# GAVLab/feature_extraction

Measured on AMD Instinct MI355X. Metric: VLP-16 scans/sec (16x1800 pts), detector+descriptor, higher is better.
Workload: dtype f32; 1 GPU; batch of 1024 synthetic VLP-16 scans (16x1800 pts, 64 uniform poles) per GPU, device-resident, preset 'launch', roll/pitch 0.02/-0.015; scans_per_gpu=1024, preset=launch, parallelism=frame-sharded x1, batches_in_flight=4

## Files before the change

feature_extraction_amd/capi.py:

```python
import ctypes as C
import os

import numpy as np

_HERE = os.path.dirname(os.path.abspath(__file__))
LIB_PATH = os.path.join(_HERE, "lib", "libfx_hip.so")

FX_DESC_BINS = 1980
FX_DESC_FLOATS = 1989
FX_FEATURE_RECORD_BYTES = 7984
FX_OK = 0
FX_ERR_NO_DEVICE = 2
FX_IN_DEVICE, FX_OUT_HOST, FX_OUT_DEBUG, FX_OUT_CLOUDS = 1, 2, 4, 8
FX_FLAG_RING_OVERFLOW, FX_FLAG_CAND_OVERFLOW, FX_FLAG_KP_OVERFLOW, FX_FLAG_NBR_OVERFLOW = 0x1, 0x2, 0x4, 0x8
FX_FLAG_NAMES = {0x1: "RING_OVERFLOW", 0x2: "CAND_OVERFLOW", 0x4: "KP_OVERFLOW", 0x8: "NBR_OVERFLOW",
                 0x10: "TOTAL_KP_OVERFLOW", 0x20: "KPC_OVERFLOW"}
FX_N_STAGES = 9
STAGE_NAMES = ("k_prep", "k_bucket", "k_rings_runs", "k_rings_large", "k_merge", "k_gather", "k_desc_group", "k_desc_mid",
               "k_desc_rare")
SINGLE_LAUNCH_STAGES = ("k_prep", "k_bucket", "k_rings_runs", "k_gather", "k_desc_group", "k_desc_mid")
STAGE_KERNELS = {"k_prep": ("k_prep", "k_front", "k_front_ab"),
                 "k_bucket": ("k_bucket", "k_bucket_many"),
                 "k_rings_large": ("k_rings_runs2", "k_rings_large"),
                 "k_merge": ("k_merge_small", "k_merge_big", "k_merge_huge", "k_front_redo", "k_slow"),
                 "k_desc_mid": ("k_desc_mid",),
                 "k_gather": ("k_gather", "k_rng_ord"),
                 "k_desc_rare": ("k_dense_sort", "k_dense_density", "k_dense_finish")}


class FxParams(C.Structure):
    _fields_ = [("cloud_leveling", C.c_int32),
                ("x_min", C.c_double), ("x_max", C.c_double),
                ("y_min", C.c_double), ("y_max", C.c_double),
                ("z_min", C.c_double), ("z_max", C.c_double),
                ("cluster_tolerance", C.c_double),
                ("cluster_min_count", C.c_int32), ("cluster_max_count", C.c_int32),
                ("cluster_radius_threshold", C.c_double),
                ("number_detection_channels", C.c_int32),
                ("estimate_descriptors", C.c_int32),
                ("descriptor_radius", C.c_double),
                ("n_rings", C.c_int32), ("el0_deg", C.c_double), ("el_step_deg", C.c_double),
                ("secondary_max", C.c_int32)]


class FxLimits(C.Structure):
    _fields_ = [(n, C.c_uint32) for n in
                ("max_batch", "max_points", "max_ring_points", "max_ring_candidates", "max_candidates",
                 "max_keypoints", "max_neighbors", "max_total_keypoints", "max_kpc_points", "max_dense_points", "max_overflow_points")]


class FxScanDesc(C.Structure):
    _fields_ = [("points", C.c_void_p), ("n_points", C.c_uint32), ("stride_bytes", C.c_uint32),
                ("roll", C.c_double), ("pitch", C.c_double)]


_U32P, _F32P, _I32P = C.POINTER(C.c_uint32), C.POINTER(C.c_float), C.POINTER(C.c_int32)


class FxBatchView(C.Structure):
    _fields_ = [("batch", C.c_uint32), ("max_points", C.c_uint32), ("max_keypoints", C.c_uint32),
                ("max_candidates", C.c_uint32), ("max_kpc_points", C.c_uint32), ("total_keypoints", C.c_uint32),
                ("d_n_keypoints", C.c_void_p), ("d_kp_offset", C.c_void_p), ("d_keypoints", C.c_void_p),
                ("d_descriptors", C.c_void_p), ("d_flags", C.c_void_p), ("d_n_filtered", C.c_void_p),
                ("d_filtered", C.c_void_p), ("d_n_kpc", C.c_void_p), ("d_kpc", C.c_void_p),
                ("h_n_keypoints", _U32P), ("h_kp_offset", _U32P), ("h_keypoints", _F32P),
                ("h_descriptors", _F32P), ("h_flags", _U32P), ("h_n_filtered", _U32P), ("h_filtered", _F32P),
                ("h_n_kpc", _U32P), ("h_kpc", _F32P),
                ("h_n_candidates", _U32P), ("h_candidates", _F32P), ("h_cand_size", _U32P),
                ("h_cand_keypoint", _I32P), ("h_kpc_cand", _U32P), ("h_kp_size", _U32P),
                ("h_kp_neighbors", _U32P)]


class FxPc2Layout(C.Structure):
    _fields_ = [(n, C.c_uint32) for n in
                ("point_step", "offset_x", "offset_y", "offset_z", "offset_intensity", "is_bigendian")]


class FxTimings(C.Structure):
    _fields_ = [("ms", C.c_float * FX_N_STAGES), ("total_ms", C.c_float), ("k_prep_exec_ms", C.c_float)]


class FxStageBytes(C.Structure):
    _fields_ = [("read", C.c_double * FX_N_STAGES), ("written", C.c_double * FX_N_STAGES)]


class FxSynthCfg(C.Structure):
    _fields_ = [("n_rings", C.c_uint32), ("n_az", C.c_uint32), ("el0_deg", C.c_double), ("el_step_deg", C.c_double),
                ("n_poles", C.c_uint32), ("pole_radius", C.c_double), ("pole_height", C.c_double),
                ("x_lo", C.c_double), ("x_hi", C.c_double), ("y_lo", C.c_double), ("y_hi", C.c_double),
                ("sensor_height", C.c_double), ("wall_radius", C.c_double), ("seed", C.c_uint64)]


FX_HEADER_VERSION = (0 << 16) | 7
EXPORTS = ("fx_version", "fx_check_abi", "fx_status_str", "fx_last_error", "fx_params_default", "fx_params_launch",
           "fx_limits_default", "fx_limits_sparse", "fx_create", "fx_destroy", "fx_set_stream", "fx_get_stream", "fx_set_graph_batch", "fx_set_batches_in_flight", "fx_set_profiling", "fx_set_profiling_stages", "fx_get_timings",
           "fx_get_stage_bytes", "fx_get_limits", "fx_process_batch", "fx_synchronize", "fx_pack_features", "fx_pack_keypoint_records", "fx_keypoint_block_bytes", "fx_pack_keypoint_block",
           "fx_rotation_from_roll_pitch", "fx_sc3d_tables", "fx_sc3d_xaxis", "fx_synth_cfg_vlp16",
           "fx_synth_scan", "fx_unpack_pointcloud2", "fx_pack_pointxyzi")
TEST_EXPORTS = ("fx_test_sort_replay", "fx_test_sort_replay_ranked", "fx_test_sort_replay_lists", "fx_test_sort_replay_device",
                "fx_test_elevation_device", "fx_test_within_device")

_lib = None
_libs = {}
TEST_LIB_PATH = os.path.join(_HERE, "lib", "libfx_hip_test.so")


class test_hooks:

    def __enter__(self):
        global _lib, LIB_PATH
        self._saved = (_lib, LIB_PATH)
        LIB_PATH = TEST_LIB_PATH
        _lib = _libs.get(LIB_PATH)
        try:
            return load()
        except BaseException:
            _lib, LIB_PATH = self._saved
            raise

    def __exit__(self, *exc):
        global _lib, LIB_PATH
        _lib, LIB_PATH = self._saved
        return False


def load_test():
    with test_hooks() as lib:
        return lib


def load():
    global _lib
    if _lib is not None:
        return _lib
    if LIB_PATH in _libs:
        _lib = _libs[LIB_PATH]
        return _lib
    try:
        import torch
    except ImportError:
        pass
    if not os.path.exists(LIB_PATH):
        raise RuntimeError(
            f"{LIB_PATH} is missing: build it with `python -c 'import __graft_entry__ as g; g.build()'` "
            "(hipcc --offload-arch=gfx950). The hot path has no CPU fallback.")
    lib = C.CDLL(LIB_PATH)
    lib.fx_version.restype = C.c_uint32
    lib.fx_last_error.restype = C.c_char_p
    lib.fx_check_abi.argtypes = [C.c_uint32, C.c_size_t, C.c_size_t, C.c_size_t, C.c_size_t]
    if lib.fx_check_abi(FX_HEADER_VERSION, C.sizeof(FxParams), C.sizeof(FxLimits), C.sizeof(FxScanDesc), C.sizeof(FxBatchView)) != FX_OK:
        raise RuntimeError(f"{LIB_PATH}: {lib.fx_last_error().decode()}")
    lib.fx_status_str.restype = C.c_char_p
    lib.fx_status_str.argtypes = [C.c_int]
    lib.fx_last_error.restype = C.c_char_p
    lib.fx_params_default.argtypes = [C.POINTER(FxParams)]
    lib.fx_params_launch.argtypes = [C.POINTER(FxParams)]
    lib.fx_limits_default.argtypes = [C.POINTER(FxLimits), C.c_uint32, C.c_uint32]
    lib.fx_limits_sparse.argtypes = [C.POINTER(FxLimits), C.c_uint32, C.c_uint32]
    lib.fx_create.argtypes = [C.POINTER(FxParams), C.POINTER(FxLimits), C.c_int, C.POINTER(C.c_void_p)]
    lib.fx_create.restype = C.c_int
    lib.fx_destroy.argtypes = [C.c_void_p]
    lib.fx_destroy.restype = None
    lib.fx_set_stream.argtypes = [C.c_void_p, C.c_void_p]
    lib.fx_set_profiling.argtypes = [C.c_void_p, C.c_int]
    lib.fx_set_profiling_stages.argtypes = [C.c_void_p, C.c_uint32]
    lib.fx_set_graph_batch.argtypes = [C.c_void_p, C.c_uint32]
    lib.fx_set_batches_in_flight.argtypes = [C.c_void_p, C.c_uint32]
    lib.fx_get_stream.argtypes = [C.c_void_p, C.POINTER(C.c_void_p)]
    lib.fx_get_stream.restype = C.c_int
    lib.fx_get_timings.argtypes = [C.c_void_p, C.c_uint32, C.POINTER(FxTimings)]
    lib.fx_get_limits.argtypes = [C.c_void_p, C.POINTER(FxLimits)]
    lib.fx_get_stage_bytes.argtypes = [C.c_void_p, C.POINTER(FxStageBytes)]
    lib.fx_process_batch.argtypes = [C.c_void_p, C.POINTER(FxScanDesc), C.c_uint32, C.c_uint32,
                                     C.POINTER(FxBatchView)]
    lib.fx_process_batch.restype = C.c_int
    lib.fx_synchronize.argtypes = [C.c_void_p]
    lib.fx_pack_features.argtypes = [C.c_void_p, C.c_void_p, C.c_uint32]
# ... 215 lines not shown
```

feature_extraction_amd/csrc/fx_api.cpp:

```cpp
#include <hip/hip_runtime.h>

#include <algorithm>
#include <cmath>
#include <cstdio>
#include <cstdlib>
#include <cstring>
#include <string>
#include <utility>
#include <vector>

#include "../../include/fx.h"
#include "fx_device.h"

extern "C" {
size_t fxk_ring_large_lds_bytes(uint32_t cap, uint32_t ccap);
void fxk_rings_large(hipStream_t s, const FxDevParams &P, const FxBuffers &B, uint32_t cap, uint32_t ccap, uint32_t grid,
                     uint32_t after_runs2);
void fxk_rings_runs2(hipStream_t s, const FxDevParams &P, const FxBuffers &B, uint32_t max_pts, uint32_t grid);
size_t fxk_merge_lds_bytes(uint32_t cap, uint32_t n_rings);
size_t fxk_desc_lds_bytes(uint32_t cap);
size_t fxk_gather_lds_bytes(uint32_t max_keypoints);
uint32_t fxk_dense_cells(void);
uint32_t fxk_group_cap(void);
uint32_t fxk_dfin_k(void);
void fxk_dense(hipStream_t s, const FxDevParams &P, const FxBuffers &B, uint32_t n_cu, uint32_t rows, uint32_t items, uint32_t skip);
size_t fxk_dense_slow_words(uint32_t max_points);
size_t fxk_merge_huge_lds_bytes(uint32_t cap, uint32_t ccap, uint32_t n_rings);
hipError_t fxk_configure(size_t ring_big, size_t merge_big, size_t merge_huge, size_t desc_big, size_t gather);
uint32_t fxk_near_words(uint32_t max_points);
void fxk_prep(hipStream_t s, const FxDevParams &P, const FxBuffers &B, uint32_t batch, float near_margin, float el0, float inv_step,
              uint32_t clk_slot);
void fxk_bucket(hipStream_t s, const FxDevParams &P, const FxBuffers &B, uint32_t batch, float el0, float inv_step, uint32_t clk_next);
uint32_t fxk_prep_slices_max(void);
void fxk_prep_sliced(hipStream_t s, const FxDevParams &P, const FxBuffers &B, uint32_t batch, uint32_t slices, float near_margin, float el0, float inv_step,
                     uint32_t clk_slot);
void fxk_bucket_sliced(hipStream_t s, const FxDevParams &P, const FxBuffers &B, uint32_t batch, uint32_t slices, float el0, float inv_step,
                       uint32_t clk_next);
size_t fxk_ring_runs_lds_bytes(void);
void fxk_rings_runs(hipStream_t s, const FxDevParams &P, const FxBuffers &B, uint32_t batch, uint32_t max_pts, uint32_t grid);
void fxk_merge_small(hipStream_t s, const FxDevParams &P, const FxBuffers &B, uint32_t batch, uint32_t cap);
void fxk_merge_big(hipStream_t s, const FxDevParams &P, const FxBuffers &B, uint32_t cap, uint32_t grid, uint32_t last);
void fxk_merge_huge(hipStream_t s, const FxDevParams &P, const FxBuffers &B, uint32_t cap, uint32_t ccap, uint32_t grid);
size_t fxk_merge_hp_words(uint32_t cap);
uint32_t fxk_merge_slices_max(void);
void fxk_merge_huge_split(hipStream_t s, const FxDevParams &P, const FxBuffers &B, uint32_t cap, uint32_t ccap, uint32_t grid, uint32_t slices);
uint32_t fxk_front_max_rings(void);
uint32_t fxk_front_merge_cap(void);
void fxk_front(hipStream_t s, const FxDevParams &P, const FxBuffers &B, uint32_t batch, float near_margin, float el0, float inv_step,
               uint32_t clk_slot, uint32_t merge_cap, uint32_t force_redo);
void fxk_front_ab(hipStream_t s, const FxDevParams &P, const FxBuffers &B, uint32_t batch, float near_margin, float el0, float inv_step,
                  uint32_t clk_slot, uint32_t force_redo);
void fxk_front_cd(hipStream_t s, const FxDevParams &P, const FxBuffers &B, uint32_t batch, uint32_t clk_slot, uint32_t merge_cap, uint32_t lean,
                  uint32_t self_n, uint32_t force_redo);
void fxk_front_redo(hipStream_t s, const FxDevParams &P, const FxBuffers &B, float el0, float inv_step, uint32_t huge_ccap, uint32_t force_slow,
                    uint32_t grid);
size_t fxk_slow_words(uint32_t max_ring_points, uint32_t max_candidates, uint32_t huge_ccap);
void fxk_slow(hipStream_t s, const FxDevParams &P, const FxBuffers &B, uint32_t huge_ccap, uint32_t grid, uint32_t batch, uint32_t clk_next);
hipError_t fxk_configure_front(void);
uint32_t fxk_gather_slices(uint32_t batch);
uint32_t fxk_gather(hipStream_t s, const FxDevParams &P, const FxBuffers &B, uint32_t batch, float box_margin, uint32_t counted);
uint32_t fxk_gather_counted_max(void);
void fxk_desc_group(hipStream_t s, const FxDevParams &P, const FxBuffers &B, uint32_t batch, uint32_t grid);
void fxk_desc_mid(hipStream_t s, const FxDevParams &P, const FxBuffers &B, uint32_t batch, uint32_t cap, uint32_t n_wg, uint32_t n_wave,
                  uint32_t n_dslow);
void fxk_pack_kp_records(hipStream_t s, const FxDevParams &P, const FxBuffers &B, uint32_t batch, void *dst,
                         uint32_t rec_kp);
size_t fxk_kp_block_bytes(uint32_t max_scans, uint32_t max_total);
void fxk_pack_kp_block(hipStream_t s, const FxDevParams &P, const FxBuffers &B, uint32_t batch, void *dst, uint32_t max_scans, uint32_t max_total,
                       uint32_t grid);
void fxk_rng_ord(hipStream_t s, const FxDevParams &P, const FxBuffers &B, uint32_t batch);
#ifdef FX_TEST_HOOKS
void fxk_test_sort_replay(hipStream_t s, const uint32_t *sizes, uint32_t n_seq, uint32_t n, uint32_t *perm);
void fxk_test_elevation(hipStream_t s, const float *xyz, uint32_t n, const double *tab, float *fast, uint8_t *ok, float *exact);
void fxk_test_within(hipStream_t s, const float4 *sp, uint32_t n, const float4 *queries, uint32_t nq, float r2, uint32_t *packed, uint32_t *plain);
#endif
void fxk_unpack_pc2(hipStream_t s, const void *src, uint32_t n, uint32_t point_step, uint32_t ox, uint32_t oy, uint32_t oz,
                    uint32_t oi, uint32_t big_endian, void *dst, uint32_t grid);
void fxk_pack_xyzi32(hipStream_t s, const void *src, uint32_t n, void *dst, uint32_t grid);
void fxk_pack_features(hipStream_t s, const FxDevParams &P, const FxBuffers &B, uint32_t batch, void *dst,
                       uint32_t capacity, uint32_t grid);
}

namespace {
thread_local std::string g_last_error;

fx_status fail(fx_status s, const std::string &msg) {
  g_last_error = msg;
  return s;
}
#define FX_HIP(expr)                                                                              \
  do {                                                                                            \
    hipError_t e_ = (expr);                                                                       \
    if (e_ != hipSuccess)                                                                         \
      return fail(e_ == hipErrorOutOfMemory ? FX_ERR_OOM : FX_ERR_HIP,                            \
                  std::string(#expr) + ": " + hipGetErrorString(e_));                             \
  } while (0)

constexpr int kMetaSlots = 8;
inline const char *test_hook(const char *name) {
#ifdef FX_TEST_HOOKS
  return getenv(name);
#else
  (void)name;
  return nullptr;
#endif
}
constexpr uint32_t kMergeCapSmall = 512, kListCap = 4096, kDenseMin = 1024;
}

struct fx_ctx {
  fx_params params;
  fx_limits lim;
  int device = 0;
  int n_cu = 256;
  FxDevParams dp;
  FxBuffers buf;
  std::vector<void *> dev_allocs;
  std::vector<void *> host_allocs;
  hipStream_t own_stream = nullptr, stream = nullptr;
  FxScanMeta *h_meta[kMetaSlots] = {};
  hipEvent_t meta_ev[kMetaSlots] = {};
  bool meta_used[kMetaSlots] = {};
  int meta_next = 0;
  FxScanMeta *d_meta = nullptr;
  float box_margin = 0.f;
  uint32_t desc_wgs_per_cu = 0;
  uint32_t desc_grid_abs = 0;
  uint32_t batches_in_flight = 1;
  uint32_t ring_lds_cap = 0;
  uint32_t merge_big_cap = 0;
  uint32_t merge_huge_cap = 0;
  uint32_t merge_huge_ccap = 0;
  float *d_stage = nullptr;
  uint32_t stage_stride = 0;
  uint32_t *h_hdr = nullptr;
  size_t hdr_stride = 0;
  uint32_t *h_n_kp = nullptr, *h_kp_offset = nullptr, *h_flags = nullptr, *h_n_filt = nullptr, *h_n_kpc = nullptr,
           *h_n_cand = nullptr, *h_cand_size = nullptr, *h_kpc_cand = nullptr, *h_kp_size = nullptr,
           *h_kp_nbrs = nullptr;
  int32_t *h_cand_kp = nullptr;
  float *h_keypoints = nullptr, *h_desc = nullptr, *h_filtered = nullptr, *h_kpc = nullptr, *h_cand = nullptr;
  bool profiling = false;
  std::vector<hipEvent_t> ev_ring;
  uint32_t ev_depth = 0, ev_count = 0;
  uint32_t prof_mask = ~0u;
  std::vector<uint32_t> ev_mask;
  std::vector<uint64_t> ev_seq;
  uint64_t batch_seq = 0;
  double clk_khz = 100000.0;
  hipEvent_t *ev = nullptr;
  uint32_t last_batch = 0;
  std::vector<std::pair<uint32_t, hipGraphExec_t>> graphs;
  uint32_t graph_max_batch = 0;
  bool debug_sync = false;
  volatile uint32_t *tier_hint = nullptr;
  uint32_t tier_min_grid = 8;
  uint32_t hint_hold[FX_N_HINTS] = {}, hint_age[FX_N_HINTS] = {};
  static constexpr uint32_t hint_hold_batches = 64;
  bool front_ok = false;
  bool front_last = false;
  uint32_t front_force = 0;
  int front_stream = -1;
  static constexpr uint32_t front_stream_max_batch = 8;
  int front_split = 0;
  bool state_suspect = false;
  uint32_t fail_after = 0;
  uint32_t front_pause = 0;
  uint32_t dense_fast_left = 0;
  static constexpr uint32_t dense_linger = 64;
  int gather_slices = -1;
  int merge_slices = -1;
  int prep_slices = -1;
  int dense_force = -1;
  uint32_t skip_mask = 0;
  static constexpr uint32_t front_retry = 64;
};

namespace {

template <typename T>
fx_status dev_alloc(fx_ctx *c, T **p, size_t count) {
  void *q = nullptr;
  const size_t bytes = (count ? count : 1) * sizeof(T);
  hipError_t e = hipMalloc(&q, bytes);
  if (e != hipSuccess) return fail(FX_ERR_OOM, std::string("hipMalloc(") + std::to_string(bytes) + "): " + hipGetErrorString(e));
  c->dev_allocs.push_back(q);
  *p = (T *)q;
  return FX_OK;
}
template <typename T>
fx_status host_alloc(fx_ctx *c, T **p, size_t count) {
  if (*p) return FX_OK;
  void *q = nullptr;
  const size_t bytes = (count ? count : 1) * sizeof(T);
  hipError_t e = hipHostMalloc(&q, bytes, hipHostMallocDefault);
  if (e != hipSuccess) return fail(FX_ERR_OOM, std::string("hipHostMalloc(") + std::to_string(bytes) + "): " + hipGetErrorString(e));
  c->host_allocs.push_back(q);
  *p = (T *)q;
  return FX_OK;
}
#define FX_TRY(expr)              \
  do {                            \
    fx_status s_ = (expr);        \
    if (s_ != FX_OK) return s_;   \
  } while (0)

}

namespace {
std::vector<double> atan_table() {
  std::vector<double> at((FX_ATAN_N + 1) * (FX_ATAN_DEG + 1));
  for (int i = 0; i <= FX_ATAN_N; ++i) {
    const long double cpt = (long double)i / FX_ATAN_N, a0 = atanl(cpt), th = atan2l(1.0L, cpt), st = sinl(th);
    long double pw = 1.0L;
    at[(size_t)i * (FX_ATAN_DEG + 1)] = (double)a0;
    for (int kk = 1; kk <= FX_ATAN_DEG; ++kk) {
      pw *= st;
      at[(size_t)i * (FX_ATAN_DEG + 1) + kk] = (double)(((kk & 1) ? 1.0L : -1.0L) * pw * sinl(kk * th) / kk);
    }
  }
  return at;
}

fx_status enqueue_stages(fx_ctx *c, hipStream_t s, uint32_t batch, bool prof, bool front, bool capture = false) {
  const fx_limits &L = c->lim;
  const FxDevParams &P = c->dp;
  const FxBuffers &B = c->buf;
  const uint32_t big_grid = (uint32_t)c->n_cu;
  uint32_t hint[FX_N_HINTS];
  for (int i = 0; i < FX_N_HINTS; ++i) {
    hint[i] = (capture || !c->tier_min_grid) ? 0xffffffffu : c->tier_hint[i];
    if (capture || !c->tier_min_grid) continue;
    if (hint[i] == 0xffffffffu || c->hint_hold[i] == 0xffffffffu || hint[i] >= c->hint_hold[i] || ++c->hint_age[i] > fx_ctx::hint_hold_batches)
      c->hint_hold[i] = hint[i], c->hint_age[i] = 0;
    hint[i] = c->hint_hold[i];
  }
  auto tier_grid = [&](uint32_t work, uint32_t full, uint32_t bound, uint32_t per = 1, uint32_t min_wg = 0) -> uint32_t {
    uint32_t g = work > full / 2 ? full : 2 * work;
    const uint32_t floor_wg = min_wg ? std::min(min_wg, c->tier_min_grid) : c->tier_min_grid;
    if (g < (floor_wg + per - 1) / per) g = (floor_wg + per - 1) / per;
    if (g > bound) g = bound ? bound : 1;
    return g < full ? g : full;
  };
  if (prof) {
    c->ev = &c->ev_ring[(size_t)(c->ev_count % c->ev_depth) * (FX_N_STAGES + 1)];
    c->ev_mask[c->ev_count % c->ev_depth] = c->prof_mask;
    c->ev_seq[c->ev_count % c->ev_depth] = c->batch_seq;
  }
  const uint32_t pmask = c->prof_mask;
  auto mark = [&](int i) -> hipError_t {
    if (c->debug_sync) {
      fprintf(stderr, "[fx] stage %d enqueued\n", i);
      hipError_t e = hipStreamSynchronize(s);
      if (e != hipSuccess) return e;
    }
    const bool wanted = i == 0 || i == FX_N_STAGES || ((pmask >> i) & 1u) || ((pmask >> (i - 1)) & 1u);
    return (prof && wanted) ? hipEventRecord(c->ev[i], s) : hipSuccess;
  };
  FX_HIP(mark(0));
  if (!batch) FX_HIP(hipMemsetAsync(B.counters, 0, FX_N_COUNTERS * sizeof(uint32_t), s));
  if (batch) {
    const uint32_t merge_small = L.max_candidates < kMergeCapSmall ? L.max_candidates : kMergeCapSmall;
    const uint32_t desc_per_cu = c->desc_wgs_per_cu ? c->desc_wgs_per_cu : (c->batches_in_flight >= 4u ? 1u : (c->batches_in_flight == 3u ? 3u : 10u));
    const uint32_t rows_bound = std::min<uint64_t>((uint64_t)batch * L.max_keypoints, L.max_total_keypoints);
    uint32_t desc_grid = std::max(1u, std::min((uint32_t)c->n_cu * desc_per_cu, (rows_bound + 15u) / 16u));
    if (c->desc_grid_abs) desc_grid = c->desc_grid_abs;
    const uint32_t clk_slot = (uint32_t)(c->batch_seq % FX_CLK_SLOTS), clk_next = (uint32_t)((c->batch_seq + 1) % FX_CLK_SLOTS);
    const float el0 = (float)c->params.el0_deg, inv_step = (float)(1.0 / c->params.el_step_deg);
    if (front) {
      const uint32_t mcap = std::min(fxk_front_merge_cap(), L.max_candidates);
      const bool split = c->front_split != 0;
      const bool stream = c->front_stream >= 0 ? c->front_stream != 0 : batch <= fx_ctx::front_stream_max_batch;
      if (stream && !split) {
        fxk_prep_sliced(s, P, B, batch, fxk_prep_slices_max(), c->box_margin, el0, inv_step, clk_slot);
        FX_HIP(mark(1));
        fxk_bucket_sliced(s, P, B, batch, fxk_prep_slices_max(), el0, inv_step, clk_next);
        fxk_front_cd(s, P, B, batch, clk_slot, mcap, 0u, 1u, c->front_force >= 1u ? 1u : 0u);
      } else if (split) {
        fxk_front_ab(s, P, B, batch, c->box_margin, el0, inv_step, clk_slot, c->front_force >= 1u ? 1u : 0u);
        FX_HIP(mark(1));
        fxk_front_cd(s, P, B, batch, clk_slot, mcap, c->front_split >= 2 ? 1u : 0u, 0u, 0u);
      } else {
        fxk_front(s, P, B, batch, c->box_margin, el0, inv_step, clk_slot, mcap, c->front_force >= 1u ? 1u : 0u);
        FX_HIP(mark(1));
      }
      for (int i = 2; i <= 4; ++i) FX_HIP(mark(i));
      const uint32_t redo_floor = c->batches_in_flight >= 4u ? 1u : 4u;
      if (!(c->skip_mask & 1u))
      fxk_front_redo(s, P, B, el0, inv_step, c->merge_huge_ccap, c->front_force >= 2u ? 1u : 0u, tier_grid(hint[6], 2 * big_grid, batch, 1, redo_floor));
      fxk_slow(s, P, B, c->merge_huge_ccap, tier_grid(hint[7], big_grid, batch), batch, clk_next);
      FX_HIP(mark(5));
    } else {
    uint32_t slices = 1;
    if (c->prep_slices >= 0) {
      slices = (uint32_t)c->prep_slices;
    } else if (4u * batch <= 2u * big_grid && L.max_points >= 65536u) {
      slices = 3u * big_grid / batch;
    }
    slices = std::max(1u, std::min(slices, fxk_prep_slices_max()));
    if (slices > 1) {
      fxk_prep_sliced(s, P, B, batch, slices, c->box_margin, el0, inv_step, clk_slot);
      FX_HIP(mark(1));
      fxk_bucket_sliced(s, P, B, batch, slices, el0, inv_step, clk_next);
    } else {
      fxk_prep(s, P, B, batch, c->box_margin, el0, inv_step, clk_slot);
      FX_HIP(mark(1));
      fxk_bucket(s, P, B, batch, el0, inv_step, clk_next);
    }
    FX_HIP(mark(2));
    fxk_rings_runs(s, P, B, batch, L.max_ring_points, (batch * (uint32_t)c->params.n_rings + 7) / 8 * 8);
    FX_HIP(mark(3));
    const bool runs2 = c->params.n_rings > 16;
    const uint32_t n_items = batch * (uint32_t)c->params.n_rings;
    if (runs2) fxk_rings_runs2(s, P, B, L.max_ring_points, 8 * tier_grid(hint[0], (big_grid * 7 + 7) / 8, (n_items + 7) / 8, 8));
    fxk_rings_large(s, P, B, c->ring_lds_cap, c->ring_lds_cap, 8 * tier_grid(hint[runs2 ? 1 : 0], (big_grid + 7) / 8, (n_items + 7) / 8, 8),
                    runs2 ? 1u : 0u);
    FX_HIP(mark(4));
    fxk_merge_small(s, P, B, batch, merge_small);
    fxk_merge_big(s, P, B, c->merge_big_cap, tier_grid(hint[2], big_grid, batch), c->merge_big_cap >= L.max_candidates);
    if (c->merge_big_cap < L.max_candidates) {
      const uint32_t g = tier_grid(hint[3], big_grid, batch);
      uint32_t slices = 1;
      if (c->merge_slices >= 0)
        slices = (uint32_t)c->merge_slices;
      else if (!capture && hint[3] != 0xffffffffu && hint[3] > 0 && 2u * hint[3] * c->batches_in_flight <= big_grid)
        slices = big_grid / (hint[3] * c->batches_in_flight);
      slices = std::min(slices, fxk_merge_slices_max());
      if (slices > 1 && B.merge_hp)
        fxk_merge_huge_split(s, P, B, c->merge_huge_cap, c->merge_huge_ccap, g, slices);
      else
        fxk_merge_huge(s, P, B, c->merge_huge_cap, c->merge_huge_ccap, g);
    }
    fxk_slow(s, P, B, c->merge_huge_ccap, tier_grid(hint[7], big_grid, batch), batch, clk_next);
    FX_HIP(mark(5));
    }
    if (P.estimate_descriptors) {
      uint32_t counted = 1;
      if (c->gather_slices >= 0)
        counted = (uint32_t)c->gather_slices;
      else if (!capture && 10u * batch * c->batches_in_flight <= 3u * big_grid && L.max_points >= 65536u)
        counted = 3u * big_grid / (batch * c->batches_in_flight);
      if (fxk_gather(s, P, B, batch, c->box_margin, counted) > 1) fxk_rng_ord(s, P, B, batch);
      FX_HIP(mark(6));
      fxk_desc_group(s, P, B, batch, desc_grid);
      FX_HIP(mark(7));
      bool fast = capture || hint[4] != 0u;
      if (fast && !capture && hint[4] != 0xffffffffu) c->dense_fast_left = fx_ctx::dense_linger;
      if (!fast && c->dense_fast_left) --c->dense_fast_left, fast = true;
      if (c->dense_force >= 0) fast = c->dense_force == 0;
      const bool skip_dense = (c->skip_mask & 2u) != 0u;
      fxk_desc_mid(s, P, B, batch, P.list_cap < P.dense_min ? P.list_cap : P.dense_min, std::max(1u, std::min(big_grid * 4, rows_bound)),
                   std::max(1u, std::min(big_grid * 4, (rows_bound + 3u) / 4u)), fast || skip_dense ? 0u : (c->tier_min_grid ? c->tier_min_grid : 8u));
      FX_HIP(mark(8));
      if (fast && !skip_dense) {
        const uint32_t max_rows = batch * L.max_keypoints < L.max_total_keypoints ? batch * L.max_keypoints : L.max_total_keypoints;
        const uint32_t rows = tier_grid(hint[4], 3 * big_grid, max_rows);
        const uint32_t items = hint[5] == 0xffffffffu ? 3 * big_grid : tier_grid(hint[4] + hint[5] / 1024u, 3 * big_grid, 0xffffffffu);
        fxk_dense(s, P, B, big_grid, rows, items, (c->skip_mask >> 2) & 3u);
      }
    } else {
      for (int i = 6; i <= 8; ++i) FX_HIP(mark(i));
    }
    FX_HIP(mark(9));
    FX_HIP(hipGetLastError());
  } else {
    for (int i = 1; i <= FX_N_STAGES; ++i) FX_HIP(mark(i));
  }
  return FX_OK;
}

fx_status launch_graph(fx_ctx *c, hipStream_t s, uint32_t batch, bool front) {
  hipGraphExec_t exec = nullptr;
  const uint32_t key = batch | (front ? 0x80000000u : 0u);
  for (auto &g : c->graphs)
    if (g.first == key) exec = g.second;
  if (!exec) {
    hipGraph_t graph = nullptr;
    FX_HIP(hipStreamBeginCapture(s, hipStreamCaptureModeThreadLocal));
    fx_status st = enqueue_stages(c, s, batch, false, front, true);
    hipError_t e = hipStreamEndCapture(s, &graph);
    if (st != FX_OK) {
      if (graph) (void)hipGraphDestroy(graph);
      return st;
    }
    FX_HIP(e);
    e = hipGraphInstantiate(&exec, graph, nullptr, nullptr, 0);
    (void)hipGraphDestroy(graph);
    FX_HIP(e);
    if (c->graphs.size() >= 8) {
      (void)hipGraphExecDestroy(c->graphs.front().second);
      c->graphs.erase(c->graphs.begin());
    }
    c->graphs.emplace_back(key, exec);
  }
  FX_HIP(hipGraphLaunch(exec, s));
  return FX_OK;
}
}

extern "C" {

const char *fx_last_error(void) { return g_last_error.c_str(); }

fx_status fx_check_abi(uint32_t header_version, size_t sizeof_params, size_t sizeof_limits, size_t sizeof_scan_desc, size_t sizeof_batch_view) {
  const uint32_t lib_version = ((uint32_t)FX_VERSION_MAJOR << 16) | FX_VERSION_MINOR;
  if (header_version == lib_version && sizeof_params == sizeof(fx_params) && sizeof_limits == sizeof(fx_limits) &&
      sizeof_scan_desc == sizeof(fx_scan_desc) && sizeof_batch_view == sizeof(fx_batch_view))
    return FX_OK;
  char msg[256];
  snprintf(msg, sizeof msg, "caller compiled against fx.h %u.%u (fx_params %zu, fx_limits %zu, fx_scan_desc %zu, fx_batch_view %zu bytes); "
           "this library is %u.%u (%zu, %zu, %zu, %zu)", header_version >> 16, header_version & 0xffffu, sizeof_params, sizeof_limits,
           sizeof_scan_desc, sizeof_batch_view, lib_version >> 16, lib_version & 0xffffu, sizeof(fx_params), sizeof(fx_limits),
           sizeof(fx_scan_desc), sizeof(fx_batch_view));
  return fail(FX_ERR_INVALID_ARG, msg);
}

fx_status fx_create(const fx_params *params, const fx_limits *limits, int device_id, fx_ctx **out) {
  if (!params || !limits || !out) return fail(FX_ERR_INVALID_ARG, "null argument");
  *out = nullptr;
  int n_dev = 0;
  hipError_t e = hipGetDeviceCount(&n_dev);
  if (e != hipSuccess || n_dev <= 0)
    return fail(FX_ERR_NO_DEVICE, std::string("hipGetDeviceCount: ") + (e != hipSuccess ? hipGetErrorString(e) : "0 devices"));
  if (device_id < 0 || device_id >= n_dev) return fail(FX_ERR_INVALID_ARG, "device_id out of range");

  fx_limits L = *limits;
  fx_limits D;
  fx_limits_default(&D, L.max_batch, L.max_points);
  if (!L.max_ring_points) L.max_ring_points = D.max_ring_points;
  if (!L.max_ring_candidates) L.max_ring_candidates = D.max_ring_candidates;
  if (!L.max_candidates) L.max_candidates = D.max_candidates;
  if (!L.max_keypoints) L.max_keypoints = D.max_keypoints;
  if (!L.max_neighbors) L.max_neighbors = D.max_neighbors;
  if (!L.max_total_keypoints) L.max_total_keypoints = D.max_total_keypoints;
  if (!L.max_kpc_points) L.max_kpc_points = D.max_kpc_points;
  if (!L.max_dense_points) L.max_dense_points = D.max_dense_points;
  if (!L.max_overflow_points) L.max_overflow_points = D.max_overflow_points;
  if (L.max_batch == 0 || L.max_points == 0) return fail(FX_ERR_INVALID_ARG, "max_batch and max_points must be > 0");
  if (L.max_batch > 65535) return fail(FX_ERR_INVALID_ARG, "max_batch > 65535 (one grid row per scan in the support gather)");
  if (L.max_points > (1u << 20)) return fail(FX_ERR_INVALID_ARG, "max_points > 2^20 (descriptor sort key packs the point index in 20 bits)");
  if (params->n_rings < 1 || params->n_rings > 1024) return fail(FX_ERR_INVALID_ARG, "n_rings must be in [1, 1024]");
  if (!(params->descriptor_radius > 0.0) || !(params->el_step_deg > 0.0))
    return fail(FX_ERR_INVALID_ARG, "descriptor_radius and el_step_deg must be > 0");
  if (params->descriptor_radius < 1e-12 || params->descriptor_radius > 1e12)
    return fail(FX_ERR_INVALID_ARG, "descriptor_radius out of range");
  if (L.max_ring_candidates > L.max_ring_points) L.max_ring_candidates = L.max_ring_points;
  const size_t kLds = 160 * 1024;
  if (L.max_ring_points > 32768 || L.max_candidates > 32768 || L.max_keypoints > 65535)
    return fail(FX_ERR_INVALID_ARG, "limit exceeds the 16-bit packing of the order replay (max_ring_points, max_candidates <= 32768)");
  uint32_t ring_lds_cap = L.max_ring_points;
  while (fxk_ring_large_lds_bytes(ring_lds_cap, ring_lds_cap) > kLds) ring_lds_cap -= ring_lds_cap > 64 ? 16 : 1;
  uint32_t merge_big_cap = L.max_candidates;
  while (fxk_merge_lds_bytes(merge_big_cap, params->n_rings) > kLds) merge_big_cap -= merge_big_cap > 64 ? 64 : 1;
  if (const char *e = test_hook("FX_MERGE_BIG_CAP")) {
    const uint32_t v = (uint32_t)atoi(e);
    if (v >= 16 && v < merge_big_cap) merge_big_cap = v;
  }
  const uint32_t merge_huge_ccap = L.max_keypoints > 64 ? L.max_keypoints : 64;
  uint32_t merge_huge_cap = L.max_candidates;
  while (merge_huge_cap > merge_big_cap && fxk_merge_huge_lds_bytes(merge_huge_cap, merge_huge_ccap, params->n_rings) > kLds) merge_huge_cap -= 64;
  if (merge_huge_cap < merge_big_cap) merge_huge_cap = merge_big_cap;
  if (const char *e = test_hook("FX_MERGE_HUGE_CAP")) {
    const uint32_t v = (uint32_t)atoi(e);
    if (v >= merge_big_cap && v < merge_huge_cap) merge_huge_cap = v;
  }
  if (const char *e = test_hook("FX_RING_LDS_CAP")) {
    const uint32_t v = (uint32_t)atoi(e);
    if (v >= 16 && v < ring_lds_cap) ring_lds_cap = v & ~3u;
  }
  if (fxk_gather_lds_bytes(L.max_keypoints) > kLds) return fail(FX_ERR_INVALID_ARG, "support gather: LDS tables beyond the budget (build parameter FX_GATHER_KCAP)");

  FX_HIP(hipSetDevice(device_id));
  fx_ctx *c = new fx_ctx();
  c->params = *params;
  c->lim = L;
  c->device = device_id;
  c->ring_lds_cap = ring_lds_cap;
  c->merge_big_cap = merge_big_cap;
  c->merge_huge_cap = merge_huge_cap;
  c->merge_huge_ccap = merge_huge_ccap;
  if (const char *e = test_hook("FX_DESC_WGS_PER_CU")) {
    const int v = atoi(e);
    if (v >= 1 && v <= 32) c->desc_wgs_per_cu = (uint32_t)v;
  }
  if (const char *e = test_hook("FX_DESC_GRID")) c->desc_grid_abs = (uint32_t)std::max(0, atoi(e));
  if (const char *e = test_hook("FX_DEBUG_SYNC")) c->debug_sync = atoi(e) != 0;
  if (const char *e = test_hook("FX_GRAPH_MAX_BATCH")) {
    const int v = atoi(e);
    if (v >= 0) c->graph_max_batch = (uint32_t)v;
  }
  hipDeviceProp_t prop;
  if (hipGetDeviceProperties(&prop, device_id) == hipSuccess) c->n_cu = prop.multiProcessorCount;

  FxDevParams &P = c->dp;
  std::memset(&P, 0, sizeof(P));
  P.x_min = (float)params->x_min;
  P.x_max = (float)params->x_max;
  P.y_min = (float)params->y_min;
  P.y_max = (float)params->y_max;
  P.z_min = (float)params->z_min;
  P.z_max = (float)params->z_max;
  P.n_rings = params->n_rings;
  {
    const double tol = (double)(float)params->cluster_tolerance;
    P.r2_cluster = (float)(tol * tol);
    const double crt = (double)(float)params->cluster_radius_threshold;
    P.r2_merge = (float)(crt * crt);
  }
  P.min_count = (uint32_t)params->cluster_min_count;
  P.max_count = (uint32_t)params->cluster_max_count;
  P.gate_diameter = 2 * params->cluster_radius_threshold;
  P.crt = params->cluster_radius_threshold;
  P.ndc = (uint32_t)params->number_detection_channels;
  P.secondary_max = (uint32_t)params->secondary_max;
  {
    const double R = params->descriptor_radius, rd = params->descriptor_radius / 5.0;
    P.r2_search = (float)(R * R);
    P.r2_density = (float)(rd * rd);
    const double rs = (R + rd) * 1.0001 + 1e-4;
    P.r2_support = (float)(rs * rs);
    c->box_margin = (float)(rs * 1.001 + 1e-3);
  }
  P.estimate_descriptors = params->estimate_descriptors;
  P.max_points = L.max_points;
  P.max_ring_cands = L.max_ring_candidates;
  P.max_candidates = L.max_candidates;
  P.max_keypoints = L.max_keypoints;
  P.max_total_kp = L.max_total_keypoints;
  P.max_kpc = L.max_kpc_points;
  P.max_neighbors = L.max_neighbors;
  P.max_ring_points = L.max_ring_points;
  P.list_cap = L.max_neighbors < kListCap ? L.max_neighbors : kListCap;
  P.near_words = fxk_near_words(L.max_points);
  P.dense_min = kDenseMin;
  P.ovf_cap = L.max_overflow_points > 0x7ff00000u ? 0x7ff00000u : L.max_overflow_points;
  {
    const unsigned long long want = L.max_dense_points ? L.max_dense_points : (unsigned long long)(L.max_batch > 32u ? L.max_batch : 32u) * L.max_points;
    P.dense_cap = (uint32_t)(want > 0xfff00000ull ? 0xfff00000ull : (want < 4096ull ? 4096ull : want));
    const uint32_t per_row = P.list_cap < P.dense_min ? P.list_cap : P.dense_min;
    const unsigned long long rows = (unsigned long long)P.dense_cap / (per_row ? per_row : 1u) + 1ull;
    P.max_dense_rows = (uint32_t)(rows < L.max_total_keypoints ? rows : L.max_total_keypoints);
  }
  P.dense_qcap = P.dense_cap > 0x7ff00000u ? 0xfff00000u : 2u * P.dense_cap;
  P.dense_lds_keys = fxk_dfin_k();
  if (const char *e = test_hook("FX_DENSE_LDS_KEYS")) {
    const int v = atoi(e);
    if (v >= 1 && (uint32_t)v < P.dense_lds_keys) P.dense_lds_keys = (uint32_t)v;
  }
  P.dense_won_points = 0xffffffffu;
  if (const char *e = test_hook("FX_DENSE_WON_POINTS")) {
    const int v = atoi(e);
    if (v >= 0) P.dense_won_points = (uint32_t)v;
  }
  P.ring_slot_cap = 2 * L.max_points;
  P.ring_list_cap = ((L.max_batch + 7) / 8) * (uint32_t)params->n_rings;

  fx_status st = FX_OK;
  auto bail = [&](fx_status s) {
    fx_destroy(c);
    return s;
  };
#define FX_A(expr)                     \
  st = (expr);                         \
  if (st != FX_OK) return bail(st)

  const size_t B = L.max_batch, R = (size_t)params->n_rings;
  FxBuffers &b = c->buf;
  std::memset(&b, 0, sizeof(b));
  FX_A(dev_alloc(c, &c->d_meta, B));
  b.meta = c->d_meta;
  float2 *d_win = nullptr;
  FX_A(dev_alloc(c, &d_win, R));
  b.ring_win = d_win;
  double *d_atan = nullptr;
  FX_A(dev_alloc(c, &d_atan, (size_t)(FX_ATAN_N + 1) * (FX_ATAN_DEG + 1)));
  b.atan_tab = d_atan;
  FxScTables *d_tab = nullptr;
  FX_A(dev_alloc(c, &d_tab, 1));
  b.tables = d_tab;
  float2 *d_xa = nullptr;
  FX_A(dev_alloc(c, &d_xa, L.max_keypoints));
  b.xaxis = d_xa;
  FX_A(dev_alloc(c, &b.filt, B * L.max_points));
  {
    c->hdr_stride = (B + 1 + 3) & ~(size_t)3;
    uint32_t *hdr = nullptr;
    FX_A(dev_alloc(c, &hdr, 5 * c->hdr_stride));
    if (hipMemset(hdr, 0, 5 * c->hdr_stride * sizeof(uint32_t)) != hipSuccess) return bail(fail(FX_ERR_HIP, "hipMemset"));
    b.n_kp = hdr, b.kp_offset = hdr + c->hdr_stride, b.flags = hdr + 2 * c->hdr_stride, b.n_filt = hdr + 3 * c->hdr_stride,
    b.n_kpc = hdr + 4 * c->hdr_stride;
  }
  FX_A(dev_alloc(c, &b.near_bits, B * P.near_words));
  FX_A(dev_alloc(c, &b.prep_cnt, B * fxk_prep_slices_max()));
  FX_A(dev_alloc(c, &b.prep_ring_cnt, B * fxk_prep_slices_max() * R));
  FX_A(dev_alloc(c, &b.ring_cand, B * R * L.max_ring_candidates));
  FX_A(dev_alloc(c, &b.ring_cand_size, B * R * L.max_ring_candidates));
  FX_A(dev_alloc(c, &b.ring_cand_cnt, B * R));
  FX_A(dev_alloc(c, &b.ring_pts, B * P.ring_slot_cap));
  FX_A(dev_alloc(c, &b.ring_off, B * R));
  FX_A(dev_alloc(c, &b.ring_cnt, B * R));
  FX_A(dev_alloc(c, &b.kpc_pool, B * P.ring_slot_cap));
  FX_A(dev_alloc(c, &b.kpc_pool_cand, B * P.ring_slot_cap));
  FX_A(dev_alloc(c, &b.kpc_ring_cnt, B * R));
  FX_A(dev_alloc(c, &b.cand, B * L.max_candidates));
  FX_A(dev_alloc(c, &b.cand_size, B * L.max_candidates));
  FX_A(dev_alloc(c, &b.cand_kp, B * L.max_candidates));
  FX_A(dev_alloc(c, &b.n_cand, B));
  FX_A(dev_alloc(c, &b.keypoints, B * L.max_keypoints));
  FX_A(dev_alloc(c, &b.kp_size, B * L.max_keypoints));
  FX_A(dev_alloc(c, &b.kp_nbrs, B * L.max_keypoints));
  FX_A(dev_alloc(c, &b.kpc, B * L.max_kpc_points));
  FX_A(dev_alloc(c, &b.kpc_cand, B * L.max_kpc_points));
  FX_A(dev_alloc(c, &b.desc, (size_t)L.max_total_keypoints * FX_DESC_FLOATS + 4));
  FX_A(dev_alloc(c, &b.desc_nbins, (size_t)L.max_total_keypoints));
  FX_A(dev_alloc(c, &b.desc_bins, (size_t)L.max_total_keypoints * fxk_group_cap()));
  if (hipMemset(b.desc, 0, ((size_t)L.max_total_keypoints * FX_DESC_FLOATS + 4) * sizeof(float)) != hipSuccess ||
      hipMemset(b.desc_nbins, 0, (size_t)L.max_total_keypoints * sizeof(uint32_t)) != hipSuccess)
    return bail(fail(FX_ERR_HIP, "hipMemset"));
  FX_A(dev_alloc(c, &b.huge_rings, (size_t)8 * P.ring_list_cap));
  FX_A(dev_alloc(c, &b.huge_rings2, (size_t)8 * P.ring_list_cap));
  FX_A(dev_alloc(c, &b.big_merge, B));
  FX_A(dev_alloc(c, &b.huge_merge, B));
  FX_A(dev_alloc(c, &b.redo, B));
  FX_A(dev_alloc(c, &b.front_n, B));
  FX_A(dev_alloc(c, &b.slow, B));
  FX_A(dev_alloc(c, &b.slow_state, B));
  FX_A(dev_alloc(c, &b.ring_pending, B * ((R + 31) / 32)));
  if (hipMemset(b.slow_state, 0, B * sizeof(uint32_t)) != hipSuccess || hipMemset(b.ring_pending, 0, B * ((R + 31) / 32) * sizeof(uint32_t)) != hipSuccess)
    return bail(fail(FX_ERR_HIP, "hipMemset"));
  {
    const size_t words = fxk_slow_words(L.max_ring_points, L.max_candidates, c->merge_huge_ccap);
    size_t slots = std::min<size_t>((size_t)c->n_cu, B);
    while (slots > 1 && slots * words * 4 > ((size_t)256 << 20)) --slots;
    P.gs_words = (uint32_t)words;
    P.gs_slots = (uint32_t)slots;
    FX_A(dev_alloc(c, &b.gs_pool, slots * words));
  }
  {
    const size_t words = fxk_dense_slow_words(L.max_points);
    size_t slots = 32;
    while (slots > 1 && slots * words * 4 > ((size_t)128 << 20)) --slots;
    P.gsd_words = (uint32_t)words;
    P.gsd_slots = (uint32_t)slots;
    FX_A(dev_alloc(c, &b.gsd_pool, slots * words));
  }
  FX_A(dev_alloc(c, &b.merge_sorted, (size_t)B * L.max_candidates));
  if (c->merge_big_cap < L.max_candidates && (size_t)B * fxk_merge_hp_words(c->merge_huge_cap) * 4 <= ((size_t)256 << 20))
    FX_A(dev_alloc(c, &b.merge_hp, (size_t)B * fxk_merge_hp_words(c->merge_huge_cap)));
  FX_A(dev_alloc(c, &b.list_desc, L.max_total_keypoints));
  FX_A(dev_alloc(c, &b.s_pts, (size_t)L.max_total_keypoints * P.list_cap));
  FX_A(dev_alloc(c, &b.s_cnt, L.max_total_keypoints));
  FX_A(dev_alloc(c, &b.gather_cnt, (size_t)B * fxk_gather_counted_max() * L.max_keypoints));
  FX_A(dev_alloc(c, &b.row_map, L.max_total_keypoints));
  FX_A(dev_alloc(c, &b.row_kp, L.max_total_keypoints));
  FX_A(dev_alloc(c, &b.row_xa, L.max_total_keypoints));
  FX_A(dev_alloc(c, &b.wave_desc, L.max_total_keypoints));
  FX_A(dev_alloc(c, &b.dense_rows, P.max_dense_rows));
  FX_A(dev_alloc(c, &b.dense_order, (size_t)4 * P.max_dense_rows));
  FX_A(dev_alloc(c, &b.dense_off, P.max_dense_rows));
  FX_A(dev_alloc(c, &b.dense_koff, P.max_dense_rows));
  FX_A(dev_alloc(c, &b.dense_nq, P.max_dense_rows));
  FX_A(dev_alloc(c, &b.dense_nm, P.max_dense_rows));
  FX_A(dev_alloc(c, &b.dense_cells, (size_t)P.max_dense_rows * fxk_dense_cells()));
  FX_A(dev_alloc(c, &b.dense_items, (size_t)P.dense_cap / 256 + P.max_dense_rows + 1));
  FX_A(dev_alloc(c, &b.dense_pts, P.dense_cap));
  FX_A(dev_alloc(c, &b.dense_q, P.dense_qcap));
  FX_A(dev_alloc(c, &b.dense_qoff, P.max_dense_rows));
  FX_A(dev_alloc(c, &b.dense_key, P.dense_cap));
  FX_A(dev_alloc(c, &b.dens_cache, B * L.max_points));
  FX_A(dev_alloc(c, &b.seq, 1));
  FX_A(dev_alloc(c, &b.ovf_pts, (size_t)B * P.ovf_cap));
  FX_A(dev_alloc(c, &b.ovf_kp, (size_t)B * P.ovf_cap));
  FX_A(dev_alloc(c, &b.ovf_cnt, B));
  if (hipMemset(b.dens_cache, 0, B * L.max_points * sizeof(unsigned long long)) != hipSuccess) return bail(fail(FX_ERR_HIP, "hipMemset"));
  if (hipMemset(b.seq, 0, sizeof(unsigned long long)) != hipSuccess) return bail(fail(FX_ERR_HIP, "hipMemset"));
  if (hipMemset(b.ovf_cnt, 0, B * sizeof(uint32_t)) != hipSuccess) return bail(fail(FX_ERR_HIP, "hipMemset"));
  FX_A(dev_alloc(c, &b.counters, FX_N_COUNTER_WORDS));
  {
    uint32_t *h = nullptr;
    FX_A(host_alloc(c, &h, FX_N_HINTS));
    for (int i = 0; i < FX_N_HINTS; ++i) h[i] = 0xffffffffu;
    void *dv = nullptr;
    if (hipHostGetDevicePointer(&dv, h, 0) != hipSuccess) return bail(fail(FX_ERR_HIP, "hipHostGetDevicePointer"));
    b.tier_hint = (uint32_t *)dv;
    c->tier_hint = h;
    if (const char *e = test_hook("FX_TIER_MIN_GRID")) c->tier_min_grid = (uint32_t)std::max(0, atoi(e));
  }
  FX_A(dev_alloc(c, &b.clk, 2 * FX_CLK_SLOTS));
  {
    std::vector<unsigned long long> init(2 * FX_CLK_SLOTS);
    for (int i = 0; i < FX_CLK_SLOTS; ++i) init[2 * i] = ~0ull, init[2 * i + 1] = 0ull;
    if (hipMemcpy(b.clk, init.data(), init.size() * 8, hipMemcpyHostToDevice) != hipSuccess) return bail(fail(FX_ERR_HIP, "hipMemcpy"));
    int khz = 0;
    if (hipDeviceGetAttribute(&khz, hipDeviceAttributeWallClockRate, device_id) == hipSuccess && khz > 0) c->clk_khz = khz;
  }
  FX_A(dev_alloc(c, &b.stamps, 64 * 64));
  if (hipMemset(b.stamps, 0, 64 * 64 * 8) != hipSuccess) return bail(fail(FX_ERR_HIP, "hipMemset"));

  {
    std::vector<float2> win(R);
    const double half = params->el_step_deg / 2.0;
    for (size_t i = 0; i < R; ++i) {
      const double centre = params->el0_deg + (double)i * params->el_step_deg;
      win[i].x = (float)(centre - half);
      win[i].y = (float)(centre + half);
    }
    if (hipMemcpy(d_win, win.data(), R * sizeof(float2), hipMemcpyHostToDevice) != hipSuccess)
      return bail(fail(FX_ERR_HIP, "upload ring windows"));
    {
      const std::vector<double> at = atan_table();
      if (hipMemcpy(d_atan, at.data(), at.size() * sizeof(double), hipMemcpyHostToDevice) != hipSuccess)
        return bail(fail(FX_ERR_HIP, "upload arctangent table"));
    }
    FxScTables T;
    std::vector<float> lut(FX_DESC_BINS);
    fx_sc3d_tables(params->descriptor_radius, T.radii, T.theta, T.phi, lut.data());
    for (int k = 0; k < 11; ++k)
      for (int j = 0; j < 15; ++j) T.lut[k * 15 + j] = lut[k * 15 + j];
    if (hipMemcpy(d_tab, &T, sizeof(T), hipMemcpyHostToDevice) != hipSuccess)
      return bail(fail(FX_ERR_HIP, "upload 3DSC tables"));
    std::vector<float2> xa(L.max_keypoints);
    for (uint32_t k = 0; k < L.max_keypoints; ++k) {
      float xy[2];
      fx_sc3d_xaxis(k, xy);
      xa[k].x = xy[0];
      xa[k].y = xy[1];
    }
    if (hipMemcpy(d_xa, xa.data(), xa.size() * sizeof(float2), hipMemcpyHostToDevice) != hipSuccess)
      return bail(fail(FX_ERR_HIP, "upload 3DSC x-axes"));
  }
  for (int i = 0; i < kMetaSlots; ++i) {
    FX_A(host_alloc(c, &c->h_meta[i], B));
    if (hipEventCreateWithFlags(&c->meta_ev[i], hipEventDisableTiming) != hipSuccess)
      return bail(fail(FX_ERR_HIP, "hipEventCreate"));
  }
  if (hipStreamCreateWithFlags(&c->own_stream, hipStreamNonBlocking) != hipSuccess)
    return bail(fail(FX_ERR_HIP, "hipStreamCreate"));
  c->stream = c->own_stream;
  {
    hipError_t ce = fxk_configure(fxk_ring_large_lds_bytes(c->ring_lds_cap, c->ring_lds_cap), fxk_merge_lds_bytes(c->merge_big_cap, params->n_rings),
                                  c->merge_big_cap < L.max_candidates ? fxk_merge_huge_lds_bytes(c->merge_huge_cap, c->merge_huge_ccap, params->n_rings) : 0,
                                  fxk_desc_lds_bytes(P.list_cap < P.dense_min ? P.list_cap : P.dense_min), fxk_gather_lds_bytes(L.max_keypoints));
    if (ce != hipSuccess) return bail(fail(FX_ERR_HIP, std::string("hipFuncSetAttribute: ") + hipGetErrorString(ce)));
  }
  if (hipMemset(b.counters, 0, FX_N_COUNTER_WORDS * sizeof(uint32_t)) != hipSuccess) return bail(fail(FX_ERR_HIP, "hipMemset"));
  c->front_ok = (uint32_t)params->n_rings <= fxk_front_max_rings();
  if (const char *e = test_hook("FX_FRONT")) c->front_ok = c->front_ok && atoi(e) != 0;
  if (const char *e = test_hook("FX_FRONT_FORCE")) c->front_force = (uint32_t)std::max(0, atoi(e));
  if (const char *e = test_hook("FX_FRONT_STREAM")) c->front_stream = atoi(e) != 0 ? 1 : 0;
  if (const char *e = test_hook("FX_FRONT_SPLIT")) c->front_split = std::max(0, std::min(2, atoi(e)));
  if (const char *e = test_hook("FX_FAIL_AFTER_ENQUEUE")) c->fail_after = (uint32_t)std::max(0, atoi(e));
  if (const char *e = test_hook("FX_SKIP_EMPTY")) c->skip_mask = (uint32_t)std::max(0, atoi(e));
  if (const char *e = test_hook("FX_DENSE_SLOW")) c->dense_force = atoi(e) != 0 ? 1 : 0;
  if (const char *e = test_hook("FX_PREP_SLICES")) c->prep_slices = std::max(1, atoi(e));
  if (const char *e = test_hook("FX_MERGE_SLICES")) c->merge_slices = std::max(1, atoi(e));
  if (const char *e = test_hook("FX_GATHER_COUNTED")) c->gather_slices = std::max(1, atoi(e));
  if (c->front_ok) {
    hipError_t ce = fxk_configure_front();
    if (ce != hipSuccess) return bail(fail(FX_ERR_HIP, std::string("hipFuncSetAttribute: ") + hipGetErrorString(ce)));
  }
  if (hipMemset(b.kp_offset, 0, (B + 1) * sizeof(uint32_t)) != hipSuccess) return bail(fail(FX_ERR_HIP, "hipMemset"));
  if (hipMemset(b.n_kp, 0, B * sizeof(uint32_t)) != hipSuccess) return bail(fail(FX_ERR_HIP, "hipMemset"));
#undef FX_A
  *out = c;
  return FX_OK;
}

void fx_destroy(fx_ctx *c) {
  if (!c) return;
  (void)hipSetDevice(c->device);
  if (c->own_stream) (void)hipStreamSynchronize(c->own_stream);
  (void)hipDeviceSynchronize();
  for (void *p : c->dev_allocs) (void)hipFree(p);
  for (void *p : c->host_allocs) (void)hipHostFree(p);
  if (c->d_stage) (void)hipFree(c->d_stage);
  for (int i = 0; i < kMetaSlots; ++i)
    if (c->meta_ev[i]) (void)hipEventDestroy(c->meta_ev[i]);
  for (hipEvent_t e : c->ev_ring) (void)hipEventDestroy(e);
  for (auto &g : c->graphs) (void)hipGraphExecDestroy(g.second);
  if (c->own_stream) (void)hipStreamDestroy(c->own_stream);
  delete c;
}

fx_status fx_set_stream(fx_ctx *c, void *hip_stream) {
  if (!c) return fail(FX_ERR_INVALID_ARG, "null ctx");
  c->stream = hip_stream ? (hipStream_t)hip_stream : c->own_stream;
  return FX_OK;
}
fx_status fx_get_stream(fx_ctx *c, void **hip_stream) {
  if (!c || !hip_stream) return fail(FX_ERR_INVALID_ARG, "null argument");
  *hip_stream = (void *)c->stream;
  return FX_OK;
}
fx_status fx_set_batches_in_flight(fx_ctx *c, uint32_t n) {
  if (!c) return fail(FX_ERR_INVALID_ARG, "null ctx");
  c->batches_in_flight = n ? n : 1u;
  if (!c->graphs.empty()) {
    FX_HIP(hipSetDevice(c->device));
    FX_HIP(hipStreamSynchronize(c->stream));
    for (auto &g : c->graphs) (void)hipGraphExecDestroy(g.second);
    c->graphs.clear();
  }
  return FX_OK;
}
fx_status fx_set_graph_batch(fx_ctx *c, uint32_t max_batch) {
  if (!c) return fail(FX_ERR_INVALID_ARG, "null ctx");
  c->graph_max_batch = max_batch;
  return FX_OK;
}

fx_status fx_set_profiling(fx_ctx *c, int depth) {
  if (!c || depth < 0) return fail(FX_ERR_INVALID_ARG, "bad argument");
  FX_HIP(hipSetDevice(c->device));
  FX_HIP(hipStreamSynchronize(c->stream));
  for (hipEvent_t e : c->ev_ring) (void)hipEventDestroy(e);
  c->ev_ring.clear();
  c->ev_depth = (uint32_t)depth;
  c->ev_count = 0;
  c->profiling = depth > 0;
  c->ev_ring.resize((size_t)depth * (FX_N_STAGES + 1), nullptr);
  c->ev_mask.assign((size_t)depth, ~0u);
  c->ev_seq.assign((size_t)depth, 0);
  for (hipEvent_t &e : c->ev_ring) FX_HIP(hipEventCreate(&e));
  return FX_OK;
}
fx_status fx_get_limits(const fx_ctx *c, fx_limits *l) {
  if (!c || !l) return fail(FX_ERR_INVALID_ARG, "null argument");
  *l = c->lim;
  return FX_OK;
}
fx_status fx_set_profiling_stages(fx_ctx *c, uint32_t stage_mask) {
  if (!c) return fail(FX_ERR_INVALID_ARG, "null ctx");
  c->prof_mask = stage_mask;
  return FX_OK;
}
fx_status fx_get_timings(fx_ctx *c, uint32_t back, fx_timings *t) {
  if (!c || !t) return fail(FX_ERR_INVALID_ARG, "null argument");
  std::memset(t, 0, sizeof(*t));
  if (!c->profiling || back >= c->ev_count || back >= c->ev_depth)
    return fail(FX_ERR_INVALID_ARG, "no profiled batch that far back (fx_set_profiling(depth) first)");
  hipEvent_t *ev = &c->ev_ring[(size_t)((c->ev_count - 1 - back) % c->ev_depth) * (FX_N_STAGES + 1)];
  FX_HIP(hipEventSynchronize(ev[FX_N_STAGES]));
  const uint32_t mask = c->ev_mask[(c->ev_count - 1 - back) % c->ev_depth];
  for (int i = 0; i < FX_N_STAGES; ++i)
    if ((mask >> i) & 1u) FX_HIP(hipEventElapsedTime(&t->ms[i], ev[i], ev[i + 1]));
  FX_HIP(hipEventElapsedTime(&t->total_ms, ev[0], ev[FX_N_STAGES]));
  {
    const uint64_t seq = c->ev_seq[(c->ev_count - 1 - back) % c->ev_depth];
    unsigned long long span[2] = {0, 0};
    if (c->batch_seq - seq < FX_CLK_SLOTS - 1) {
      FX_HIP(hipMemcpy(span, c->buf.clk + 2 * (seq % FX_CLK_SLOTS), sizeof(span), hipMemcpyDeviceToHost));
      if (span[1] > span[0]) t->k_prep_exec_ms = (float)((double)(span[1] - span[0]) / c->clk_khz);
    }
  }
  return FX_OK;
}
fx_status fx_get_stage_bytes(fx_ctx *c, fx_stage_bytes *out) {
  if (!c || !out) return fail(FX_ERR_INVALID_ARG, "null argument");
  std::memset(out, 0, sizeof(*out));
  const uint32_t B = c->last_batch;
  if (!B) return FX_OK;
  FX_HIP(hipSetDevice(c->device));
  FX_HIP(hipStreamSynchronize(c->stream));
  const fx_limits &L = c->lim;
  const FxBuffers &b = c->buf;
  const size_t R = (size_t)c->params.n_rings;
  auto fetch = [&](const uint32_t *src, size_t n, std::vector<uint32_t> &v) -> hipError_t {
    v.resize(n);
    return n ? hipMemcpy(v.data(), src, n * 4, hipMemcpyDeviceToHost) : hipSuccess;
  };
  std::vector<uint32_t> n_filt, ring_cnt, ring_cand, kpc_ring, n_cand, n_kp, n_kpc, kp_off, s_cnt, near;
  std::vector<FxScanMeta> meta(B);
  FX_HIP(hipMemcpy(meta.data(), c->d_meta, (size_t)B * sizeof(FxScanMeta), hipMemcpyDeviceToHost));
  FX_HIP(fetch(b.n_filt, B, n_filt));
  FX_HIP(fetch(b.ring_cnt, B * R, ring_cnt));
  FX_HIP(fetch(b.ring_cand_cnt, B * R, ring_cand));
  FX_HIP(fetch(b.kpc_ring_cnt, B * R, kpc_ring));
  FX_HIP(fetch(b.n_cand, B, n_cand));
  FX_HIP(fetch(b.n_kp, B, n_kp));
  FX_HIP(fetch(b.n_kpc, B, n_kpc));
  FX_HIP(fetch(b.kp_offset, B + 1, kp_off));
  uint32_t total_kp = kp_off[B] < L.max_total_keypoints ? kp_off[B] : L.max_total_keypoints;
  FX_HIP(fetch(b.s_cnt, total_kp, s_cnt));
  FX_HIP(fetch(b.near_bits, (size_t)B * c->dp.near_words, near));
  double n_pts = 0, nf = 0, n_ring = 0, n_rc = 0, n_mem = 0, nc = 0, nk = 0, nkpc = 0, near_pts = 0;
  for (uint32_t i = 0; i < B; ++i) {
    n_pts += meta[i].n, nf += n_filt[i], nc += n_cand[i], nk += n_kp[i], nkpc += n_kpc[i];
    for (size_t r = 0; r < R; ++r) n_ring += ring_cnt[i * R + r], n_rc += ring_cand[i * R + r], n_mem += kpc_ring[i * R + r];
    if (n_kp[i]) {
      const uint32_t words = (meta[i].n + 127u) / 128u;
      for (uint32_t w = 0; w < words && w < c->dp.near_words; ++w) near_pts += 4.0 * __builtin_popcount(near[(size_t)i * c->dp.near_words + w]);
    }
  }
  double s_small = 0, s_mid = 0, s_dense = 0, rows_mid = 0, rows_dense = 0;
  for (uint32_t r = 0; r < total_kp; ++r) {
    const double n = s_cnt[r];
    if (s_cnt[r] > c->dp.dense_min || s_cnt[r] > c->dp.list_cap)
      s_dense += n, rows_dense += 1;
    else if (s_cnt[r] > 64u)
      s_mid += n, rows_mid += 1;
    else
      s_small += n;
  }
  const bool desc = c->params.estimate_descriptors != 0;
  double *rd = out->read, *wr = out->written;
  rd[0] = 16.0 * n_pts, wr[0] = 16.0 * nf + n_pts / 32.0 + 4.0 * R * B;
// ... 408 lines not shown
```

feature_extraction_amd/csrc/fx_device.h:

```cpp
#ifndef FX_DEVICE_H_
#define FX_DEVICE_H_
#include <stdint.h>

struct FxScanMeta {
  const float *pts;
  uint32_t n;
  uint32_t stride_f;
  float R[9];
  uint32_t pad_;
};

struct FxDevParams {
  float x_min, x_max, y_min, y_max, z_min, z_max;
  int32_t n_rings;
  float r2_cluster;
  uint32_t min_count, max_count;
  double gate_diameter;
  double crt;
  float r2_merge;
  uint32_t ndc, secondary_max;
  float r2_search, r2_density, r2_support;
  int32_t estimate_descriptors;
  uint32_t max_points, max_ring_cands, max_candidates, max_keypoints, max_total_kp, max_kpc, max_neighbors,
      max_ring_points, list_cap, ring_slot_cap;
  uint32_t ring_list_cap;
  uint32_t near_words;
  uint32_t dense_min;
  uint32_t ovf_cap;
  uint32_t dense_cap;
  uint32_t max_dense_rows;
  uint32_t dense_qcap;
  uint32_t dense_lds_keys;
  uint32_t dense_won_points;
  uint32_t gs_slots;
  uint32_t gs_words;
  uint32_t gsd_slots, gsd_words;
};

struct FxScTables {
  float radii[16];
  float theta[12];
  float phi[13];
  float lut[165];
};

#define FX_CLK_SLOTS 64
#define FX_N_COUNTERS 48
#define FX_CNT_REDO 48
#define FX_CNT_SLOW_TICKET 50
#define FX_N_COUNTER_WORDS 56
#define FX_CNT_RUNS2_TICKET 40
#define FX_ATAN_N 64
#define FX_ATAN_DEG 6
#define FX_ROW_DIRTY 0xffffffffu
#define FX_N_HINTS 8
#define FX_CNT_QPOOL 32
#define FX_CNT_LARGE2 16
#define FX_CNT_LARGE 24
struct FxBuffers {
  const FxScanMeta *meta;
  const float2 *ring_win;
  const double *atan_tab;
  const FxScTables *tables;
  const float2 *xaxis;
  float4 *filt;
  uint32_t *n_filt;
  uint32_t *near_bits;
  uint32_t *prep_cnt;
  uint32_t *prep_ring_cnt;
  float4 *ring_pts;
  uint32_t *ring_off;
  uint32_t *ring_cnt;
  float4 *ring_cand;
  uint32_t *ring_cand_size;
  uint32_t *ring_cand_cnt;
  float4 *kpc_pool;
  uint32_t *kpc_pool_cand;
  uint32_t *kpc_ring_cnt;
  float4 *cand;
  uint32_t *cand_size;
  int32_t *cand_kp;
  uint32_t *n_cand;
  float4 *keypoints;
  uint32_t *kp_size;
  uint32_t *kp_nbrs;
  uint32_t *n_kp;
  uint32_t *kp_offset;
  float4 *kpc;
  uint32_t *kpc_cand;
  uint32_t *n_kpc;
  float *desc;
  uint32_t *desc_nbins;
  uint16_t *desc_bins;
  uint32_t *flags;
  uint32_t *huge_rings;
  uint32_t *huge_rings2;
  uint32_t *big_merge;
  uint32_t *huge_merge;
  uint32_t *front_n;
  uint32_t *redo;
  uint32_t *slow;
  uint32_t *slow_state;
  uint32_t *ring_pending;
  uint32_t *gs_pool;
  uint32_t *gsd_pool;
  uint32_t *merge_hp;
  float4 *merge_sorted;
  uint32_t *list_desc;
  uint32_t *wave_desc;
  uint32_t *dense_rows;
  uint32_t *dense_order;
  uint32_t *dense_off;
  uint32_t *dense_koff;
  uint32_t *dense_qoff;
  uint32_t *dense_nq;
  uint32_t *dense_nm;
  uint32_t *dense_cells;
  uint2 *dense_items;
  float4 *dense_pts;
  uint32_t *dense_q;
  unsigned long long *dense_key;
  unsigned long long *dens_cache;
  unsigned long long *seq;
  float4 *ovf_pts;
  uint32_t *ovf_kp;
  uint32_t *ovf_cnt;
  uint32_t *gather_cnt;
  float4 *s_pts;
  uint32_t *s_cnt;
  uint2 *row_map;
  float4 *row_kp;
  float2 *row_xa;
  unsigned long long *clk;
  unsigned long long *stamps;
  uint32_t *tier_hint;
  uint32_t *counters;
};

#endif
```

feature_extraction_amd/csrc/fx_kernels.hip:

```cpp
#include <hip/hip_runtime.h>
#include <float.h>
#include <math.h>
#include <type_traits>
#include <algorithm>

#include "fx_device.h"
#include "fx_sort_replay.h"
#include "../../include/fx.h"

#pragma clang fp contract(off)

#define FX_WG 256
#define FX_NWAVE (FX_WG / 64)

namespace {

typedef float fx_f2 __attribute__((ext_vector_type(2)));

__device__ __forceinline__ uint32_t lanes_below(unsigned long long m) {
  return __builtin_amdgcn_mbcnt_hi((uint32_t)(m >> 32), __builtin_amdgcn_mbcnt_lo((uint32_t)m, 0u));
}

__device__ __forceinline__ uint32_t wave_incl_scan(uint32_t x) {
  x += (uint32_t)__builtin_amdgcn_update_dpp(0, (int)x, 0x111, 0xf, 0xf, false);
// ... 3559 lines not shown
    if (b < batch) {
      const uint32_t off = run + ex;
      B.kp_offset[b] = off;
      if (off + c > P.max_total_kp) atomicOr(&B.flags[b], FX_FLAG_TOTAL_KP_OVERFLOW);
    }
    run += tot;
  }
  if (threadIdx.x == 0) {
    uint32_t l1 = 0, l2 = 0;
    for (uint32_t c = 0; c < 8u; ++c) l1 = max(l1, B.counters[FX_CNT_LARGE + c]), l2 = max(l2, B.counters[FX_CNT_LARGE2 + c]);
    B.tier_hint[0] = l1;
    B.tier_hint[1] = l2;
    B.tier_hint[2] = B.counters[1];
    B.tier_hint[3] = B.counters[9];
    B.tier_hint[6] = B.counters[FX_CNT_REDO];
    B.tier_hint[7] = B.counters[FX_CNT_REDO + 1];
    B.counters[FX_CNT_REDO] = 0u;
    B.counters[FX_CNT_REDO + 1] = 0u;
    B.clk[2 * clk_next] = ~0ull;
    B.clk[2 * clk_next + 1] = 0ull;
    B.kp_offset[batch] = run;
    B.seq[0] += 1ull;
  }
}


__device__ __forceinline__ uint32_t dense_class(uint32_t nS);
__device__ __forceinline__ uint32_t dense_class_counter(uint32_t cls);

__device__ __forceinline__ uint32_t scan_of_row(const uint32_t *kp_offset, uint32_t batch, uint32_t w) {
  uint32_t lo = 0, hi = batch;
  while (hi - lo > 1) {
    const uint32_t mid = (lo + hi) >> 1;
    if (kp_offset[mid] <= w)
      lo = mid;
    else
      hi = mid;
  }
  return lo;
}

#define FX_FAST_EPS_DEG 5e-4f
__device__ __forceinline__ bool near_multiple(float v, float step, float inv_step) {
  const float t = v * inv_step;
  return fabsf(t - rintf(t)) * step < FX_FAST_EPS_DEG;
}
__device__ __noinline__ void sc3d_angles_exact(float cn, float xd, float tc, float *phi, float *theta) {
  *phi = (float)atan2((double)cn, (double)xd) * 57.29578f;
  *theta = (float)acos((double)tc) * 57.29578f;
}
template <bool FAST>
__device__ __forceinline__ uint32_t sc3d_bin(const float4 kp, float bx, float by, float bz, float d2, const float2 xa,
                                             const FxScTables *T, float &lut, bool &amb) {
  const float nx = 0.0f, ny = 0.0f, nz = 1.0f;
  const float ax = xa.x, ay = xa.y, az = -0.0f;
  const float r = sqrtf(d2);
  const float pox = bx - kp.x, poy = by - kp.y, poz = bz - kp.z;
  const float lambda = nx * pox + (ny * poy + nz * poz);
  float p0 = (bx - lambda * nx) - kp.x;
  float p1 = (by - lambda * ny) - kp.y;
  float p2 = (bz - lambda * nz) - kp.z;
  {
    const float zz = p0 * p0 + (p1 * p1 + p2 * p2);
    if (zz > 0.0f) {
      const float s = sqrtf(zz);
      p0 /= s;
      p1 /= s;
      p2 /= s;
    }
  }
  const float c0 = ay * p2 - az * p1;
  const float c1 = az * p0 - ax * p2;
  const float c2 = ax * p1 - ay * p0;
  const float cn = sqrtf(c0 * c0 + (c1 * c1 + c2 * c2));
  const float xd = ax * p0 + (ay * p1 + az * p2);
  float phi = (FAST ? atan2f(cn, xd) : (float)atan2((double)cn, (double)xd)) * 57.29578f;
  const float cdn = c0 * nx + (c1 * ny + c2 * nz);
  phi = cdn < 0.f ? (360.0f - phi) : phi;
  float n0 = pox, n1 = poy, n2 = poz;
  {
    const float zz = n0 * n0 + (n1 * n1 + n2 * n2);
    if (zz > 0.0f) {
      const float s = sqrtf(zz);
      n0 /= s;
      n1 /= s;
      n2 /= s;
    }
  }
  float theta = nx * n0 + (ny * n1 + nz * n2);
  const float mx = (-1.0f < theta) ? theta : -1.0f;
  const float tc = (mx < 1.0f) ? mx : 1.0f;
  theta = (FAST ? acosf(tc) : (float)acos((double)tc)) * 57.29578f;
#ifndef FX_TRIG_LITERAL_F32
  if (FAST) {
    if (!(phi == phi) || !(theta == theta) || near_multiple(phi, 30.0f, 1.0f / 30.0f) ||
        near_multiple(theta, 180.0f / 11.0f, 11.0f / 180.0f)) {
      float pe, te;
      sc3d_angles_exact(cn, xd, tc, &pe, &te);
      phi = cdn < 0.f ? (360.0f - pe) : pe;
      theta = te;
    }
  }
#endif

  uint32_t j = 0, kk = 0, l = 0;
#pragma unroll
  for (uint32_t rad = 1; rad < 16; ++rad) j += (r > T->radii[rad]) ? 1u : 0u;
#pragma unroll
  for (uint32_t ang = 1; ang < 12; ++ang) kk += (theta > T->theta[ang]) ? 1u : 0u;
#pragma unroll
  for (uint32_t ang = 1; ang < 13; ++ang) l += (phi > T->phi[ang]) ? 1u : 0u;
  j = j == 15u ? 0u : j;
  kk = kk == 11u ? 0u : kk;
  l = l == 12u ? 0u : l;
  lut = T->lut[kk * 15 + j];
  return (l * 11 + kk) * 15 + j;
}
#ifdef FX_SKIP_EPSILON
__device__ __forceinline__ bool sc3d_is_origin(float d2) { return fabsf(d2 - 0.0f) < FLT_EPSILON; }
#else
__device__ __forceinline__ bool sc3d_is_origin(float d2) { return fabsf(d2 - 0.0f) < FLT_MIN; }
#endif
__device__ __forceinline__ unsigned long long sc3d_key(uint32_t bin, float d2, uint32_t idx) {
  return ((unsigned long long)bin << 52) | ((unsigned long long)__float_as_uint(d2) << 20) | (unsigned long long)idx;
}

#ifndef FX_GATHER_T
#define FX_GATHER_T 256
#endif
#define FX_GATHER_WIDE_T 1024
#define FX_GATHER_G 32
#define FX_GATHER_CELLS (FX_GATHER_G * FX_GATHER_G)
#ifndef FX_GATHER_STAGE
#define FX_GATHER_STAGE 384
#endif
#ifndef FX_GATHER_DIRECT
#define FX_GATHER_DIRECT 1
#endif
#ifndef FX_GATHER_QUEUE
#define FX_GATHER_QUEUE 128
#endif
#define FX_GATHER_QUEUE_WIDE 80
#define FX_GATHER_KCAP 2048
__host__ __device__ constexpr uint32_t gather_queue(uint32_t nt) { return nt <= 256u ? (uint32_t)FX_GATHER_QUEUE : (uint32_t)FX_GATHER_QUEUE_WIDE; }
__host__ __device__ inline uint32_t gather_words(uint32_t mk, uint32_t nt) {
  uint32_t w = 32 + 4 * mk;
  w += FX_GATHER_CELLS + 4;
  w += ((9 * mk + 1) / 2 + 3) & ~3u;
  w += (5 * mk + 3) & ~3u;
  w += FX_GATHER_STAGE + 4 * FX_GATHER_STAGE;
  w += (nt / 64) * gather_queue(nt) * 5;
  return w;
}
template <int NT, bool PASSES, int MODE = 0>
__device__ __forceinline__ void gather_body(const FxDevParams &P, const FxBuffers &B, float box_margin, uint32_t *smem) {
  static_assert(MODE == 0 || !PASSES, "the counted slices hold a scan's keypoints in one pass");
  static_assert(MODE == 0 || FX_GATHER_DIRECT, "the scatter pass writes its hits straight to their slots");
  constexpr uint32_t FX_GATHER_NW = NT / 64;
  const uint32_t MK = PASSES ? (uint32_t)FX_GATHER_KCAP : P.max_keypoints;
  uint32_t *s_w = smem;
  float4 *s_kp = reinterpret_cast<float4 *>(smem + 32);
  uint32_t *s_cell = smem + 32 + 4 * MK;
  uint16_t *s_flat = reinterpret_cast<uint16_t *>(s_cell + FX_GATHER_CELLS + 4);
  uint32_t *s_kcnt = reinterpret_cast<uint32_t *>(s_flat) + (((9 * MK + 1) / 2 + 3) & ~3u);
  uint32_t *s_kbase = s_kcnt + MK;
  uint32_t *s_kpos = s_kbase + MK;
  uint32_t *s_knbr = s_kpos + MK;
  uint32_t *s_kovf = s_knbr + MK;
  uint32_t *s_smeta = s_kcnt + ((5 * MK + 3) & ~3u);
  const bool solo = gridDim.x == 1 && MODE == 0;
  const bool own = solo || MODE == 2;
  float4 *s_spt = reinterpret_cast<float4 *>(s_smeta + FX_GATHER_STAGE);
  uint32_t *s_cur = reinterpret_cast<uint32_t *>(s_spt);
  const uint32_t scan = blockIdx.y, slice = blockIdx.x, tid = threadIdx.x, lane = tid & 63, wave = tid >> 6;
  constexpr uint32_t kQueue = gather_queue(NT);
  float4 *q_pt = s_spt + FX_GATHER_STAGE + wave * kQueue;
  uint32_t *q_info = reinterpret_cast<uint32_t *>(s_spt + FX_GATHER_STAGE + FX_GATHER_NW * kQueue) + wave * kQueue;
  uint32_t K_all = B.n_kp[scan];
  if (K_all == 0) return;
  const uint32_t row_first = B.kp_offset[scan];
  if (row_first >= P.max_total_kp) return;
  if (row_first + K_all > P.max_total_kp) K_all = P.max_total_kp - row_first;
  const FxScanMeta M = B.meta[scan];
  const bool passes = PASSES && K_all > MK;
  if (tid == 0) s_w[9] = 0;
  uint32_t kb = 0;
  do {
  const uint32_t K = PASSES ? min(MK, K_all - kb) : K_all, row0 = row_first + kb;
  __syncthreads();
  if (slice == 0 && MODE != 1)
    for (uint32_t k = tid; k < K; k += NT) B.row_map[row0 + k] = make_uint2(scan, kb + k);
  if (tid < 6) s_w[tid] = (tid & 1) ? f2ord(-INFINITY) : f2ord(INFINITY);
  if (tid == 0) s_w[8] = 0;
  for (uint32_t c = tid; c < FX_GATHER_CELLS; c += NT) s_cell[c] = 0;
  __syncthreads();
  for (uint32_t k = tid; k < K; k += NT) {
    const float4 kp = B.keypoints[(size_t)scan * P.max_keypoints + kb + k];
    s_kp[k] = kp;
    s_kcnt[k] = 0;
    s_kpos[k] = 0;
    s_knbr[k] = 0;
    if (slice == 0 && MODE != 1) B.row_kp[row0 + k] = kp;
    atomicMin(&s_w[0], f2ord(kp.x));
    atomicMax(&s_w[1], f2ord(kp.x));
    atomicMin(&s_w[2], f2ord(kp.y));
    atomicMax(&s_w[3], f2ord(kp.y));
    atomicMin(&s_w[4], f2ord(kp.z));
    atomicMax(&s_w[5], f2ord(kp.z));
  }
  __syncthreads();
  const float kx0 = ord2f(s_w[0]), kx1 = ord2f(s_w[1]), ky0 = ord2f(s_w[2]), ky1 = ord2f(s_w[3]);
  const float bx0 = kx0 - box_margin, bx1 = kx1 + box_margin;
  const float by0 = ky0 - box_margin, by1 = ky1 + box_margin;
  const float bz0 = ord2f(s_w[4]) - box_margin, bz1 = ord2f(s_w[5]) + box_margin;
  const float wx = fmaxf(box_margin, (bx1 - bx0) / (float)(FX_GATHER_G - 1) * 1.0001f + 1e-6f);
  const float wy = fmaxf(box_margin, (by1 - by0) / (float)(FX_GATHER_G - 1) * 1.0001f + 1e-6f);
  const float inv_wx = 1.0f / wx, inv_wy = 1.0f / wy;
  const int ncx = min((int)((bx1 - bx0) * inv_wx) + 1, FX_GATHER_G), ncy = min((int)((by1 - by0) * inv_wy) + 1, FX_GATHER_G);
  auto cell_x = [&](float x) { return min(max((int)floorf((x - bx0) * inv_wx), 0), ncx - 1); };
  auto cell_y = [&](float y) { return min(max((int)floorf((y - by0) * inv_wy), 0), ncy - 1); };
  for (uint32_t k = tid; k < K; k += NT) {
    const int cx = cell_x(s_kp[k].x), cy = cell_y(s_kp[k].y);
    for (int dy = -1; dy <= 1; ++dy)
      for (int dx = -1; dx <= 1; ++dx)
        if (cx + dx >= 0 && cx + dx < ncx && cy + dy >= 0 && cy + dy < ncy) atomicAdd(&s_cell[(cy + dy) * ncx + cx + dx], 1u);
  }
  __syncthreads();
  if (tid < 64) {
    const uint32_t n_cells = (uint32_t)(ncx * ncy), per = (n_cells + 63) / 64;
    uint32_t sum = 0;
    for (uint32_t u = 0; u < per; ++u) {
      const uint32_t ci = tid * per + u;
      sum += ci < n_cells ? s_cell[ci] : 0u;
    }
    uint32_t incl = sum;
    incl = wave_incl_scan(incl);
    uint32_t run = incl - sum;
    for (uint32_t u = 0; u < per; ++u) {
      const uint32_t ci = tid * per + u;
      if (ci < n_cells) {
        const uint32_t c = s_cell[ci];
        s_cell[ci] = run | (c << 20);
        s_cur[ci] = run;
        run += c;
      }
    }
  }
  __syncthreads();
  for (uint32_t k = tid; k < K; k += NT) {
    const int cx = cell_x(s_kp[k].x), cy = cell_y(s_kp[k].y);
    for (int dy = -1; dy <= 1; ++dy)
      for (int dx = -1; dx <= 1; ++dx)
        if (cx + dx >= 0 && cx + dx < ncx && cy + dy >= 0 && cy + dy < ncy)
          s_flat[atomicAdd(&s_cur[(cy + dy) * ncx + cx + dx], 1u)] = (uint16_t)k;
  }
  __syncthreads();

  if (MODE == 2) {
    const uint32_t S = gridDim.x;
    const uint32_t *cnt = B.gather_cnt + (size_t)scan * S * P.max_keypoints;
    uint32_t ovf_before = 0, ovf_all = 0;
    for (uint32_t k = tid; k < K; k += NT) {
      uint32_t run = 0, mine = 0;
      for (uint32_t sl = 0; sl < S; ++sl) {
        const uint32_t c = cnt[(size_t)sl * P.max_keypoints + k];
        const uint32_t o = run + c > P.list_cap ? run + c - max(run, P.list_cap) : 0u;
        if (sl == slice) mine = run;
        if (sl < slice) ovf_before += o;
        ovf_all += o;
        run += c;
      }
      s_kpos[k] = mine;
      if (slice == 0) B.s_cnt[row0 + k] = run;
    }
    if (ovf_before) atomicAdd(&s_w[9], ovf_before);
    if (slice == 0 && ovf_all) atomicAdd(&B.ovf_cnt[scan], ovf_all);
    __syncthreads();
  }
  constexpr uint32_t kTile = NT * 4;
  const uint32_t n = M.n;
  uint32_t chunk = (n + gridDim.x - 1) / gridDim.x;
  chunk = (chunk + kTile - 1) / kTile * kTile;
  const uint32_t tstep = MODE != 0 ? gridDim.x * kTile : kTile;
  const uint32_t lo = MODE != 0 ? slice * kTile : slice * chunk;
  const uint32_t hi = MODE != 0 ? n : (lo + chunk < n ? lo + chunk : n);
  const uint32_t *near_bits = B.near_bits + (size_t)scan * P.near_words;
  float4 *ovf_pts = B.ovf_pts + (size_t)scan * P.ovf_cap;
  uint32_t *ovf_kp = B.ovf_kp + (size_t)scan * P.ovf_cap;
  auto ovf_reserve = [&](uint32_t n) -> uint32_t { return own ? atomicAdd(&s_w[9], n) : atomicAdd(&B.ovf_cnt[scan], n); };
  auto flush = [&](uint32_t staged) {
    staged = min(staged, (uint32_t)FX_GATHER_STAGE);
    for (uint32_t k = tid; k < K; k += NT) {
      const uint32_t c = s_kcnt[k];
      if (c) {
        uint32_t base;
        if (solo) {
          base = s_kpos[k];
          s_kpos[k] = base + c;
        } else {
          base = atomicAdd(&B.s_cnt[row0 + k], c);
        }
        s_kbase[k] = base;
        if (base + c > P.list_cap) {
          const uint32_t first = base < P.list_cap ? P.list_cap - base : 0u;
          s_kovf[k] = ovf_reserve(c - first) - first;
        }
// ... 12 lines not shown
          ovf_pts[slot] = s_spt[e];
          ovf_kp[slot] = k;
        }
      }
    }
    if (tid == 0) s_w[8] = 0;
    __syncthreads();
  };
  uint32_t qn = 0;
  auto drain = [&]() {
    wave_sync_lds();
    for (uint32_t t = lane; t < qn; t += 64) {
      const float4 pq = q_pt[t];
      const uint32_t info = q_info[t], st = info & 0xfffffu, cnt = info >> 20;
      for (uint32_t e = 0; e < cnt; ++e) {
        const uint32_t k = s_flat[st + e];
        const float4 kp = s_kp[k];
        const float d2 = dist2(kp.x, kp.y, kp.z, pq.x, pq.y, pq.z);
        if (d2 < P.r2_support) {
          if (d2 < P.r2_search && MODE != 2) {
            if (solo && !passes)
              s_knbr[k] = 1u;
            else
              B.kp_nbrs[(size_t)scan * P.max_keypoints + kb + k] = 1u;
          }
          if (MODE == 1) {
            atomicAdd(&s_kpos[k], 1u);
            continue;
          }
          const uint32_t slot = (FX_GATHER_DIRECT && own) ? FX_GATHER_STAGE : atomicAdd(&s_w[8], 1u);
          if (slot < FX_GATHER_STAGE) {
            s_spt[slot] = pq;
            s_smeta[slot] = (k << 16) | atomicAdd(&s_kcnt[k], 1u);
          } else {
            const uint32_t pos = own ? atomicAdd(&s_kpos[k], 1u) : atomicAdd(&B.s_cnt[row0 + k], 1u);
            if (pos < P.list_cap) {
              B.s_pts[(size_t)(row0 + k) * P.list_cap + pos] = pq;
            } else {
              const uint32_t os = ovf_reserve(1u);
              if (os < P.ovf_cap) {
                ovf_pts[os] = pq;
                ovf_kp[os] = k;
              }
            }
          }
        }
      }
    }
    wave_sync_lds();
    qn = 0;
  };
  uint2 nb_words = make_uint2(0u, 0u);
  uint32_t nb_first = lo;
  auto nb_fill = [&](uint32_t i_first) {
    nb_first = i_first;
    const uint32_t i = i_first + lane * tstep;
    nb_words = make_uint2(0u, 0u);
    if (i < hi) {
      const uint32_t w = (i + wave * 256u) / 128u;
      nb_words = *reinterpret_cast<const uint2 *>(near_bits + w);
    }
  };
  nb_fill(lo);
  auto near_sectors = [&](uint32_t i0) -> unsigned long long {
    if (i0 >= hi) return 0ull;
    uint32_t t = (i0 - nb_first) / tstep;
    if (t >= 64u) nb_fill(i0), t = 0u;
    const uint32_t ts = (uint32_t)__builtin_amdgcn_readfirstlane((int)t);
    return (unsigned long long)(uint32_t)__builtin_amdgcn_readlane((int)nb_words.x, (int)ts) |
           ((unsigned long long)(uint32_t)__builtin_amdgcn_readlane((int)nb_words.y, (int)ts) << 32);
  };
  auto load_tile = [&](uint32_t i0, unsigned long long sect, float4 (&v)[4]) {
#pragma unroll
    for (int u = 0; u < 4; ++u) {
      const uint32_t i = i0 + wave * 256 + u * 64 + lane;
      v[u] = make_float4(NAN, NAN, NAN, 0);
      if (((sect >> (16 * u + (lane >> 2))) & 1ull) && i < hi) v[u] = *reinterpret_cast<const float4 *>(M.pts + (size_t)i * M.stride_f);
    }
  };
  float4 v[4], nv[4];
  unsigned long long nib = near_sectors(lo), nnib = 0;
  load_tile(lo, nib, v);
  for (uint32_t i0 = lo; i0 < hi; i0 += tstep) {
    nnib = near_sectors(i0 + tstep);
    load_tile(i0 + tstep, nnib, nv);
    if (MODE == 0 && i0 != lo && !(FX_GATHER_DIRECT && solo)) {
      __syncthreads();
      const uint32_t staged = s_w[8];
      __syncthreads();
      if (staged > FX_GATHER_STAGE / 2) flush(staged);
    }
#pragma unroll
    for (int u = 0; u < 4; ++u) {
      if (!((nib >> (16 * u)) & 0xffffull)) continue;
      const float x = v[u].x, y = v[u].y, z = v[u].z;
      const float rx = ((M.R[0] * x + M.R[1] * y) + M.R[2] * z) + 0.0f;
      const float ry = ((M.R[3] * x + M.R[4] * y) + M.R[5] * z) + 0.0f;
      const float rz = ((M.R[6] * x + M.R[7] * y) + M.R[8] * z) + 0.0f;
      const bool near = rx >= bx0 && rx <= bx1 && ry >= by0 && ry <= by1 && rz >= bz0 && rz <= bz1 &&
                        isfinite(rx) && isfinite(ry) && isfinite(rz);
      uint32_t info = 0;
      if (near) info = s_cell[cell_y(ry) * ncx + cell_x(rx)];
      const bool has = (info >> 20) != 0u;
      const unsigned long long m = __ballot(has);
      if (m) {
        if (has) {
          const uint32_t slot = qn + lanes_below(m);
          q_pt[slot] = make_float4(rx, ry, rz, __uint_as_float(i0 + wave * 256 + u * 64 + lane));
          q_info[slot] = info;
        }
        qn += (uint32_t)__popcll(m);
        if (qn > kQueue - 64) drain();
      }
    }
    nib = nnib;
#pragma unroll
    for (int u = 0; u < 4; ++u) v[u] = nv[u];
  }
  drain();
  __syncthreads();
  if (MODE == 0) flush(s_w[8]);
  if (MODE == 1) {
    uint32_t *cnt = B.gather_cnt + ((size_t)scan * gridDim.x + slice) * P.max_keypoints;
    for (uint32_t k = tid; k < K; k += NT) cnt[k] = s_kpos[k];
  }
  if (solo) {
    for (uint32_t k = tid; k < K; k += NT) B.s_cnt[row0 + k] = s_kpos[k];
    __syncthreads();
    if (wave == 0 && !passes) {
      uint32_t base = 0;
      for (uint32_t k0 = 0; k0 < K; k0 += 64) {
        const uint32_t k = k0 + lane;
        const unsigned long long m = __ballot(k < K && s_knbr[k] != 0u);
        if (k < K) B.row_xa[row0 + k] = B.xaxis[base + lanes_below(m)];
        base += (uint32_t)__popcll(m);
      }
    }
  }
  } while (PASSES && (kb += MK) < K_all);
  if (solo) {
    if (tid == 0) B.ovf_cnt[scan] = s_w[9];
    if (passes) {
      wg_global_sync();
      if (wave == 0) {
        uint32_t base = 0;
        for (uint32_t k0 = 0; k0 < K_all; k0 += 64) {
          const uint32_t k = k0 + lane;
          const unsigned long long m = __ballot(k < K_all && B.kp_nbrs[(size_t)scan * P.max_keypoints + k] != 0u);
          if (k < K_all) B.row_xa[row_first + k] = B.xaxis[base + lanes_below(m)];
          base += (uint32_t)__popcll(m);
        }
      }
    }
  }
}
extern "C" __global__ __launch_bounds__(FX_GATHER_T) void k_gather(FxDevParams P, FxBuffers B, float box_margin) {
  extern __shared__ __attribute__((aligned(16))) uint32_t smem[];
  gather_body<FX_GATHER_T, false>(P, B, box_margin, smem);
}
extern "C" __global__ __launch_bounds__(FX_GATHER_WIDE_T) void k_gather_wide(FxDevParams P, FxBuffers B, float box_margin) {
  extern __shared__ __attribute__((aligned(16))) uint32_t smem[];
  gather_body<FX_GATHER_WIDE_T, false>(P, B, box_margin, smem);
}
extern "C" __global__ __launch_bounds__(FX_GATHER_T) void k_gather_count(FxDevParams P, FxBuffers B, float box_margin) {
  extern __shared__ __attribute__((aligned(16))) uint32_t smem[];
  gather_body<FX_GATHER_T, false, 1>(P, B, box_margin, smem);
}
extern "C" __global__ __launch_bounds__(FX_GATHER_T) void k_gather_scatter(FxDevParams P, FxBuffers B, float box_margin) {
  extern __shared__ __attribute__((aligned(16))) uint32_t smem[];
  gather_body<FX_GATHER_T, false, 2>(P, B, box_margin, smem);
}
extern "C" __global__ __launch_bounds__(FX_GATHER_WIDE_T) void k_gather_passes(FxDevParams P, FxBuffers B, float box_margin) {
  extern __shared__ __attribute__((aligned(16))) uint32_t smem[];
  gather_body<FX_GATHER_WIDE_T, true>(P, B, box_margin, smem);
}

#ifndef FX_WAVE_CAP
#define FX_WAVE_CAP 192
#endif
#define FX_WAVE_WORDS (FX_WAVE_CAP * 8)
__device__ __forceinline__ void desc_zero_row(float *out, uint32_t lane, uint32_t stride) {
  const uint32_t head = (uint32_t)((16u - ((uintptr_t)out & 15u)) & 15u) / 4u;
  const uint32_t n4 = (FX_DESC_FLOATS - head) / 4u, tail0 = head + 4u * n4;
  if (lane < head) out[lane] = 0.0f;
  if (lane < FX_DESC_FLOATS - tail0) out[tail0 + lane] = 0.0f;
  float4 *body = reinterpret_cast<float4 *>(out + head);
  for (uint32_t t = lane; t < n4; t += stride) body[t] = make_float4(0.f, 0.f, 0.f, 0.f);
}
__device__ __forceinline__ void desc_fill_nan(float *out, uint32_t lane, uint32_t stride) {
  for (uint32_t t = lane; t < FX_DESC_FLOATS; t += stride) out[t] = t < FX_DESC_BINS ? NAN : 0.0f;
}

#define FX_TABLE_WORDS 208
__device__ __forceinline__ const FxScTables *tables_to_lds(const FxBuffers &B, uint32_t *dst) {
  const float *src = reinterpret_cast<const float *>(B.tables);
  for (uint32_t t = threadIdx.x; t < sizeof(FxScTables) / 4; t += blockDim.x) dst[t] = __float_as_uint(src[t]);
  __syncthreads();
  return reinterpret_cast<const FxScTables *>(dst);
}

template <bool FAST>
__device__ __forceinline__ void desc_wave_body(const FxDevParams &P, const FxBuffers &B, uint32_t batch,
                                               uint32_t *smem, uint32_t bid, uint32_t nblk) {
  const uint32_t lane = threadIdx.x & 63, wave = threadIdx.x >> 6;
  const WithinR2 within(P.r2_density);
  uint32_t *base = smem + wave * FX_WAVE_WORDS;
  float4 *sp = reinterpret_cast<float4 *>(base);
  unsigned long long *nkey = reinterpret_cast<unsigned long long *>(base + 4 * FX_WAVE_CAP);
  float *nw = reinterpret_cast<float *>(base + 6 * FX_WAVE_CAP);
  uint32_t *sidx = base + 7 * FX_WAVE_CAP;
  unsigned long long *skey = reinterpret_cast<unsigned long long *>(base);
  float *sw = reinterpret_cast<float *>(base + 2 * FX_WAVE_CAP);
  const FxScTables *T = tables_to_lds(B, smem + FX_NWAVE * FX_WAVE_WORDS);

  uint32_t total = B.kp_offset[batch];
  if (total > P.max_total_kp) total = P.max_total_kp;
  const uint32_t n_items = B.counters[8];
  for (uint32_t it = bid * FX_NWAVE + wave; it < n_items; it += nblk * FX_NWAVE) {
    const uint32_t row = B.wave_desc[it];
    const uint2 rm = B.row_map[row];
    const uint32_t scan = rm.x, k = rm.y;
    const uint32_t nS = B.s_cnt[row];
    const float4 kp = B.row_kp[row];
    const float2 xa = B.row_xa[row];
    float4 lv[FX_WAVE_CAP / 64];
#pragma unroll
    for (uint32_t u = 0; u < FX_WAVE_CAP / 64; ++u)
      if (lane + u * 64 < P.list_cap) lv[u] = B.s_pts[(size_t)row * P.list_cap + lane + u * 64];
    if (nS > FX_WAVE_CAP || nS > P.list_cap) continue;
    float *out = B.desc + (size_t)row * FX_DESC_FLOATS;
    __builtin_amdgcn_wave_barrier();
#pragma unroll
    for (uint32_t u = 0; u < FX_WAVE_CAP / 64; ++u) {
      const uint32_t e = lane + u * 64;
      if (e < nS) {
        const float4 v = lv[u];
        sp[e] = make_float4(v.x, v.y, v.z, dist2(kp.x, kp.y, kp.z, v.x, v.y, v.z));
        sidx[e] = __float_as_uint(v.w);
      }
    }
    __builtin_amdgcn_fence(__ATOMIC_RELEASE, "wavefront");
    __builtin_amdgcn_wave_barrier();
    __builtin_amdgcn_fence(__ATOMIC_ACQUIRE, "wavefront");

    uint32_t nAll = 0, nM = 0;
    bool amb = false;
    for (uint32_t e0 = 0; e0 < nS; e0 += 64) {
      const uint32_t e = e0 + lane;
      const float4 b = e < nS ? sp[e] : make_float4(0, 0, 0, INFINITY);
      const float d2 = b.w;
      const bool nb = d2 < P.r2_search;
      nAll += (uint32_t)__popcll(__ballot(nb));
      const bool use = nb && !sc3d_is_origin(d2);
      unsigned long long key = 0;
      float w = 0.f;
      if (use) {
        float lut;
        const uint32_t bin = sc3d_bin<FAST>(kp, b.x, b.y, b.z, d2, xa, T, lut, amb);
        const uint32_t dens = within.count(sp, 0u, nS, b.x, b.y, b.z);
        w = (1.0f / (float)dens) * lut;
        key = sc3d_key(bin, d2, sidx[e]);
      }
      const unsigned long long um = __ballot(use);
      if (use) {
        const uint32_t pos = nM + lanes_below(um);
        nkey[pos] = key;
        nw[pos] = w;
      }
      nM += (uint32_t)__popcll(um);
    }
    if (lane == 0) B.kp_nbrs[(size_t)scan * P.max_keypoints + k] = nAll;
    if (nAll == 0) {
      desc_fill_nan(out, lane, 64);
      continue;
    }
    __builtin_amdgcn_fence(__ATOMIC_RELEASE, "wavefront");
    __builtin_amdgcn_wave_barrier();
    __builtin_amdgcn_fence(__ATOMIC_ACQUIRE, "wavefront");
    for (uint32_t e0 = 0; e0 < nM; e0 += 64) {
      const uint32_t e = e0 + lane;
      if (e < nM) {
        const unsigned long long key = nkey[e];
        uint32_t rank = 0;
#pragma unroll 8
        for (uint32_t q = 0; q < nM; ++q) rank += (nkey[q] < key) ? 1u : 0u;
        skey[rank] = key;
        sw[rank] = nw[e];
      }
    }
    __builtin_amdgcn_fence(__ATOMIC_RELEASE, "wavefront");
    __builtin_amdgcn_wave_barrier();
    __builtin_amdgcn_fence(__ATOMIC_ACQUIRE, "wavefront");
    for (uint32_t e0 = 0; e0 < nM; e0 += 64) {
      const uint32_t e = e0 + lane;
      if (e >= nM) continue;
      const uint32_t bin = (uint32_t)(skey[e] >> 52);
      if (e > 0 && (uint32_t)(skey[e - 1] >> 52) == bin) continue;
      float acc = 0.0f;
      uint32_t q = e;
      do {
        acc += sw[q];
        ++q;
      } while (q < nM && (uint32_t)(skey[q] >> 52) == bin);
      out[bin] = acc;
    }
    __builtin_amdgcn_wave_barrier();
  }
}

#ifndef FX_GLANES
#define FX_GLANES 16
#endif
#define FX_GROUPS (64 / FX_GLANES)
#ifndef FX_GROUP_CAP
#define FX_GROUP_CAP 64
#endif
#define FX_GROUP_WORDS (FX_GROUP_CAP * 8 + 8)
#ifndef FX_GROUP_UNROLL
#define FX_GROUP_UNROLL 8
#endif
#ifndef FX_GROUP_OCC
#define FX_GROUP_OCC 4
#endif
extern "C" __global__ __launch_bounds__(FX_WG, FX_GROUP_OCC) void k_desc_group(FxDevParams P, FxBuffers B, uint32_t batch) {
  extern __shared__ __attribute__((aligned(16))) uint32_t smem[];
  const uint32_t lane = threadIdx.x & 63, wave = threadIdx.x >> 6;
  const uint32_t gl = lane % FX_GLANES, g = lane / FX_GLANES;
  const WithinR2 within(P.r2_density);
  uint32_t *base = smem + (wave * FX_GROUPS + g) * FX_GROUP_WORDS;
  float4 *sp = reinterpret_cast<float4 *>(base);
  unsigned long long *nkey = reinterpret_cast<unsigned long long *>(base + 4 * FX_GROUP_CAP);
  float *nw = reinterpret_cast<float *>(base + 6 * FX_GROUP_CAP);
  uint32_t *sidx = base + 7 * FX_GROUP_CAP;
  uint32_t *cnt = base + 8 * FX_GROUP_CAP;
  unsigned long long *skey = reinterpret_cast<unsigned long long *>(base);
  float *sw = reinterpret_cast<float *>(base + 2 * FX_GROUP_CAP);
  const FxScTables *T = tables_to_lds(B, smem + FX_NWAVE * FX_GROUPS * FX_GROUP_WORDS);

  uint32_t total = B.kp_offset[batch];
  if (total > P.max_total_kp) total = P.max_total_kp;
  const uint32_t stride = gridDim.x * FX_NWAVE * FX_GROUPS;
  static_assert(FX_GROUP_CAP == 4 * FX_GLANES, "a lane fetches four slots of the row's bin list");
  uint2 f_rm = make_uint2(0u, 0u), f_pb = make_uint2(0u, 0u);
  uint32_t f_nS = 0, f_nb = 0;
  float4 f_kp = make_float4(0, 0, 0, 0), f_lv[FX_GROUP_CAP / FX_GLANES];
  float2 f_xa = make_float2(1.f, 0.f);
  auto fetch = [&](uint32_t row) {
    f_rm = make_uint2(0u, 0u), f_pb = make_uint2(0u, 0u), f_nS = 0, f_nb = 0, f_kp = make_float4(0, 0, 0, 0), f_xa = make_float2(1.f, 0.f);
#pragma unroll
    for (uint32_t u = 0; u < FX_GROUP_CAP / FX_GLANES; ++u) f_lv[u] = make_float4(0, 0, 0, 0);
    if (row < total) {
      f_rm = B.row_map[row];
      f_nS = B.s_cnt[row];
      f_kp = B.row_kp[row];
      f_xa = B.row_xa[row];
#pragma unroll
      for (uint32_t u = 0; u < FX_GROUP_CAP / FX_GLANES; ++u)
        if (gl + u * FX_GLANES < P.list_cap) f_lv[u] = B.s_pts[(size_t)row * P.list_cap + gl + u * FX_GLANES];
      f_nb = B.desc_nbins[row];
      f_pb = *reinterpret_cast<const uint2 *>(B.desc_bins + (size_t)row * FX_GROUP_CAP + 4u * gl);
    }
  };
  fetch((blockIdx.x * FX_NWAVE + wave) * FX_GROUPS + g);
  for (uint32_t r0 = (blockIdx.x * FX_NWAVE + wave) * FX_GROUPS; r0 < total; r0 += stride) {
    const uint32_t row = r0 + g;
    bool live = row < total;
    uint32_t scan = 0, k = 0, nS = 0;
    float4 kp = make_float4(0, 0, 0, 0);
    float2 xa = make_float2(1.f, 0.f);
    float4 lv[FX_GROUP_CAP / FX_GLANES];
    uint32_t nb_prev = 0;
    uint2 pb = make_uint2(0u, 0u);
    if (live) {
      scan = f_rm.x, k = f_rm.y, nS = f_nS, kp = f_kp, xa = f_xa, nb_prev = f_nb, pb = f_pb;
#pragma unroll
      for (uint32_t u = 0; u < FX_GROUP_CAP / FX_GLANES; ++u) lv[u] = f_lv[u];
    }
    float *out = B.desc + (size_t)row * FX_DESC_FLOATS;
    uint16_t *my_bins = B.desc_bins + (size_t)row * FX_GROUP_CAP;
    if (live) {
      if (nb_prev > FX_GROUP_CAP) {
        desc_zero_row(out, gl, FX_GLANES);
      } else {
        const uint32_t t0 = 4u * gl;
        if (t0 + 0u < nb_prev) out[pb.x & 0xffffu] = 0.0f;
        if (t0 + 1u < nb_prev) out[pb.x >> 16] = 0.0f;
        if (t0 + 2u < nb_prev) out[pb.y & 0xffffu] = 0.0f;
        if (t0 + 3u < nb_prev) out[pb.y >> 16] = 0.0f;
      }
    }
    const bool too_long = live && (nS > FX_GROUP_CAP || nS > P.list_cap);
    uint32_t dense_fail = 0;
    {
      const bool lead = too_long && gl == 0;
      const bool to_dense = lead && (nS > P.dense_min || nS > P.list_cap);
      const bool to_list = lead && !to_dense && nS > FX_WAVE_CAP, to_wave = lead && !to_dense && !to_list;
      auto draw = [&](unsigned long long m, bool mine, uint32_t c, uint32_t amount, uint32_t before) -> uint32_t {
        if (!m) return 0u;
        const uint32_t first = (uint32_t)__ffsll((long long)m) - 1u;
        uint32_t b0 = 0;
        if (lane == first) b0 = atomicAdd(&B.counters[c], amount);
        b0 = (uint32_t)__shfl((int)b0, (int)first, 64);
        return mine ? b0 + before : 0u;
      };
      const unsigned long long m_list = __ballot(to_list), m_wave = __ballot(to_wave), m_dense = __ballot(to_dense);
      const uint32_t p_list = draw(m_list, to_list, 4u, (uint32_t)__popcll(m_list), lanes_below(m_list));
      const uint32_t p_wave = draw(m_wave, to_wave, 8u, (uint32_t)__popcll(m_wave), lanes_below(m_wave));
      if (to_list) B.list_desc[p_list] = row;
      if (to_wave) B.wave_desc[p_wave] = row;
      if (m_dense) {
        uint32_t pre = 0, tot = 0;
#pragma unroll
        for (uint32_t g2 = 0; g2 < FX_GROUPS; ++g2) {
          const uint32_t v = (uint32_t)__shfl((int)(to_dense ? nS : 0u), (int)(g2 * FX_GLANES), 64);
          pre += g2 < g ? v : 0u;
          tot += v;
        }
        const uint32_t slot = draw(m_dense, to_dense, 6u, (uint32_t)__popcll(m_dense), lanes_below(m_dense));
        const uint32_t off = draw(m_dense, to_dense, 13u, tot, pre);
        const uint32_t cls = dense_class(nS);
        uint32_t p_cls = 0;
#pragma unroll
        for (uint32_t c2 = 0; c2 < 4u; ++c2) {
          const bool in = to_dense && slot < P.max_dense_rows && cls == c2;
          const unsigned long long m_c = __ballot(in);
          const uint32_t v = draw(m_c, in, dense_class_counter(c2), (uint32_t)__popcll(m_c), lanes_below(m_c));
          p_cls = in ? v : p_cls;
        }
        if (to_dense) {
          const bool ok = slot < P.max_dense_rows && off <= P.dense_cap && nS <= P.dense_cap - off;
          if (slot < P.max_dense_rows) {
            B.dense_rows[slot] = ok ? row : FX_NONE;
            B.dense_off[slot] = off;
            B.dense_order[cls * P.max_dense_rows + p_cls] = slot;
          }
          if (!ok) {
            atomicOr(&B.flags[scan], FX_FLAG_NBR_OVERFLOW);
            B.kp_nbrs[(size_t)scan * P.max_keypoints + k] = FX_NONE;
            dense_fail = 1;
          }
        }
      }
    }
    dense_fail = (uint32_t)__shfl((int)dense_fail, (int)(g * FX_GLANES), 64);
    if (dense_fail) {
      __builtin_amdgcn_fence(__ATOMIC_RELEASE, "workgroup");
      desc_fill_nan(out, gl, FX_GLANES);
    }
    if (too_long && gl == 0) B.desc_nbins[row] = FX_ROW_DIRTY;
    if (too_long) live = false;
    if (!live) nS = 0;
    __builtin_amdgcn_wave_barrier();
#pragma unroll
    for (uint32_t u = 0; u < FX_GROUP_CAP / FX_GLANES; ++u) {
      const uint32_t e = gl + u * FX_GLANES;
      if (e < nS) {
        const float4 v = lv[u];
        sp[e] = make_float4(v.x, v.y, v.z, dist2(kp.x, kp.y, kp.z, v.x, v.y, v.z));
        sidx[e] = __float_as_uint(v.w);
      }
    }
    if (gl < 3) cnt[gl] = 0;
    __builtin_amdgcn_fence(__ATOMIC_RELEASE, "wavefront");
    __builtin_amdgcn_wave_barrier();
    __builtin_amdgcn_fence(__ATOMIC_ACQUIRE, "wavefront");
    for (uint32_t e = gl; e < nS; e += FX_GLANES) {
      const float4 b = sp[e];
      const float d2 = b.w;
      if (!(d2 < P.r2_search)) continue;
      atomicAdd(&cnt[0], 1u);
      if (sc3d_is_origin(d2)) continue;
      float lut;
      bool amb = false;
      const uint32_t bin = sc3d_bin<true>(kp, b.x, b.y, b.z, d2, xa, T, lut, amb);
      const uint32_t dens = within.count(sp, 0u, nS, b.x, b.y, b.z);
      const uint32_t pos = atomicAdd(&cnt[1], 1u);
      nkey[pos] = sc3d_key(bin, d2, sidx[e]);
      nw[pos] = (1.0f / (float)dens) * lut;
    }
    __builtin_amdgcn_fence(__ATOMIC_RELEASE, "wavefront");
    __builtin_amdgcn_wave_barrier();
    __builtin_amdgcn_fence(__ATOMIC_ACQUIRE, "wavefront");
    const uint32_t nAll = live ? cnt[0] : 0u;
    uint32_t nM = live ? cnt[1] : 0u;
    __builtin_amdgcn_fence(__ATOMIC_RELEASE, "workgroup");
    if (live) {
      if (gl == 0) B.kp_nbrs[(size_t)scan * P.max_keypoints + k] = nAll;
      if (nAll == 0) {
        desc_fill_nan(out, gl, FX_GLANES);
        nM = 0;
        if (gl == 0) B.desc_nbins[row] = FX_ROW_DIRTY;
      }
    }
    if (gl == 0) cnt[2] = 0;
    unsigned long long my_key[FX_GROUP_CAP / FX_GLANES];
    float my_w[FX_GROUP_CAP / FX_GLANES];
    uint32_t my_rank[FX_GROUP_CAP / FX_GLANES];
#pragma unroll
    for (uint32_t u = 0; u < FX_GROUP_CAP / FX_GLANES; ++u) {
      const uint32_t e = gl + u * FX_GLANES;
      my_rank[u] = FX_NONE;
      if (e < nM) {
        my_key[u] = nkey[e];
        my_w[u] = nw[e];
        uint32_t rank = 0;
#pragma unroll FX_GROUP_UNROLL
        for (uint32_t q = 0; q < nM; ++q) rank += (nkey[q] < my_key[u]) ? 1u : 0u;
        my_rank[u] = rank;
      }
    }
    __builtin_amdgcn_fence(__ATOMIC_RELEASE, "wavefront");
    __builtin_amdgcn_wave_barrier();
    __builtin_amdgcn_fence(__ATOMIC_ACQUIRE, "wavefront");
#pragma unroll
    for (uint32_t u = 0; u < FX_GROUP_CAP / FX_GLANES; ++u)
      if (my_rank[u] != FX_NONE) {
        skey[my_rank[u]] = my_key[u];
        sw[my_rank[u]] = my_w[u];
      }
    __builtin_amdgcn_fence(__ATOMIC_RELEASE, "wavefront");
    __builtin_amdgcn_wave_barrier();
    __builtin_amdgcn_fence(__ATOMIC_ACQUIRE, "wavefront");
    fetch(r0 + stride + g);
    for (uint32_t e = gl; e < nM; e += FX_GLANES) {
      const uint32_t bin = (uint32_t)(skey[e] >> 52);
      if (e > 0 && (uint32_t)(skey[e - 1] >> 52) == bin) continue;
      float acc = 0.0f;
      uint32_t q = e;
      do {
        acc += sw[q];
        ++q;
      } while (q < nM && (uint32_t)(skey[q] >> 52) == bin);
      out[bin] = acc;
      my_bins[atomicAdd(&cnt[2], 1u)] = (uint16_t)bin;
    }
    __builtin_amdgcn_fence(__ATOMIC_RELEASE, "wavefront");
    __builtin_amdgcn_wave_barrier();
    __builtin_amdgcn_fence(__ATOMIC_ACQUIRE, "wavefront");
    if (live && nAll != 0 && gl == 0) B.desc_nbins[row] = cnt[2];
  }
}

struct DescLds {
  unsigned long long *nkey;
  float4 *sp;
  float *nw, *img;
  uint32_t *sidx, *s_w;
};
#define FX_DESC_WORDS_PER_POINT 8
#define FX_DGRID3 12
__device__ __forceinline__ DescLds desc_carve(uint32_t *smem, uint32_t cap) {
  DescLds L;
  L.s_w = smem;
  uint32_t *p = smem + 16;
  L.sp = (float4 *)p, p += 4 * cap;
  L.nkey = (unsigned long long *)p, p += 2 * cap;
  L.nw = (float *)p, p += cap;
  L.sidx = p, p += cap;
  L.img = (float *)p;
  return L;
}

__device__ __forceinline__ DescLds desc_carve_gs(uint32_t *smem, uint32_t *gs, uint32_t cap) {
  DescLds L;
  L.s_w = smem;
  L.img = (float *)(smem + 16);
  uint32_t *p = gs;
  L.sp = (float4 *)p, p += 4 * (size_t)cap;
  L.nkey = (unsigned long long *)p, p += 2 * (size_t)cap;
  L.nw = (float *)p, p += cap;
  L.sidx = p;
  return L;
}

template <bool FAST, int NT, bool GS = false>
__device__ __forceinline__ bool desc_body(const FxDevParams &P, const FxBuffers &B, uint32_t row, uint32_t scan, uint32_t k,
                          uint32_t cap, uint32_t *smem, bool from_list, uint32_t *gs = nullptr) {
  DescLds L = GS ? desc_carve_gs(smem, gs, cap) : desc_carve(smem, cap);
  FX_STAMP_INIT(B.stamps && FAST ? B.stamps + 48 : nullptr);
  const uint32_t tid = threadIdx.x;
  const WithinR2 within(P.r2_density);
  const FxScanMeta M = B.meta[scan];
  const float4 kp = B.keypoints[(size_t)scan * P.max_keypoints + k];
  float *out = B.desc + (size_t)row * FX_DESC_FLOATS;
  constexpr uint32_t kPre = 4;
  const bool pre = from_list && !GS;
  float4 lv[kPre];
  uint32_t nS_pre = 0;
  float2 xa_pre = make_float2(1.f, 0.f);
  if (pre) {
    nS_pre = B.s_cnt[row];
    xa_pre = B.row_xa[row];
#pragma unroll
    for (uint32_t u = 0; u < kPre; ++u)
      if (tid + u * NT < P.list_cap) lv[u] = B.s_pts[(size_t)row * P.list_cap + tid + u * NT];
  }

  if (tid < 4) L.s_w[tid] = 0;
  uint32_t *tl = reinterpret_cast<uint32_t *>(L.img) + FX_DGRID3 * FX_DGRID3 * FX_DGRID3;
  for (uint32_t t = tid; t < sizeof(FxScTables) / 4; t += NT) tl[t] = __float_as_uint(reinterpret_cast<const float *>(B.tables)[t]);
  wg_sync<GS>();
  uint32_t nS;
  constexpr uint32_t G = FX_DGRID3, kCells = G * G * G;
  uint32_t *cell_end = reinterpret_cast<uint32_t *>(L.img);
  const float r_sup = sqrtf(P.r2_support);
  const float cell_w = fmaxf(sqrtf(P.r2_density) * 1.001f, 2.0f * r_sup / (float)(G - 1) * 1.0001f);
  const float inv_cw = 1.0f / cell_w, gx0 = kp.x - r_sup, gy0 = kp.y - r_sup, gz0 = kp.z - r_sup;
  auto cell_1d = [&](float v, float v0) { return (uint32_t)min(max((int)floorf((v - v0) * inv_cw), 0), (int)G - 1); };
  auto cell_of = [&](float x, float y, float z) { return (cell_1d(z, gz0) * G + cell_1d(y, gy0)) * G + cell_1d(x, gx0); };
  bool grid = false;
  if (from_list) {
    nS = pre ? nS_pre : B.s_cnt[row];
    grid = nS <= cap;
    const bool in_regs = pre && nS <= kPre * NT;
    if (grid) {
      const float4 *lst = B.s_pts + (size_t)row * P.list_cap;
      for (uint32_t t = tid; t < kCells; t += NT) cell_end[t] = 0;
      wg_sync<GS>();
      if (in_regs) {
#pragma unroll
        for (uint32_t u = 0; u < kPre; ++u)
          if (tid + u * NT < nS) atomicAdd(&cell_end[cell_of(lv[u].x, lv[u].y, lv[u].z)], 1u);
      } else {
        for (uint32_t e = tid; e < nS; e += NT) {
          const float4 v = lst[e];
          atomicAdd(&cell_end[cell_of(v.x, v.y, v.z)], 1u);
        }
      }
      wg_sync<GS>();
      if (tid < 64) {
        constexpr uint32_t per = (kCells + 63) / 64;
        uint32_t sum = 0;
        for (uint32_t u = 0; u < per; ++u) {
          const uint32_t ci = tid * per + u;
          sum += ci < kCells ? cell_end[ci] : 0u;
        }
        uint32_t incl = sum;
        incl = wave_incl_scan(incl);
        uint32_t run = incl - sum;
        for (uint32_t u = 0; u < per; ++u) {
          const uint32_t ci = tid * per + u;
          if (ci < kCells) {
            const uint32_t c = cell_end[ci];
            cell_end[ci] = run;
            run += c;
          }
        }
      }
      wg_sync<GS>();
      if (in_regs) {
#pragma unroll
        for (uint32_t u = 0; u < kPre; ++u)
          if (tid + u * NT < nS) {
            const float4 v = lv[u];
            const uint32_t slot = atomicAdd(&cell_end[cell_of(v.x, v.y, v.z)], 1u);
            L.sp[slot] = make_float4(v.x, v.y, v.z, dist2(kp.x, kp.y, kp.z, v.x, v.y, v.z));
            L.sidx[slot] = __float_as_uint(v.w);
          }
      } else {
        for (uint32_t e = tid; e < nS; e += NT) {
          const float4 v = lst[e];
          const uint32_t slot = atomicAdd(&cell_end[cell_of(v.x, v.y, v.z)], 1u);
          L.sp[slot] = make_float4(v.x, v.y, v.z, dist2(kp.x, kp.y, kp.z, v.x, v.y, v.z));
          L.sidx[slot] = __float_as_uint(v.w);
        }
      }
    } else {
      for (uint32_t e = tid; e < nS; e += NT) {
        const float4 v = B.s_pts[(size_t)row * P.list_cap + e];
        L.sp[e] = make_float4(v.x, v.y, v.z, dist2(kp.x, kp.y, kp.z, v.x, v.y, v.z));
        L.sidx[e] = __float_as_uint(v.w);
      }
    }
    wg_sync<GS>();
  } else {
    const uint32_t n = M.n;
    for (uint32_t i0 = 0; i0 < n; i0 += NT * 4) {
      float4 v[4];
#pragma unroll
      for (int u = 0; u < 4; ++u) {
        const uint32_t i = i0 + u * NT + tid;
        v[u] = i < n ? *reinterpret_cast<const float4 *>(M.pts + (size_t)i * M.stride_f) : make_float4(NAN, NAN, NAN, 0);
      }
#pragma unroll
      for (int u = 0; u < 4; ++u) {
        const float x = v[u].x, y = v[u].y, z = v[u].z;
        const float rx = ((M.R[0] * x + M.R[1] * y) + M.R[2] * z) + 0.0f;
        const float ry = ((M.R[3] * x + M.R[4] * y) + M.R[5] * z) + 0.0f;
        const float rz = ((M.R[6] * x + M.R[7] * y) + M.R[8] * z) + 0.0f;
        const float d = dist2(kp.x, kp.y, kp.z, rx, ry, rz);
        if (d < P.r2_support && isfinite(rx) && isfinite(ry) && isfinite(rz)) {
          const uint32_t pos = atomicAdd(&L.s_w[0], 1u);
          if (pos < cap) {
            L.sp[pos] = make_float4(rx, ry, rz, d);
            L.sidx[pos] = i0 + u * NT + tid;
          }
        }
      }
    }
    wg_sync<GS>();
    nS = L.s_w[0];
    if (nS > cap) return false;
  }
  FX_STAMP(1);

  const FxScTables *T = reinterpret_cast<const FxScTables *>(tl);
  const float2 xa = pre ? xa_pre : B.row_xa[row];
  uint32_t *nlist = reinterpret_cast<uint32_t *>(L.nw);
  uint32_t *dens = reinterpret_cast<uint32_t *>(L.nkey);
  {
    uint32_t *scratch = reinterpret_cast<uint32_t *>(L.img) + FX_DESC_BINS - 32;
    uint32_t n_use = 0;
    for (uint32_t e0 = 0; e0 < nS; e0 += NT) {
      const uint32_t e = e0 + tid;
      const float d2 = e < nS ? L.sp[e].w : INFINITY;
      const bool nb = d2 < P.r2_search, use = nb && !sc3d_is_origin(d2);
      const unsigned long long m_nb = __ballot(nb);
      if ((tid & 63u) == 0 && m_nb) atomicAdd(&L.s_w[2], (uint32_t)__popcll(m_nb));
      uint32_t tot;
      const uint32_t r = block_rank<NT>(use, scratch, tot);
      if (use) {
        nlist[n_use + r] = e;
        dens[2 * (n_use + r)] = 0u;
      }
      n_use += tot;
    }
    if (tid == 0) L.s_w[1] = n_use;
  }
  wg_sync<GS>();
  FX_STAMP(6);
  {
    const uint32_t nMq = L.s_w[1];
    uint32_t parts = 1;
    while (parts < (grid ? 8u : 32u) && nMq * parts * 2 <= (uint32_t)NT) parts <<= 1;
    const uint32_t chunk = (nS + parts - 1) / parts;
    for (uint32_t t = tid; t < nMq * parts; t += NT) {
      const uint32_t m = t / parts, part = t % parts;
      const float4 bq = L.sp[nlist[m]];
      uint32_t c = 0;
      if (grid) {
        const uint32_t cx = cell_1d(bq.x, gx0), cy = cell_1d(bq.y, gy0), cz = cell_1d(bq.z, gz0);
        const uint32_t xa0 = cx > 0 ? cx - 1 : 0, xa1 = min(cx + 1, G - 1);
        for (uint32_t rowi = part; rowi < 9; rowi += parts) {
          const uint32_t yy = cy + rowi % 3u - 1u, zz = cz + rowi / 3u - 1u;
          if (yy >= G || zz >= G) continue;
          const uint32_t c0 = (zz * G + yy) * G + xa0, c1 = (zz * G + yy) * G + xa1;
          const uint32_t q0 = c0 ? cell_end[c0 - 1] : 0u, q1 = cell_end[c1];
          c += within.count(L.sp, q0, q1, bq.x, bq.y, bq.z);
        }
      } else {
        const uint32_t q0 = part * chunk, q1 = min(q0 + chunk, nS);
        c += within.count(L.sp, q0, q1, bq.x, bq.y, bq.z);
      }
      if (c) atomicAdd(&dens[2 * m], c);
    }
    wg_sync<GS>();
    FX_STAMP(7);
    for (uint32_t m = tid; m < nMq; m += NT) {
      const uint32_t e = nlist[m];
      const float4 bq = L.sp[e];
      float lut;
      bool amb = false;
      const uint32_t bin = sc3d_bin<FAST>(kp, bq.x, bq.y, bq.z, bq.w, xa, T, lut, amb);
      const uint32_t d = dens[2 * m];
      L.nkey[m] = sc3d_key(bin, bq.w, L.sidx[e]);
      L.nw[m] = (1.0f / (float)d) * lut;
    }
  }
  wg_sync<GS>();
  FX_STAMP(2);
  for (uint32_t t = tid; t < FX_DESC_BINS; t += NT) L.img[t] = 0.0f;
  const uint32_t nM = L.s_w[1], nAll = L.s_w[2];
  if (tid == 0) {
    FX_COUNT(12, 1);
    FX_COUNT(13, nS);
    FX_COUNT(14, nM);
  }
  if (tid == 0) B.kp_nbrs[(size_t)scan * P.max_keypoints + k] = nAll;
  if (nAll == 0) {
    desc_fill_nan(out, tid, NT);
    wg_sync<GS>();
    return true;
  }
  uint32_t *bin_end = reinterpret_cast<uint32_t *>(L.img);
  unsigned long long *skey = reinterpret_cast<unsigned long long *>(L.sp);
  float *sw = reinterpret_cast<float *>(L.sp) + 2 * cap;
  float *sorted_w = reinterpret_cast<float *>(L.sp) + 3 * cap;
  wg_sync<GS>();
  for (uint32_t m = tid; m < nM; m += NT) atomicAdd(&bin_end[(uint32_t)(L.nkey[m] >> 52)], 1u);
  wg_sync<GS>();
  if (tid < 64) {
    constexpr uint32_t per = (FX_DESC_BINS + 63) / 64;
    uint32_t sum = 0;
    for (uint32_t u = 0; u < per; ++u) {
      const uint32_t bi = tid * per + u;
      sum += bi < FX_DESC_BINS ? bin_end[bi] : 0u;
    }
    uint32_t incl = sum;
    incl = wave_incl_scan(incl);
    uint32_t run = incl - sum;
    for (uint32_t u = 0; u < per; ++u) {
      const uint32_t bi = tid * per + u;
      if (bi < FX_DESC_BINS) {
        const uint32_t c = bin_end[bi];
        bin_end[bi] = run;
        run += c;
      }
    }
  }
  wg_sync<GS>();
  for (uint32_t m = tid; m < nM; m += NT) {
    const unsigned long long key = L.nkey[m];
    const uint32_t pos = atomicAdd(&bin_end[(uint32_t)(key >> 52)], 1u);
    skey[pos] = key;
    sw[pos] = L.nw[m];
  }
  wg_sync<GS>();
  for (uint32_t p = tid; p < nM; p += NT) {
    const unsigned long long key = skey[p];
    const uint32_t bin = (uint32_t)(key >> 52);
    const uint32_t s0 = bin ? bin_end[bin - 1u] : 0u, s1 = bin_end[bin];
    uint32_t rank = 0;
    for (uint32_t q = s0; q < s1; ++q) rank += skey[q] < key ? 1u : 0u;
    sorted_w[s0 + rank] = sw[p];
  }
  wg_sync<GS>();
  FX_STAMP(3);
  for (uint32_t bin = tid; bin < FX_DESC_BINS; bin += NT) {
    const uint32_t s0 = bin ? bin_end[bin - 1u] : 0u, s1 = bin_end[bin];
    if (s0 == s1) continue;
    float acc = 0.0f;
    for (uint32_t q = s0; q < s1; ++q) acc += sorted_w[q];
    out[bin] = acc;
  }
  wg_sync<GS>();
  FX_STAMP(4);
  FX_STAMP(5);
  return true;
}

template <bool FAST, int NT>
__device__ __forceinline__ void desc_wg_loop(const FxDevParams &P, const FxBuffers &B, uint32_t batch, uint32_t cap,
                                             uint32_t *smem, uint32_t bid, uint32_t nblk) {
  const uint32_t n_items = B.counters[4];
  for (uint32_t i = bid; i < n_items; i += nblk) {
    const uint32_t row = B.list_desc[i];
    const uint2 rm = B.row_map[row];
    const uint32_t nS = B.s_cnt[row];
    if (nS > P.list_cap || nS > cap) continue;
    desc_body<FAST, NT>(P, B, row, rm.x, rm.y, cap, smem, true);
    __syncthreads();
  }
}
#define FX_DESC_WG_FAST_T 256
#define FX_DSLOW_T 256
__device__ __forceinline__ void dense_slow_loop(const FxDevParams &P, const FxBuffers &B, uint32_t *smem, uint32_t bid, uint32_t nblk) {
  const uint32_t n_rows = min(B.counters[6], P.max_dense_rows);
  uint32_t *gs = B.gsd_pool + (size_t)bid * P.gsd_words;
  for (uint32_t slot = bid; slot < n_rows; slot += nblk) {
    const uint32_t row = B.dense_rows[slot];
    if (row == FX_NONE) continue;
    const uint2 rm = B.row_map[row];
    desc_body<true, FX_DSLOW_T, true>(P, B, row, rm.x, rm.y, P.max_points, smem, false, gs);
    wg_global_sync();
  }
}
static_assert(FX_DSLOW_T == FX_WG && FX_DESC_WG_FAST_T == FX_WG, "k_desc_mid's three kinds of workgroups");
extern "C" __global__ __launch_bounds__(FX_WG) void k_desc_mid(FxDevParams P, FxBuffers B, uint32_t batch, uint32_t cap,
                                                                uint32_t n_wg, uint32_t n_dslow) {
  if (blockIdx.x == 0 && threadIdx.x == 0) {
    B.tier_hint[4] = B.counters[6];
    B.tier_hint[5] = B.counters[13];
  }
  extern __shared__ __attribute__((aligned(16))) uint32_t smem[];
  const uint32_t n_mid = gridDim.x - n_dslow;
  if (blockIdx.x >= n_mid)
    dense_slow_loop(P, B, smem, blockIdx.x - n_mid, n_dslow);
  else if (blockIdx.x < n_wg)
    desc_wg_loop<true, FX_DESC_WG_FAST_T>(P, B, batch, cap, smem, blockIdx.x, n_wg);
  else
    desc_wave_body<true>(P, B, batch, smem, blockIdx.x - n_wg, n_mid - n_wg);
}

#define FX_DG 25
#define FX_DGZ 7
#define FX_DCELLS (FX_DG * FX_DG * FX_DGZ)
#define FX_DENS_BITS 21
#define FX_DENS_MASK ((1ull << FX_DENS_BITS) - 1ull)
#ifndef FX_DSORT_T
#define FX_DSORT_T 512
#endif
#ifndef FX_DSORT_PER_CU
#define FX_DSORT_PER_CU (1024 / FX_DSORT_T)
#endif
#define FX_DSORT_WONW 2048
#define FX_DQ_WON 0x80000000u
#ifndef FX_DFIN_K
#define FX_DFIN_K 14336
#endif
#ifndef FX_DFIN_T
#define FX_DFIN_T 1024
#endif
#ifndef FX_DFIN_OCC
#define FX_DFIN_OCC 1
#endif
__device__ __forceinline__ uint32_t dense_class(uint32_t nS) { return nS > 8192u ? 0u : (nS > 4096u ? 1u : (nS > 2048u ? 2u : 3u)); }
__device__ __forceinline__ uint32_t dense_class_counter(uint32_t cls) { return cls == 0u ? 2u : (cls == 1u ? 3u : (cls == 2u ? 7u : 10u)); }
__device__ __forceinline__ uint32_t dense_nth(const FxDevParams &P, const FxBuffers &B, uint32_t i) {
#pragma unroll
  for (uint32_t cls = 0; cls < 4; ++cls) {
    const uint32_t n = min(B.counters[dense_class_counter(cls)], P.max_dense_rows);
    if (i < n) return B.dense_order[cls * P.max_dense_rows + i];
    i -= n;
  }
  return FX_NONE;
}
__device__ __forceinline__ uint32_t dense_next(const FxDevParams &P, const FxBuffers &B, uint32_t ticket_counter, uint32_t *s_slot) {
  __syncthreads();
  if (threadIdx.x == 0) *s_slot = dense_nth(P, B, atomicAdd(&B.counters[ticket_counter], 1u));
  __syncthreads();
  return *s_slot;
}
struct DenseGrid {
  float gx0, gy0, gz0, inv_cw, inv_ch;
  __device__ __forceinline__ uint32_t cx(float x) const { return (uint32_t)min(max((int)floorf((x - gx0) * inv_cw), 0), FX_DG - 1); }
  __device__ __forceinline__ uint32_t cy(float y) const { return (uint32_t)min(max((int)floorf((y - gy0) * inv_cw), 0), FX_DG - 1); }
  __device__ __forceinline__ uint32_t cz(float z) const { return (uint32_t)min(max((int)floorf((z - gz0) * inv_ch), 0), FX_DGZ - 1); }
  __device__ __forceinline__ uint32_t cell(float x, float y, float z) const { return (cz(z) * FX_DG + cy(y)) * FX_DG + cx(x); }
};
__device__ __forceinline__ DenseGrid dense_grid(const FxDevParams &P, const float4 kp) {
  const float r_sup = sqrtf(P.r2_support), r_d = sqrtf(P.r2_density);
  const float cw = fmaxf(0.5f * r_d * 1.001f, 2.0f * r_sup / (float)(FX_DG - 1) * 1.0001f);
  const float ch = fmaxf(r_d * 1.001f, 2.0f * r_sup / (float)(FX_DGZ - 1) * 1.0001f);
  DenseGrid g;
  g.gx0 = kp.x - r_sup, g.gy0 = kp.y - r_sup, g.gz0 = kp.z - r_sup;
  g.inv_cw = 1.0f / cw, g.inv_ch = 1.0f / ch;
  return g;
}
__device__ __forceinline__ void dense_row_failed(const FxDevParams &P, const FxBuffers &B, uint32_t slot, uint32_t row, uint32_t scan,
                                                 uint32_t k, uint32_t nt) {
  if (threadIdx.x == 0) {
    atomicOr(&B.flags[scan], FX_FLAG_NBR_OVERFLOW);
    B.kp_nbrs[(size_t)scan * P.max_keypoints + k] = FX_NONE;
    B.dense_nq[slot] = 0u;
    B.dense_nm[slot] = FX_NONE;
  }
  desc_fill_nan(B.desc + (size_t)row * FX_DESC_FLOATS, threadIdx.x, nt);
}

template <int NT, bool PAD>
__device__ __forceinline__ uint32_t dense_cells_prefix(uint32_t *cells, uint32_t *tmp) {
  constexpr uint32_t per = (FX_DCELLS + NT - 1) / NT;
  const uint32_t tid = threadIdx.x, lane = tid & 63u, wave = tid >> 6;
  uint32_t sum = 0;
  for (uint32_t u = 0; u < per; ++u) {
    const uint32_t ci = tid * per + u;
    const uint32_t c = ci < FX_DCELLS ? cells[ci] : 0u;
    sum += PAD ? (c + 3u) & ~3u : c;
  }
  uint32_t incl = sum;
  incl = wave_incl_scan(incl);
  if (lane == 63u) tmp[wave] = incl;
  __syncthreads();
  uint32_t run = incl - sum, total = 0;
#pragma unroll
  for (uint32_t w = 0; w < NT / 64; ++w) {
    const uint32_t t = tmp[w];
    run += w < wave ? t : 0u;
    total += t;
  }
  for (uint32_t u = 0; u < per; ++u) {
    const uint32_t ci = tid * per + u;
    if (ci < FX_DCELLS) {
      const uint32_t c = PAD ? (cells[ci] + 3u) & ~3u : cells[ci];
      cells[ci] = run;
      run += c;
    }
  }
  return total;
}

extern "C" __global__ __launch_bounds__(FX_DSORT_T) void k_dense_sort(FxDevParams P, FxBuffers B) {
  __shared__ uint32_t s_scan[FX_DSORT_T / 64];
  __shared__ uint32_t cell_end[FX_DCELLS + 1];
  __shared__ uint32_t s_w[16];
  const uint32_t tid = threadIdx.x;
  __shared__ uint32_t s_slot;
  __shared__ uint32_t won_bits[FX_DSORT_WONW];
  __shared__ uint32_t cell_q[FX_DCELLS + 1];
  if (B.counters[6] == 0u) return;
  const unsigned long long seq = B.seq[0];
  FX_STAMP_INIT(B.stamps ? B.stamps + 16 : nullptr);
  while (true) {
    const uint32_t slot = dense_next(P, B, 11u, &s_slot);
    if (slot == FX_NONE) break;
    const uint32_t row = B.dense_rows[slot];
    if (row == FX_NONE) {
      if (tid == 0) B.dense_nq[slot] = 0u, B.dense_nm[slot] = FX_NONE;
      continue;
    }
    const uint2 rm = B.row_map[row];
    const uint32_t scan = rm.x, k = rm.y;
    const float4 kp = B.row_kp[row];
    const uint32_t nS = B.s_cnt[row], off = B.dense_off[slot];
    const uint32_t n_list = min(nS, P.list_cap);
    const uint32_t n_ovf = nS > P.list_cap ? min(B.ovf_cnt[scan], P.ovf_cap) : 0u;
    const float4 *lst = B.s_pts + (size_t)row * P.list_cap;
    const float4 *ovf = B.ovf_pts + (size_t)scan * P.ovf_cap;
    const uint32_t *ovf_kp = B.ovf_kp + (size_t)scan * P.ovf_cap;
    const DenseGrid G = dense_grid(P, kp);
    float4 *dst = B.dense_pts + off;
    uint32_t *table = B.dense_cells + (size_t)slot * FX_DCELLS;
    __syncthreads();
#ifdef FX_STAMPS
    stamp_prev_ = __builtin_amdgcn_s_memtime();
#endif
    const bool in_lds = nS <= min(32u * FX_DSORT_WONW, P.dense_won_points);
    for (uint32_t t = tid; t < FX_DCELLS + 1; t += FX_DSORT_T) cell_end[t] = 0u, cell_q[t] = 0u;
    if (in_lds)
      for (uint32_t t = tid; t < (nS + 31u) / 32u; t += FX_DSORT_T) won_bits[t] = 0u;
    if (tid < 16) s_w[tid] = 0;
    __syncthreads();
    uint32_t mine = 0;
    auto each_point = [&](auto &&fn, auto &&done) {
      for (uint32_t e0 = 0; e0 < n_list; e0 += 4u * FX_DSORT_T) {
        float4 v[4];
#pragma unroll
        for (int u = 0; u < 4; ++u) {
          const uint32_t e = e0 + (uint32_t)u * FX_DSORT_T + tid;
          if (e < n_list) v[u] = lst[e];
        }
#pragma unroll
        for (int u = 0; u < 4; ++u) fn(v[u], u, e0 + (uint32_t)u * FX_DSORT_T + tid < n_list);
        done();
      }
      for (uint32_t e0 = 0; e0 < n_ovf; e0 += 4u * FX_DSORT_T) {
        uint32_t kk[4];
        float4 v[4];
#pragma unroll
        for (int u = 0; u < 4; ++u) {
          const uint32_t e = e0 + (uint32_t)u * FX_DSORT_T + tid;
          kk[u] = e < n_ovf ? ovf_kp[e] : FX_NONE;
        }
#pragma unroll
        for (int u = 0; u < 4; ++u)
          if (kk[u] == k) v[u] = ovf[e0 + (uint32_t)u * FX_DSORT_T + tid];
#pragma unroll
        for (int u = 0; u < 4; ++u) {
          fn(v[u], u, kk[u] == k);
          mine += kk[u] == k ? 1u : 0u;
        }
        done();
      }
    };
    each_point([&](const float4 &v, int, bool valid) { if (valid) atomicAdd(&cell_end[G.cell(v.x, v.y, v.z)], 1u); }, [] {});
    if (mine) atomicAdd(&s_w[8], mine);
    __syncthreads();
    FX_STAMP(1);
    if (n_list + s_w[8] != nS) {
      dense_row_failed(P, B, slot, row, scan, k, FX_DSORT_T);
// ... 489 lines not shown
      }
      desc_fill_nan(out, tid, NT);
      __syncthreads();
      return;
    }
    for (uint32_t t = tid; t < nM; t += NT) {
      const uint32_t bin = (uint32_t)(sk[t] >> 32);
      if (t > 0 && (uint32_t)(sk[t - 1] >> 32) == bin) continue;
      float acc = 0.0f;
      uint32_t e = t;
      do {
        acc += __uint_as_float((uint32_t)sk[e]);
        ++e;
      } while (e < nM && (uint32_t)(sk[e] >> 32) == bin);
      out[bin] = acc;
    }
    __syncthreads();
    return;
  }
  for (uint32_t t = tid; t < 1984; t += NT) bin_end[t] = 0;
  __syncthreads();
  dense_keys<NT, true>(P, pts, nS, kp, xa, T, keys, bin_end, s_w);
  __syncthreads();
  FX_STAMP(49);
  if (tid < 64) {
    constexpr uint32_t per = 1984 / 64;
    uint32_t sum = 0;
    for (uint32_t u = 0; u < per; ++u) sum += bin_end[tid * per + u];
    uint32_t incl = sum;
    incl = wave_incl_scan(incl);
    uint32_t run = incl - sum;
    for (uint32_t u = 0; u < per; ++u) {
      const uint32_t c = bin_end[tid * per + u];
      bin_end[tid * per + u] = run;
      run += c;
    }
  }
  __syncthreads();
  FX_STAMP(50);
  for (uint32_t e = tid; e < nM; e += NT) ord[atomicAdd(&bin_end[(uint32_t)(keys[e] >> 52)], 1u)] = (uint16_t)e;
  __syncthreads();
  FX_STAMP(51);
  unsigned long long mykey[PER];
#pragma unroll
  for (int u = 0; u < PER; ++u) {
    const uint32_t p = tid + (uint32_t)u * NT;
    mykey[u] = p < nM ? keys[ord[p]] : 0ull;
  }
  __syncthreads();
#pragma unroll
  for (int u = 0; u < PER; ++u) {
    const uint32_t p = tid + (uint32_t)u * NT;
    if (p < nM) keys[p] = mykey[u];
  }
  __syncthreads();
  uint32_t dst[PER];
  float wgt[PER];
#pragma unroll
  for (int u = 0; u < PER; ++u) {
    const uint32_t p = tid + (uint32_t)u * NT;
    dst[u] = FX_NONE;
    if (p < nM) {
      const unsigned long long key = mykey[u];
      const uint32_t bin = (uint32_t)(key >> 52);
      const uint32_t s0 = bin ? bin_end[bin - 1u] : 0u, s1 = bin_end[bin];
      uint32_t rank = 0;
#pragma unroll 4
      for (uint32_t qq = s0; qq < s1; ++qq) rank += keys[qq] < key ? 1u : 0u;
      dst[u] = s0 + rank;
    }
  }
#ifdef FX_STAMPS
  __syncthreads();
  FX_STAMP(57);
#endif
#pragma unroll
  for (int u = 0; u < PER; ++u) {
    const uint32_t p = tid + (uint32_t)u * NT;
    if (p < nM) wgt[u] = dense_weight(mykey[u], cache, seq, T, &s_w[1]);
  }
  __syncthreads();
  FX_STAMP(52);
  if (s_w[1]) {
    if (tid == 0) {
      atomicOr(&B.flags[scan], FX_FLAG_NBR_OVERFLOW);
      B.kp_nbrs[(size_t)scan * P.max_keypoints + B.row_map[row].y] = FX_NONE;
    }
    desc_fill_nan(out, tid, NT);
    __syncthreads();
    return;
  }
  float *sw = reinterpret_cast<float *>(keys);
#pragma unroll
  for (int u = 0; u < PER; ++u)
    if (dst[u] != FX_NONE) sw[dst[u]] = wgt[u];
  __syncthreads();
  for (uint32_t bin = tid; bin < FX_DESC_BINS; bin += NT) {
    const uint32_t s0 = bin ? bin_end[bin - 1u] : 0u, s1 = bin_end[bin];
    if (s0 == s1) continue;
    float acc = 0.0f;
#pragma unroll 4
    for (uint32_t qq = s0; qq < s1; ++qq) acc += sw[qq];
    out[bin] = acc;
  }
  __syncthreads();
  FX_STAMP(53);
  if (tid == 0) {
    FX_COUNT(54, 1);
    FX_COUNT(55, nM);
    FX_COUNT(56, nS);
  }
}
template <int KMAX, int NT>
__device__ __forceinline__ void dense_finish_loop(const FxDevParams &P, const FxBuffers &B) {
  extern __shared__ __attribute__((aligned(16))) uint32_t smem[];
  if (B.counters[6] == 0u) return;
  uint32_t *tl = smem + 2 * KMAX + KMAX / 2 + 1984;
  const FxScTables *T = tables_to_lds(B, tl);
  uint32_t *s_slot = tl + FX_TABLE_WORDS + 8;
  const unsigned long long seq = B.seq[0];
  while (true) {
    const uint32_t slot = dense_next(P, B, 0u, s_slot);
    if (slot == FX_NONE) break;
    const uint32_t nM = B.dense_nm[slot];
    if (nM == FX_NONE) continue;
    const uint32_t row = B.dense_rows[slot];
    const uint2 rm = B.row_map[row];
    if (B.kp_nbrs[(size_t)rm.x * P.max_keypoints + rm.y] == 0u) {
      desc_fill_nan(B.desc + (size_t)row * FX_DESC_FLOATS, threadIdx.x, NT);
      continue;
    }
    if (nM == 0) continue;
    dense_finish_row<KMAX, NT>(P, B, slot, smem, T, seq);
  }
}
extern "C" __global__ __launch_bounds__(FX_DFIN_T, FX_DFIN_OCC) void k_dense_finish(FxDevParams P, FxBuffers B) {
  dense_finish_loop<FX_DFIN_K, FX_DFIN_T>(P, B);
}

extern "C" __global__ __launch_bounds__(FX_WG) void k_rng_ord(FxDevParams P, FxBuffers B, uint32_t batch) {
  const uint32_t b = (blockIdx.x * FX_WG + threadIdx.x) >> 6, lane = threadIdx.x & 63;
  if (b >= batch) return;
  uint32_t K = B.n_kp[b];
  const uint32_t row0 = B.kp_offset[b];
  if (row0 >= P.max_total_kp) return;
  if (row0 + K > P.max_total_kp) K = P.max_total_kp - row0;
  uint32_t base = 0;
  for (uint32_t k0 = 0; k0 < K; k0 += 64) {
    const uint32_t k = k0 + lane;
    const unsigned long long m = __ballot(k < K && B.kp_nbrs[(size_t)b * P.max_keypoints + k] != 0u);
    if (k < K) B.row_xa[row0 + k] = B.xaxis[base + lanes_below(m)];
    base += (uint32_t)__popcll(m);
  }
}

extern "C" __global__ __launch_bounds__(FX_WG) void k_pack_features(FxDevParams P, FxBuffers B, uint32_t batch,
                                                                     uint8_t *dst, uint32_t capacity) {
  uint32_t total = B.kp_offset[batch];
  if (total > P.max_total_kp) total = P.max_total_kp;
  if (total > capacity) total = capacity;
  for (uint32_t w = blockIdx.x; w < total; w += gridDim.x) {
    const uint32_t scan = scan_of_row(B.kp_offset, batch, w);
    const uint32_t k = w - B.kp_offset[scan];
    const float4 kp = B.keypoints[(size_t)scan * P.max_keypoints + k];
    float *rec = reinterpret_cast<float *>(dst + (size_t)w * FX_FEATURE_RECORD_BYTES);
    const float *src = B.desc + (size_t)w * FX_DESC_FLOATS;
    if (threadIdx.x == 0) {
      rec[0] = kp.x;
      rec[1] = kp.y;
      rec[2] = kp.z;
      rec[3] = 1.0f;
      rec[4] = kp.w;
    }
    for (uint32_t t = threadIdx.x; t < FX_DESC_FLOATS; t += FX_WG) rec[5 + t] = src[t];
    if (threadIdx.x < 2) rec[5 + FX_DESC_FLOATS + threadIdx.x] = 0.0f;
  }
}

extern "C" __global__ __launch_bounds__(FX_WG) void k_pack_kp_records(FxDevParams P, FxBuffers B, uint32_t batch,
                                                                       float4 *dst, uint32_t rec_kp) {
  const uint32_t scan = blockIdx.x;
  if (scan >= batch) return;
  float4 *rec = dst + (size_t)scan * (rec_kp + 1);
  const uint32_t K = B.n_kp[scan];
  if (threadIdx.x == 0) {
    uint4 h = make_uint4(K < rec_kp ? K : rec_kp, B.flags[scan] | (K > rec_kp ? FX_FLAG_KP_OVERFLOW : 0u), 0u, 0u);
    rec[0] = *reinterpret_cast<float4 *>(&h);
  }
  const float4 *kp = B.keypoints + (size_t)scan * P.max_keypoints;
  for (uint32_t k = threadIdx.x; k < rec_kp; k += FX_WG) rec[1 + k] = k < K ? kp[k] : make_float4(0, 0, 0, 0);
}

__host__ __device__ inline uint32_t kp_block_off_rows(uint32_t max_scans) { return (max_scans + 1u + 3u) / 4u; }
__host__ __device__ inline uint32_t kp_block_flag_rows(uint32_t max_scans) { return (max_scans + 3u) / 4u; }
extern "C" __global__ __launch_bounds__(FX_WG) void k_pack_kp_block(FxDevParams P, FxBuffers B, uint32_t batch, uint32_t *dst, uint32_t max_scans,
                                                                     uint32_t max_total) {
  __shared__ uint32_t s_or[FX_NWAVE];
  uint32_t *off = dst + 4, *flg = off + 4u * kp_block_off_rows(max_scans);
  float4 *kp = reinterpret_cast<float4 *>(flg + 4u * kp_block_flag_rows(max_scans));
  const uint32_t tid = threadIdx.x, nb = min(batch, max_scans);
  const uint32_t total = min(B.kp_offset[nb], max_total);
  if (blockIdx.x == 0) {
    uint32_t acc = 0;
    for (uint32_t i = tid; i < 4u * kp_block_off_rows(max_scans); i += FX_WG) off[i] = min(B.kp_offset[min(i, nb)], max_total);
    for (uint32_t i = tid; i < 4u * kp_block_flag_rows(max_scans); i += FX_WG) {
      uint32_t f = 0;
      if (i < nb) {
        const uint32_t o0 = B.kp_offset[i], o1 = B.kp_offset[i + 1u];
        f = B.flags[i] | (min(o1, max_total) - min(o0, max_total) < o1 - o0 ? FX_FLAG_KP_OVERFLOW : 0u);
      }
      flg[i] = f;
      acc |= f;
    }
#pragma unroll
    for (int d = 32; d > 0; d >>= 1) acc |= (uint32_t)__shfl_xor((int)acc, d, 64);
    if ((tid & 63u) == 0u) s_or[tid >> 6] = acc;
    __syncthreads();
    if (tid == 0) {
      uint32_t o = batch > max_scans ? FX_FLAG_KP_OVERFLOW : 0u;
      for (uint32_t w = 0; w < FX_NWAVE; ++w) o |= s_or[w];
      dst[0] = nb, dst[1] = total, dst[2] = o, dst[3] = max_total;
    }
  }
  for (uint32_t scan = blockIdx.x; scan < nb; scan += gridDim.x) {
    const uint32_t o0 = min(B.kp_offset[scan], max_total), o1 = min(B.kp_offset[scan + 1u], max_total);
    const float4 *src = B.keypoints + (size_t)scan * P.max_keypoints;
    for (uint32_t k = tid; k < o1 - o0; k += FX_WG) kp[o0 + k] = src[k];
  }
  for (uint32_t k = total + blockIdx.x * FX_WG + tid; k < max_total; k += gridDim.x * FX_WG) kp[k] = make_float4(0, 0, 0, 0);
}

extern "C" __global__ __launch_bounds__(FX_WG) void k_unpack_pc2(const uint8_t *src, uint32_t n, uint32_t point_step,
                                                                  uint32_t off_x, uint32_t off_y, uint32_t off_z,
                                                                  uint32_t off_i, uint32_t big_endian, float4 *dst) {
  for (uint32_t i = blockIdx.x * FX_WG + threadIdx.x; i < n; i += gridDim.x * FX_WG) {
    const uint8_t *rec = src + (size_t)i * point_step;
    auto rd = [&](uint32_t off) -> float {
      uint32_t u = (uint32_t)rec[off] | ((uint32_t)rec[off + 1] << 8) | ((uint32_t)rec[off + 2] << 16) |
                   ((uint32_t)rec[off + 3] << 24);
      if (big_endian) u = __builtin_bswap32(u);
      return __uint_as_float(u);
    };
    dst[i] = make_float4(rd(off_x), rd(off_y), rd(off_z), off_i != 0xffffffffu ? rd(off_i) : 0.0f);
  }
}
extern "C" __global__ __launch_bounds__(FX_WG) void k_pack_xyzi32(const float4 *src, uint32_t n, float *dst) {
  for (uint32_t i = blockIdx.x * FX_WG + threadIdx.x; i < n; i += gridDim.x * FX_WG) {
    const float4 v = src[i];
    float4 *o = reinterpret_cast<float4 *>(dst + (size_t)i * 8);
    o[0] = make_float4(v.x, v.y, v.z, 1.0f);
    o[1] = make_float4(v.w, 0.0f, 0.0f, 0.0f);
  }
}

#ifdef FX_TEST_HOOKS
extern "C" __global__ __launch_bounds__(64) void k_test_sort_replay(const uint32_t *sizes, uint32_t n, uint32_t *perm) {
  __shared__ uint32_t crec[192], tmp[192], stk[FX_SORT_STACK_WORDS];
  const uint32_t *src = sizes + (size_t)blockIdx.x * n;
  for (uint32_t c = threadIdx.x; c < n; c += 64) crec[c] = (src[c] << 16) | c;
  __syncthreads();
  uint16_t *pos = reinterpret_cast<uint16_t *>(tmp);
  if (n <= 64)
    sort_partition_wave<1>(crec, (int)n, (int *)stk, pos, pos + n);
  else if (n <= 128)
    sort_partition_wave<2>(crec, (int)n, (int *)stk, pos, pos + n);
  else
    sort_partition_wave<3>(crec, (int)n, (int *)stk, pos, pos + n);
  __syncthreads();
  for (uint32_t c = threadIdx.x; c < n; c += 64) {
    const uint32_t rec = crec[c], sz = rec >> 16;
    uint32_t at = 0;
    for (uint32_t d = 0; d < n; ++d) {
      const uint32_t sd = crec[d] >> 16;
      at += (sd > sz || (sd == sz && d < c)) ? 1u : 0u;
    }
    tmp[at] = rec;
  }
  __syncthreads();
  for (uint32_t c = threadIdx.x; c < n; c += 64) perm[(size_t)blockIdx.x * n + c] = tmp[c] & 0xffffu;
}

#endif

extern "C" {

size_t fxk_ring_large_lds_bytes(uint32_t cap, uint32_t ccap) {
  return (size_t)(SegCfg<FX_RING_LARGE_T>::kWords + FX_RING_WORDS_PER_POINT * cap + FX_RING_WORDS_PER_CLUSTER * ccap) * 4;
}
void fxk_rings_large(hipStream_t s, const FxDevParams &P, const FxBuffers &B, uint32_t cap, uint32_t ccap, uint32_t grid,
                     uint32_t after_runs2) {
  hipLaunchKernelGGL(k_rings_large, dim3(grid), dim3(FX_RING_LARGE_T), fxk_ring_large_lds_bytes(cap, ccap), s, P, B, cap, ccap, after_runs2);
}
size_t fxk_merge_lds_bytes(uint32_t cap, uint32_t n_rings) { return merge_words(cap, cap, n_rings, true) * 4; }
size_t fxk_merge_huge_lds_bytes(uint32_t cap, uint32_t ccap, uint32_t n_rings) { return merge_words(cap, ccap, n_rings, false) * 4; }
size_t fxk_gather_lds_bytes(uint32_t max_keypoints) { return (size_t)gather_words(std::min(max_keypoints, (uint32_t)FX_GATHER_KCAP), FX_GATHER_WIDE_T) * 4; }
size_t fxk_dense_finish_lds_bytes(void) {
  const size_t k = FX_DFIN_K;
  return (2 * k + k / 2 + 1984 + FX_TABLE_WORDS + 16) * 4;
}
uint32_t fxk_dense_cells(void) { return FX_DCELLS; }
uint32_t fxk_group_cap(void) { return FX_GROUP_CAP; }
uint32_t fxk_dfin_k(void) { return FX_DFIN_K; }
size_t fxk_desc_lds_bytes(uint32_t cap) { return (size_t)(16 + FX_DESC_WORDS_PER_POINT * cap + FX_DESC_BINS) * 4; }

hipError_t fxk_configure(size_t ring_big, size_t merge_big, size_t merge_huge, size_t desc_big, size_t gather) {
  hipError_t e;
  e = hipFuncSetAttribute((const void *)k_merge_huge, hipFuncAttributeMaxDynamicSharedMemorySize, (int)merge_huge);
  if (e != hipSuccess) return e;
  e = hipFuncSetAttribute((const void *)k_merge_huge_a, hipFuncAttributeMaxDynamicSharedMemorySize, (int)merge_huge);
  if (e != hipSuccess) return e;
  e = hipFuncSetAttribute((const void *)k_merge_huge_b, hipFuncAttributeMaxDynamicSharedMemorySize, (int)merge_huge);
  if (e != hipSuccess) return e;
  e = hipFuncSetAttribute((const void *)k_merge_huge_c, hipFuncAttributeMaxDynamicSharedMemorySize, (int)merge_huge);
  if (e != hipSuccess) return e;
  e = hipFuncSetAttribute((const void *)k_gather, hipFuncAttributeMaxDynamicSharedMemorySize, (int)gather);
  if (e != hipSuccess) return e;
  e = hipFuncSetAttribute((const void *)k_gather_wide, hipFuncAttributeMaxDynamicSharedMemorySize, (int)gather);
  if (e != hipSuccess) return e;
  e = hipFuncSetAttribute((const void *)k_gather_count, hipFuncAttributeMaxDynamicSharedMemorySize, (int)gather);
  if (e != hipSuccess) return e;
  e = hipFuncSetAttribute((const void *)k_gather_scatter, hipFuncAttributeMaxDynamicSharedMemorySize, (int)gather);
  if (e != hipSuccess) return e;
  e = hipFuncSetAttribute((const void *)k_gather_passes, hipFuncAttributeMaxDynamicSharedMemorySize, (int)gather);
  if (e != hipSuccess) return e;
  e = hipFuncSetAttribute((const void *)k_rings_large, hipFuncAttributeMaxDynamicSharedMemorySize, (int)ring_big);
  if (e != hipSuccess) return e;
  e = hipFuncSetAttribute((const void *)k_merge_big, hipFuncAttributeMaxDynamicSharedMemorySize, (int)merge_big);
  if (e != hipSuccess) return e;
  e = hipFuncSetAttribute((const void *)k_desc_mid, hipFuncAttributeMaxDynamicSharedMemorySize, (int)desc_big);
  if (e != hipSuccess) return e;
  e = hipFuncSetAttribute((const void *)k_dense_finish, hipFuncAttributeMaxDynamicSharedMemorySize, (int)fxk_dense_finish_lds_bytes());
  return e;
}

uint32_t fxk_near_words(uint32_t max_points) { return (max_points + FX_PREP_TILE - 1) / FX_PREP_TILE * (FX_PREP_TILE / 128); }
void fxk_prep(hipStream_t s, const FxDevParams &P, const FxBuffers &B, uint32_t batch, float near_margin, float el0, float inv_step,
              uint32_t clk_slot) {
  hipLaunchKernelGGL(k_prep, dim3(batch), dim3(FX_PREP_T), 0, s, P, B, near_margin, el0, inv_step, clk_slot);
}
#define FX_PREP_SLICES_MAX 16u
uint32_t fxk_prep_slices_max(void) { return FX_PREP_SLICES_MAX; }
void fxk_prep_sliced(hipStream_t s, const FxDevParams &P, const FxBuffers &B, uint32_t batch, uint32_t slices, float near_margin, float el0, float inv_step,
                     uint32_t clk_slot) {
  hipLaunchKernelGGL(k_prep_count, dim3(slices, batch), dim3(FX_PREP_T), 0, s, P, B);
  hipLaunchKernelGGL(k_prep_sliced, dim3(slices, batch), dim3(FX_PREP_T), 0, s, P, B, near_margin, el0, inv_step, clk_slot);
}
void fxk_bucket_sliced(hipStream_t s, const FxDevParams &P, const FxBuffers &B, uint32_t batch, uint32_t slices, float el0, float inv_step,
                       uint32_t clk_next) {
  const size_t lds = (48 + (size_t)P.n_rings * (2 + FX_BUCKET_NW) + 1) * 4;
  hipLaunchKernelGGL(k_bucket_sliced, dim3(slices, batch), dim3(FX_BUCKET_T), lds, s, P, B, el0, inv_step, clk_next);
}
void fxk_bucket(hipStream_t s, const FxDevParams &P, const FxBuffers &B, uint32_t batch, float el0, float inv_step,
                uint32_t clk_next) {
  const size_t lds = (48 + (size_t)P.n_rings * (2 + FX_BUCKET_NW) + 1) * 4;
  if (P.n_rings > 24)
    hipLaunchKernelGGL(k_bucket_many, dim3(batch), dim3(FX_BUCKET_T), lds, s, P, B, el0, inv_step, clk_next);
  else
    hipLaunchKernelGGL(k_bucket, dim3(batch), dim3(FX_BUCKET_T), lds, s, P, B, el0, inv_step, clk_next);
}
size_t fxk_ring_runs_lds_bytes(void) { return (size_t)rr_words<FX_RR_S, FX_RR_RN>() * 4; }
void fxk_rings_runs2(hipStream_t s, const FxDevParams &P, const FxBuffers &B, uint32_t max_pts, uint32_t grid) {
  constexpr size_t lds = (size_t)rr_words<384, 256>() * 4;
  hipLaunchKernelGGL(k_rings_runs2, dim3(grid), dim3(64), lds, s, P, B, max_pts);
}
void fxk_rings_runs(hipStream_t s, const FxDevParams &P, const FxBuffers &B, uint32_t batch, uint32_t max_pts, uint32_t grid) {
  const uint32_t n_items = batch * (uint32_t)P.n_rings;
  if (grid > n_items) grid = (n_items + 7) / 8 * 8;
  hipLaunchKernelGGL(k_rings_runs, dim3(grid), dim3(64), fxk_ring_runs_lds_bytes(), s, P, B, max_pts, n_items);
}
void fxk_merge_small(hipStream_t s, const FxDevParams &P, const FxBuffers &B, uint32_t batch, uint32_t cap) {
  hipLaunchKernelGGL(k_merge_small, dim3(batch), dim3(FX_MSMALL_T), fxk_merge_lds_bytes(cap, P.n_rings), s, P, B, cap);
}
void fxk_merge_big(hipStream_t s, const FxDevParams &P, const FxBuffers &B, uint32_t cap, uint32_t grid, uint32_t last) {
  hipLaunchKernelGGL(k_merge_big, dim3(grid), dim3(FX_MBIG_T), fxk_merge_lds_bytes(cap, P.n_rings), s, P, B, cap, last);
}
void fxk_merge_huge(hipStream_t s, const FxDevParams &P, const FxBuffers &B, uint32_t cap, uint32_t ccap, uint32_t grid) {
  hipLaunchKernelGGL(k_merge_huge, dim3(grid), dim3(FX_MBIG_T), fxk_merge_huge_lds_bytes(cap, ccap, P.n_rings), s, P, B, cap, ccap);
}
size_t fxk_merge_hp_words(uint32_t cap) { return merge_hp_words(cap); }
uint32_t fxk_merge_slices_max(void) { return FX_MERGE_SLICES; }
void fxk_merge_huge_split(hipStream_t s, const FxDevParams &P, const FxBuffers &B, uint32_t cap, uint32_t ccap, uint32_t grid, uint32_t slices) {
  const size_t lds = fxk_merge_huge_lds_bytes(cap, ccap, P.n_rings);
  hipLaunchKernelGGL(k_merge_huge_a, dim3(grid), dim3(FX_MBIG_T), lds, s, P, B, cap, ccap);
  hipLaunchKernelGGL(k_merge_huge_b, dim3(std::min(slices, (uint32_t)FX_MERGE_SLICES), grid), dim3(FX_MBIG_T), lds, s, P, B, cap, ccap);
  hipLaunchKernelGGL(k_merge_huge_c, dim3(grid), dim3(FX_MBIG_T), lds, s, P, B, cap, ccap);
}
uint32_t fxk_front_max_rings(void) { return FX_FRONT_RMAX; }
uint32_t fxk_front_merge_cap(void) { return FX_FRONT_MERGE; }
void fxk_front(hipStream_t s, const FxDevParams &P, const FxBuffers &B, uint32_t batch, float near_margin, float el0, float inv_step,
               uint32_t clk_slot, uint32_t merge_cap, uint32_t force_redo) {
  hipLaunchKernelGGL(k_front, dim3(batch), dim3(FX_FRONT_T), front_lds_bytes(), s, P, B, near_margin, el0, inv_step, clk_slot, merge_cap, force_redo);
}
void fxk_front_redo(hipStream_t s, const FxDevParams &P, const FxBuffers &B, float el0, float inv_step, uint32_t huge_ccap, uint32_t force_slow,
                    uint32_t grid) {
  hipLaunchKernelGGL(k_front_redo, dim3(grid), dim3(FX_FRONT_T), front_lds_bytes(), s, P, B, el0, inv_step, huge_ccap, force_slow);
}
size_t fxk_slow_words(uint32_t max_ring_points, uint32_t max_candidates, uint32_t huge_ccap) {
  return (std::max(slow_ring_words(max_ring_points), slow_merge_words(max_candidates, huge_ccap)) + 3) & ~(size_t)3;
}
void fxk_slow(hipStream_t s, const FxDevParams &P, const FxBuffers &B, uint32_t huge_ccap, uint32_t grid, uint32_t batch, uint32_t clk_next) {
  const size_t lds = std::max((size_t)SegCfg<FX_SLOW_T>::kWords, (size_t)FX_MERGE_HEAD + ((2 * ((size_t)P.n_rings + 1) + 3) & ~(size_t)3)) * 4;
  const uint32_t g = std::max(1u, std::min(grid, P.gs_slots));
  hipLaunchKernelGGL(k_slow, dim3(g), dim3(FX_SLOW_T), lds, s, P, B, huge_ccap, batch, clk_next);
}
void fxk_front_ab(hipStream_t s, const FxDevParams &P, const FxBuffers &B, uint32_t batch, float near_margin, float el0, float inv_step,
                  uint32_t clk_slot, uint32_t force_redo) {
  hipLaunchKernelGGL(k_front_ab, dim3(batch), dim3(FX_FRONT_T), front_ab_lds_bytes(), s, P, B, near_margin, el0, inv_step, clk_slot, force_redo);
}
void fxk_front_cd(hipStream_t s, const FxDevParams &P, const FxBuffers &B, uint32_t batch, uint32_t clk_slot, uint32_t merge_cap, uint32_t lean,
                  uint32_t self_n, uint32_t force_redo) {
  if (lean && !self_n)
    hipLaunchKernelGGL(k_front_cdl, dim3(batch), dim3(FX_FRONT_CDL_T), front_lean_lds_bytes(), s, P, B, clk_slot, merge_cap);
  else
    hipLaunchKernelGGL(k_front_cd, dim3(batch), dim3(FX_FRONT_T), front_lds_bytes(), s, P, B, clk_slot, merge_cap, self_n, force_redo);
}
hipError_t fxk_configure_front(void) {
  hipError_t e = hipFuncSetAttribute((const void *)k_front, hipFuncAttributeMaxDynamicSharedMemorySize, (int)front_lds_bytes());
  if (e != hipSuccess) return e;
  e = hipFuncSetAttribute((const void *)k_front_ab, hipFuncAttributeMaxDynamicSharedMemorySize, (int)front_ab_lds_bytes());
  if (e != hipSuccess) return e;
  e = hipFuncSetAttribute((const void *)k_front_cd, hipFuncAttributeMaxDynamicSharedMemorySize, (int)front_lds_bytes());
  if (e != hipSuccess) return e;
  return hipFuncSetAttribute((const void *)k_front_redo, hipFuncAttributeMaxDynamicSharedMemorySize, (int)front_lds_bytes());
}
#ifndef FX_GATHER_SLICES
#define FX_GATHER_SLICES 1u
#endif
uint32_t fxk_gather_slices(uint32_t batch) { return batch >= 64u ? FX_GATHER_SLICES : (batch >= 16u ? 4u : 16u); }
#define FX_GATHER_COUNTED_MAX 16u
uint32_t fxk_gather_counted_max(void) { return FX_GATHER_COUNTED_MAX; }
uint32_t fxk_gather(hipStream_t s, const FxDevParams &P, const FxBuffers &B, uint32_t batch, float box_margin, uint32_t counted) {
  const uint32_t slices = fxk_gather_slices(batch);
  const size_t lds = (size_t)gather_words(std::min(P.max_keypoints, (uint32_t)FX_GATHER_KCAP), FX_GATHER_T) * 4;
  if (P.max_keypoints > FX_GATHER_KCAP) {
    hipLaunchKernelGGL(k_gather_passes, dim3(slices, batch), dim3(FX_GATHER_WIDE_T), (size_t)gather_words(FX_GATHER_KCAP, FX_GATHER_WIDE_T) * 4, s, P, B, box_margin);
  } else if (counted > 1u && B.gather_cnt) {
    counted = std::min(counted, (uint32_t)FX_GATHER_COUNTED_MAX);
    hipLaunchKernelGGL(k_gather_count, dim3(counted, batch), dim3(FX_GATHER_T), lds, s, P, B, box_margin);
    hipLaunchKernelGGL(k_gather_scatter, dim3(counted, batch), dim3(FX_GATHER_T), lds, s, P, B, box_margin);
    return counted;
  } else if (slices == 1 && batch < 1024u) {
    hipLaunchKernelGGL(k_gather_wide, dim3(1, batch), dim3(FX_GATHER_WIDE_T), (size_t)gather_words(std::min(P.max_keypoints, (uint32_t)FX_GATHER_KCAP), FX_GATHER_WIDE_T) * 4, s, P, B, box_margin);
  } else {
    hipLaunchKernelGGL(k_gather, dim3(slices, batch), dim3(FX_GATHER_T), lds, s, P, B, box_margin);
  }
  return slices;
}
void fxk_desc_group(hipStream_t s, const FxDevParams &P, const FxBuffers &B, uint32_t batch, uint32_t grid) {
  hipLaunchKernelGGL(k_desc_group, dim3(grid), dim3(FX_WG), (size_t)(FX_NWAVE * FX_GROUPS * FX_GROUP_WORDS + FX_TABLE_WORDS) * 4, s, P, B, batch);
}
void fxk_desc_mid(hipStream_t s, const FxDevParams &P, const FxBuffers &B, uint32_t batch, uint32_t cap, uint32_t n_wg,
                  uint32_t n_wave, uint32_t n_dslow) {
  const size_t lds_wave = (size_t)(FX_NWAVE * FX_WAVE_WORDS + FX_TABLE_WORDS) * 4, lds_wg = fxk_desc_lds_bytes(cap);
  static_assert((16 + FX_DESC_BINS + 16) * 4 <= (FX_NWAVE * FX_WAVE_WORDS + FX_TABLE_WORDS) * 4, "the dense tier's rows in k_desc_mid's LDS");
  n_dslow = std::min(n_dslow, P.gsd_slots);
  hipLaunchKernelGGL(k_desc_mid, dim3(n_wg + n_wave + n_dslow), dim3(FX_WG), lds_wave > lds_wg ? lds_wave : lds_wg, s, P, B, batch, cap, n_wg, n_dslow);
}
size_t fxk_dense_slow_words(uint32_t max_points) { return ((size_t)FX_DESC_WORDS_PER_POINT * max_points + 3) & ~(size_t)3; }
void fxk_dense(hipStream_t s, const FxDevParams &P, const FxBuffers &B, uint32_t n_cu, uint32_t rows, uint32_t items, uint32_t skip) {
  auto grid = [](uint32_t want, uint32_t full) { return want < full ? (want ? want : 1u) : full; };
  hipLaunchKernelGGL(k_dense_sort, dim3(grid(rows, n_cu * FX_DSORT_PER_CU)), dim3(FX_DSORT_T), 0, s, P, B);
  if (!(skip & 2u)) hipLaunchKernelGGL(k_dense_density, dim3(grid(items, n_cu * FX_DDENS_PER_CU)), dim3(FX_DDENS_T), 0, s, P, B);
  if (!(skip & 1u)) hipLaunchKernelGGL(k_dense_finish, dim3(grid(rows, n_cu)), dim3(FX_DFIN_T), fxk_dense_finish_lds_bytes(), s, P, B);
}
#ifdef FX_TEST_HOOKS
extern "C" __global__ __launch_bounds__(FX_WG) void k_test_elevation(const float *xyz, uint32_t n, const double *tab, float *fast, uint8_t *ok,
                                                                     float *exact) {
  __shared__ double s_atan[(FX_ATAN_N + 1) * (FX_ATAN_DEG + 1)];
  for (uint32_t r = threadIdx.x; r < (FX_ATAN_N + 1) * (FX_ATAN_DEG + 1); r += FX_WG) s_atan[r] = tab[r];
  __syncthreads();
  for (uint32_t i = blockIdx.x * FX_WG + threadIdx.x; i < n; i += gridDim.x * FX_WG) {
    const float x = xyz[3 * i], y = xyz[3 * i + 1], z = xyz[3 * i + 2];
    float f = 0.f;
    ok[i] = elevation_fast(x, y, z, s_atan, f) ? 1 : 0;
    fast[i] = f;
    exact[i] = elevation_deg(x, y, z);
  }
}
extern "C" __global__ __launch_bounds__(FX_WG) void k_test_within(const float4 *sp, uint32_t n, const float4 *queries, float r2,
                                                                  uint32_t *packed, uint32_t *plain) {
  __shared__ float4 s_pts[1024];
  __shared__ uint32_t s_cnt[2];
  const float4 b = queries[blockIdx.x];
  const WithinR2 within(r2);
  if (threadIdx.x < 2) s_cnt[threadIdx.x] = 0;
  for (uint32_t c0 = 0; c0 < n; c0 += 1024) {
    const uint32_t m = min(1024u, n - c0);
    __syncthreads();
    for (uint32_t t = threadIdx.x; t < m; t += FX_WG) s_pts[t] = sp[c0 + t];
    __syncthreads();
    const uint32_t per = (m + FX_WG - 1) / FX_WG + (blockIdx.x & 3u);
    const uint32_t q0 = min(threadIdx.x * per, m), q1 = min(q0 + per, m);
    uint32_t a = within.count(s_pts, q0, q1, b.x, b.y, b.z), c = 0;
    for (uint32_t q = q0; q < q1; ++q) c += dist2(b.x, b.y, b.z, s_pts[q].x, s_pts[q].y, s_pts[q].z) < r2 ? 1u : 0u;
    if (threadIdx.x == 0 && FX_WG * per < m) {
      a += within.count(s_pts, FX_WG * per, m, b.x, b.y, b.z);
      for (uint32_t q = FX_WG * per; q < m; ++q) c += dist2(b.x, b.y, b.z, s_pts[q].x, s_pts[q].y, s_pts[q].z) < r2 ? 1u : 0u;
    }
    if (a) atomicAdd(&s_cnt[0], a);
    if (c) atomicAdd(&s_cnt[1], c);
  }
  __syncthreads();
  if (threadIdx.x == 0) packed[blockIdx.x] = s_cnt[0], plain[blockIdx.x] = s_cnt[1];
}
void fxk_test_within(hipStream_t s, const float4 *sp, uint32_t n, const float4 *queries, uint32_t nq, float r2, uint32_t *packed, uint32_t *plain) {
  hipLaunchKernelGGL(k_test_within, dim3(nq), dim3(FX_WG), 0, s, sp, n, queries, r2, packed, plain);
}
void fxk_test_elevation(hipStream_t s, const float *xyz, uint32_t n, const double *tab, float *fast, uint8_t *ok, float *exact) {
  hipLaunchKernelGGL(k_test_elevation, dim3(1024), dim3(FX_WG), 0, s, xyz, n, tab, fast, ok, exact);
}
void fxk_test_sort_replay(hipStream_t s, const uint32_t *sizes, uint32_t n_seq, uint32_t n, uint32_t *perm) {
  hipLaunchKernelGGL(k_test_sort_replay, dim3(n_seq), dim3(64), 0, s, sizes, n, perm);
}
#endif
void fxk_rng_ord(hipStream_t s, const FxDevParams &P, const FxBuffers &B, uint32_t batch) {
  hipLaunchKernelGGL(k_rng_ord, dim3((batch + FX_NWAVE - 1) / FX_NWAVE), dim3(FX_WG), 0, s, P, B, batch);
}
void fxk_pack_kp_records(hipStream_t s, const FxDevParams &P, const FxBuffers &B, uint32_t batch, void *dst,
                         uint32_t rec_kp) {
  hipLaunchKernelGGL(k_pack_kp_records, dim3(batch), dim3(FX_WG), 0, s, P, B, batch, (float4 *)dst, rec_kp);
}
size_t fxk_kp_block_bytes(uint32_t max_scans, uint32_t max_total) {
  return ((size_t)1 + kp_block_off_rows(max_scans) + kp_block_flag_rows(max_scans) + max_total) * 16;
}
void fxk_pack_kp_block(hipStream_t s, const FxDevParams &P, const FxBuffers &B, uint32_t batch, void *dst, uint32_t max_scans, uint32_t max_total,
                       uint32_t grid) {
  hipLaunchKernelGGL(k_pack_kp_block, dim3(grid), dim3(FX_WG), 0, s, P, B, batch, (uint32_t *)dst, max_scans, max_total);
}
void fxk_unpack_pc2(hipStream_t s, const void *src, uint32_t n, uint32_t point_step, uint32_t ox, uint32_t oy, uint32_t oz,
                    uint32_t oi, uint32_t big_endian, void *dst, uint32_t grid) {
  hipLaunchKernelGGL(k_unpack_pc2, dim3(grid), dim3(FX_WG), 0, s, (const uint8_t *)src, n, point_step, ox, oy, oz, oi,
                     big_endian, (float4 *)dst);
}
void fxk_pack_xyzi32(hipStream_t s, const void *src, uint32_t n, void *dst, uint32_t grid) {
  hipLaunchKernelGGL(k_pack_xyzi32, dim3(grid), dim3(FX_WG), 0, s, (const float4 *)src, n, (float *)dst);
}
void fxk_pack_features(hipStream_t s, const FxDevParams &P, const FxBuffers &B, uint32_t batch, void *dst,
                       uint32_t capacity, uint32_t grid) {
  hipLaunchKernelGGL(k_pack_features, dim3(grid), dim3(FX_WG), 0, s, P, B, batch, (uint8_t *)dst, capacity);
}

}
```

Before: 2.140 million scans/s.

## Fuse descriptor tiers into one k_desc kernel with row classification moved to gather

Row classification into list/wave/dense tiers moves out of k_desc_group into the end of the gather kernels and k_rng_ord. A single new k_desc kernel then runs the workgroup, wave and group descriptor tiers plus the dense slow path in one launch, with each tier clearing its own previously written bins. This removes one kernel launch and the serialization between k_desc_group and k_desc_mid, and lets the tiers share one grid. The cost is an extra grid-wide sync in gather, heavier LDS and register use in the fused kernel, and one combined occupancy setting for all tiers.

```diff
diff --git a/feature_extraction_amd/capi.py b/feature_extraction_amd/capi.py
--- a/feature_extraction_amd/capi.py
+++ b/feature_extraction_amd/capi.py
@@ -23,6 +23,7 @@
                  "k_bucket": ("k_bucket", "k_bucket_many"),
                  "k_rings_large": ("k_rings_runs2", "k_rings_large"),
                  "k_merge": ("k_merge_small", "k_merge_big", "k_merge_huge", "k_front_redo", "k_slow"),
+                 "k_desc_group": ("k_desc", "k_desc_group"),
                  "k_desc_mid": ("k_desc_mid",),
                  "k_gather": ("k_gather", "k_rng_ord"),
                  "k_desc_rare": ("k_dense_sort", "k_dense_density", "k_dense_finish")}
diff --git a/feature_extraction_amd/csrc/fx_api.cpp b/feature_extraction_amd/csrc/fx_api.cpp
--- a/feature_extraction_amd/csrc/fx_api.cpp
+++ b/feature_extraction_amd/csrc/fx_api.cpp
@@ -63,6 +63,7 @@
 void fxk_desc_group(hipStream_t s, const FxDevParams &P, const FxBuffers &B, uint32_t batch, uint32_t grid);
 void fxk_desc_mid(hipStream_t s, const FxDevParams &P, const FxBuffers &B, uint32_t batch, uint32_t cap, uint32_t n_wg, uint32_t n_wave,
                   uint32_t n_dslow);
+void fxk_desc(hipStream_t s, const FxDevParams &P, const FxBuffers &B, uint32_t batch, uint32_t cap, uint32_t grid, uint32_t n_dslow);
 void fxk_pack_kp_records(hipStream_t s, const FxDevParams &P, const FxBuffers &B, uint32_t batch, void *dst,
                          uint32_t rec_kp);
 size_t fxk_kp_block_bytes(uint32_t max_scans, uint32_t max_total);
@@ -264,7 +265,9 @@
     const uint32_t desc_per_cu = c->desc_wgs_per_cu ? c->desc_wgs_per_cu : (c->batches_in_flight >= 4u ? 1u : (c->batches_in_flight == 3u ? 3u : 10u));
     const uint32_t rows_bound = std::min<uint64_t>((uint64_t)batch * L.max_keypoints, L.max_total_keypoints);
     uint32_t desc_grid = std::max(1u, std::min((uint32_t)c->n_cu * desc_per_cu, (rows_bound + 15u) / 16u));
-    if (c->desc_grid_abs) desc_grid = c->desc_grid_abs;
+    const uint32_t one_per_cu = c->desc_wgs_per_cu ? c->desc_wgs_per_cu : 3u;
+    uint32_t one_grid = std::max(1u, std::min((uint32_t)c->n_cu * one_per_cu, (rows_bound + 15u) / 16u));
+    if (c->desc_grid_abs) desc_grid = one_grid = c->desc_grid_abs;
     const uint32_t clk_slot = (uint32_t)(c->batch_seq % FX_CLK_SLOTS), clk_next = (uint32_t)((c->batch_seq + 1) % FX_CLK_SLOTS);
     const float el0 = (float)c->params.el0_deg, inv_step = (float)(1.0 / c->params.el_step_deg);
     if (front) {
@@ -342,15 +345,24 @@
         counted = 3u * big_grid / (batch * c->batches_in_flight);
       if (fxk_gather(s, P, B, batch, c->box_margin, counted) > 1) fxk_rng_ord(s, P, B, batch);
       FX_HIP(mark(6));
-      fxk_desc_group(s, P, B, batch, desc_grid);
-      FX_HIP(mark(7));
+      const uint32_t cap = P.list_cap < P.dense_min ? P.list_cap : P.dense_min;
+      if (!P.desc_classify) {
+        fxk_desc_group(s, P, B, batch, desc_grid);
+        FX_HIP(mark(7));
+      }
       bool fast = capture || hint[4] != 0u;
       if (fast && !capture && hint[4] != 0xffffffffu) c->dense_fast_left = fx_ctx::dense_linger;
       if (!fast && c->dense_fast_left) --c->dense_fast_left, fast = true;
       if (c->dense_force >= 0) fast = c->dense_force == 0;
       const bool skip_dense = (c->skip_mask & 2u) != 0u;
-      fxk_desc_mid(s, P, B, batch, P.list_cap < P.dense_min ? P.list_cap : P.dense_min, std::max(1u, std::min(big_grid * 4, rows_bound)),
-                   std::max(1u, std::min(big_grid * 4, (rows_bound + 3u) / 4u)), fast || skip_dense ? 0u : (c->tier_min_grid ? c->tier_min_grid : 8u));
+      const uint32_t n_dslow = fast || skip_dense ? 0u : (c->tier_min_grid ? c->tier_min_grid : 8u);
+      if (P.desc_classify) {
+        fxk_desc(s, P, B, batch, cap, one_grid, n_dslow);
+        FX_HIP(mark(7));
+      } else {
+        fxk_desc_mid(s, P, B, batch, cap, std::max(1u, std::min(big_grid * 4, rows_bound)), std::max(1u, std::min(big_grid * 4, (rows_bound + 3u) / 4u)),
+                     n_dslow);
+      }
       FX_HIP(mark(8));
       if (fast && !skip_dense) {
         const uint32_t max_rows = batch * L.max_keypoints < L.max_total_keypoints ? batch * L.max_keypoints : L.max_total_keypoints;
@@ -533,6 +545,7 @@
   P.list_cap = L.max_neighbors < kListCap ? L.max_neighbors : kListCap;
   P.near_words = fxk_near_words(L.max_points);
   P.dense_min = kDenseMin;
+  P.desc_classify = 1u;
   P.ovf_cap = L.max_overflow_points > 0x7ff00000u ? 0x7ff00000u : L.max_overflow_points;
   {
     const unsigned long long want = L.max_dense_points ? L.max_dense_points : (unsigned long long)(L.max_batch > 32u ? L.max_batch : 32u) * L.max_points;
@@ -752,6 +765,7 @@
   if (const char *e = test_hook("FX_FAIL_AFTER_ENQUEUE")) c->fail_after = (uint32_t)std::max(0, atoi(e));
   if (const char *e = test_hook("FX_SKIP_EMPTY")) c->skip_mask = (uint32_t)std::max(0, atoi(e));
   if (const char *e = test_hook("FX_DENSE_SLOW")) c->dense_force = atoi(e) != 0 ? 1 : 0;
+  if (const char *e = test_hook("FX_DESC_SPLIT")) c->dp.desc_classify = atoi(e) != 0 ? 0u : 1u;
   if (const char *e = test_hook("FX_PREP_SLICES")) c->prep_slices = std::max(1, atoi(e));
   if (const char *e = test_hook("FX_MERGE_SLICES")) c->merge_slices = std::max(1, atoi(e));
   if (const char *e = test_hook("FX_GATHER_COUNTED")) c->gather_slices = std::max(1, atoi(e));
diff --git a/feature_extraction_amd/csrc/fx_device.h b/feature_extraction_amd/csrc/fx_device.h
--- a/feature_extraction_amd/csrc/fx_device.h
+++ b/feature_extraction_amd/csrc/fx_device.h
@@ -35,6 +35,7 @@
   uint32_t gs_slots;
   uint32_t gs_words;
   uint32_t gsd_slots, gsd_words;
+  uint32_t desc_classify;
 };
 
 struct FxScTables {
diff --git a/feature_extraction_amd/csrc/fx_kernels.hip b/feature_extraction_amd/csrc/fx_kernels.hip
--- a/feature_extraction_amd/csrc/fx_kernels.hip
+++ b/feature_extraction_amd/csrc/fx_kernels.hip
@@ -3735,6 +3735,72 @@
   w += (nt / 64) * gather_queue(nt) * 5;
   return w;
 }
+#ifndef FX_WAVE_CAP
+#define FX_WAVE_CAP 192
+#endif
+#ifndef FX_GLANES
+#define FX_GLANES 16
+#endif
+#define FX_GROUPS (64 / FX_GLANES)
+#ifndef FX_GROUP_CAP
+#define FX_GROUP_CAP 64
+#endif
+#define FX_GROUP_WORDS (FX_GROUP_CAP * 8 + 8)
+__device__ __forceinline__ uint32_t dense_class(uint32_t nS) { return nS > 8192u ? 0u : (nS > 4096u ? 1u : (nS > 2048u ? 2u : 3u)); }
+__device__ __forceinline__ uint32_t dense_class_counter(uint32_t cls) { return cls == 0u ? 2u : (cls == 1u ? 3u : (cls == 2u ? 7u : 10u)); }
+__device__ __forceinline__ void desc_classify_rows(const FxDevParams &P, const FxBuffers &B, uint32_t row_lo, uint32_t row_hi,
+                                                   uint32_t wave, uint32_t nwave) {
+  const uint32_t lane = threadIdx.x & 63u;
+  auto draw = [&](unsigned long long m, bool mine, uint32_t c, uint32_t amount, uint32_t before) -> uint32_t {
+    if (!m) return 0u;
+    const uint32_t first = (uint32_t)__ffsll((long long)m) - 1u;
+    uint32_t b0 = 0;
+    if (lane == first) b0 = atomicAdd(&B.counters[c], amount);
+    b0 = (uint32_t)__shfl((int)b0, (int)first, 64);
+    return mine ? b0 + before : 0u;
+  };
+  for (uint32_t r0 = row_lo + wave * 64u; r0 < row_hi; r0 += nwave * 64u) {
+    const uint32_t row = r0 + lane;
+    const uint32_t nS = row < row_hi ? B.s_cnt[row] : 0u;
+    const bool too_long = nS > FX_GROUP_CAP || nS > P.list_cap;
+    const bool to_dense = too_long && (nS > P.dense_min || nS > P.list_cap);
+    const bool to_list = too_long && !to_dense && nS > FX_WAVE_CAP, to_wave = too_long && !to_dense && !to_list;
+    const unsigned long long m_list = __ballot(to_list), m_wave = __ballot(to_wave), m_dense = __ballot(to_dense);
+    const uint32_t p_list = draw(m_list, to_list, 4u, (uint32_t)__popcll(m_list), lanes_below(m_list));
+    const uint32_t p_wave = draw(m_wave, to_wave, 8u, (uint32_t)__popcll(m_wave), lanes_below(m_wave));
+    if (to_list) B.list_desc[p_list] = row;
+    if (to_wave) B.wave_desc[p_wave] = row;
+    if (m_dense) {
+      const uint32_t v = to_dense ? nS : 0u, incl = wave_incl_scan(v);
+      const uint32_t tot = (uint32_t)__shfl((int)incl, 63, 64);
+      const uint32_t slot = draw(m_dense, to_dense, 6u, (uint32_t)__popcll(m_dense), lanes_below(m_dense));
+      const uint32_t off = draw(m_dense, to_dense, 13u, tot, incl - v);
+      const uint32_t cls = dense_class(nS);
+      uint32_t p_cls = 0;
+#pragma unroll
+      for (uint32_t c2 = 0; c2 < 4u; ++c2) {
+        const bool in = to_dense && slot < P.max_dense_rows && cls == c2;
+        const unsigned long long m_c = __ballot(in);
+        const uint32_t pc = draw(m_c, in, dense_class_counter(c2), (uint32_t)__popcll(m_c), lanes_below(m_c));
+        p_cls = in ? pc : p_cls;
+      }
+      if (to_dense) {
+        const bool ok = slot < P.max_dense_rows && off <= P.dense_cap && nS <= P.dense_cap - off;
+        if (slot < P.max_dense_rows) {
+          B.dense_rows[slot] = ok ? row : FX_NONE;
+          B.dense_off[slot] = off;
+          B.dense_order[cls * P.max_dense_rows + p_cls] = slot;
+        }
+        if (!ok) {
+          const uint2 rm = B.row_map[row];
+          atomicOr(&B.flags[rm.x], FX_FLAG_NBR_OVERFLOW);
+          B.kp_nbrs[(size_t)rm.x * P.max_keypoints + rm.y] = FX_NONE;
+        }
+      }
+    }
+  }
+}
+
 template <int NT, bool PASSES, int MODE = 0>
 __device__ __forceinline__ void gather_body(const FxDevParams &P, const FxBuffers &B, float box_margin, uint32_t *smem) {
   static_assert(MODE == 0 || !PASSES, "the counted slices hold a scan's keypoints in one pass");
@@ -4053,6 +4119,10 @@
         }
       }
     }
+    if (P.desc_classify) {
+      wg_global_sync();
+      desc_classify_rows(P, B, row_first, row_first + K_all, wave, FX_GATHER_NW);
+    }
   }
 }
 extern "C" __global__ __launch_bounds__(FX_GATHER_T) void k_gather(FxDevParams P, FxBuffers B, float box_margin) {
@@ -4076,9 +4146,6 @@
   gather_body<FX_GATHER_WIDE_T, true>(P, B, box_margin, smem);
 }
 
-#ifndef FX_WAVE_CAP
-#define FX_WAVE_CAP 192
-#endif
 #define FX_WAVE_WORDS (FX_WAVE_CAP * 8)
 __device__ __forceinline__ void desc_zero_row(float *out, uint32_t lane, uint32_t stride) {
   const uint32_t head = (uint32_t)((16u - ((uintptr_t)out & 15u)) & 15u) / 4u;
@@ -4100,19 +4167,20 @@
   return reinterpret_cast<const FxScTables *>(dst);
 }
 
-template <bool FAST>
+#define FX_ONE_WAVE_WORDS (FX_WAVE_WORDS > FX_GROUPS * FX_GROUP_WORDS ? FX_WAVE_WORDS : FX_GROUPS * FX_GROUP_WORDS)
+template <bool FAST, bool ONE = false>
 __device__ __forceinline__ void desc_wave_body(const FxDevParams &P, const FxBuffers &B, uint32_t batch,
-                                               uint32_t *smem, uint32_t bid, uint32_t nblk) {
+                                               uint32_t *smem, uint32_t bid, uint32_t nblk, const FxScTables *T_one = nullptr) {
   const uint32_t lane = threadIdx.x & 63, wave = threadIdx.x >> 6;
   const WithinR2 within(P.r2_density);
-  uint32_t *base = smem + wave * FX_WAVE_WORDS;
+  uint32_t *base = smem + wave * (ONE ? FX_ONE_WAVE_WORDS : FX_WAVE_WORDS);
   float4 *sp = reinterpret_cast<float4 *>(base);
   unsigned long long *nkey = reinterpret_cast<unsigned long long *>(base + 4 * FX_WAVE_CAP);
   float *nw = reinterpret_cast<float *>(base + 6 * FX_WAVE_CAP);
   uint32_t *sidx = base + 7 * FX_WAVE_CAP;
   unsigned long long *skey = reinterpret_cast<unsigned long long *>(base);
   float *sw = reinterpret_cast<float *>(base + 2 * FX_WAVE_CAP);
-  const FxScTables *T = tables_to_lds(B, smem + FX_NWAVE * FX_WAVE_WORDS);
+  const FxScTables *T = ONE ? T_one : tables_to_lds(B, smem + FX_NWAVE * FX_WAVE_WORDS);
 
   uint32_t total = B.kp_offset[batch];
   if (total > P.max_total_kp) total = P.max_total_kp;
@@ -4130,6 +4198,15 @@
       if (lane + u * 64 < P.list_cap) lv[u] = B.s_pts[(size_t)row * P.list_cap + lane + u * 64];
     if (nS > FX_WAVE_CAP || nS > P.list_cap) continue;
     float *out = B.desc + (size_t)row * FX_DESC_FLOATS;
+    uint16_t *my_bins = B.desc_bins + (size_t)row * FX_GROUP_CAP;
+    if (ONE) {
+      const uint32_t nb_prev = B.desc_nbins[row];
+      if (nb_prev > FX_GROUP_CAP)
+        desc_zero_row(out, lane, 64);
+      else if (lane < nb_prev)
+        out[my_bins[lane]] = 0.0f;
+      __builtin_amdgcn_fence(__ATOMIC_RELEASE, "workgroup");
+    }
     __builtin_amdgcn_wave_barrier();
 #pragma unroll
     for (uint32_t u = 0; u < FX_WAVE_CAP / 64; ++u) {
@@ -4173,6 +4250,7 @@
     if (lane == 0) B.kp_nbrs[(size_t)scan * P.max_keypoints + k] = nAll;
     if (nAll == 0) {
       desc_fill_nan(out, lane, 64);
+      if (ONE && lane == 0) B.desc_nbins[row] = FX_ROW_DIRTY;
       continue;
     }
     __builtin_amdgcn_fence(__ATOMIC_RELEASE, "wavefront");
@@ -4192,39 +4270,41 @@
     __builtin_amdgcn_fence(__ATOMIC_RELEASE, "wavefront");
     __builtin_amdgcn_wave_barrier();
     __builtin_amdgcn_fence(__ATOMIC_ACQUIRE, "wavefront");
+    uint32_t n_rec = 0;
     for (uint32_t e0 = 0; e0 < nM; e0 += 64) {
       const uint32_t e = e0 + lane;
-      if (e >= nM) continue;
-      const uint32_t bin = (uint32_t)(skey[e] >> 52);
-      if (e > 0 && (uint32_t)(skey[e - 1] >> 52) == bin) continue;
-      float acc = 0.0f;
-      uint32_t q = e;
-      do {
-        acc += sw[q];
-        ++q;
-      } while (q < nM && (uint32_t)(skey[q] >> 52) == bin);
-      out[bin] = acc;
-    }
+      const uint32_t bin = e < nM ? (uint32_t)(skey[e] >> 52) : 0u;
+      const bool first = e < nM && !(e > 0 && (uint32_t)(skey[e - 1] >> 52) == bin);
+      if (first) {
+        float acc = 0.0f;
+        uint32_t q = e;
+        do {
+          acc += sw[q];
+          ++q;
+        } while (q < nM && (uint32_t)(skey[q] >> 52) == bin);
+        out[bin] = acc;
+      }
+      if (ONE) {
+        const unsigned long long m = __ballot(first);
+        const uint32_t i = n_rec + lanes_below(m);
+        if (first && i < FX_GROUP_CAP) my_bins[i] = (uint16_t)bin;
+        n_rec += (uint32_t)__popcll(m);
+      }
+    }
+    if (ONE && lane == 0) B.desc_nbins[row] = n_rec <= FX_GROUP_CAP ? n_rec : FX_ROW_DIRTY;
     __builtin_amdgcn_wave_barrier();
   }
 }
 
-#ifndef FX_GLANES
-#define FX_GLANES 16
-#endif
-#define FX_GROUPS (64 / FX_GLANES)
-#ifndef FX_GROUP_CAP
-#define FX_GROUP_CAP 64
-#endif
-#define FX_GROUP_WORDS (FX_GROUP_CAP * 8 + 8)
 #ifndef FX_GROUP_UNROLL
 #define FX_GROUP_UNROLL 8
 #endif
 #ifndef FX_GROUP_OCC
 #define FX_GROUP_OCC 4
 #endif
-extern "C" __global__ __launch_bounds__(FX_WG, FX_GROUP_OCC) void k_desc_group(FxDevParams P, FxBuffers B, uint32_t batch) {
-  extern __shared__ __attribute__((aligned(16))) uint32_t smem[];
+template <bool ONE>
+__device__ __forceinline__ void desc_group_rows(const FxDevParams &P, const FxBuffers &B, uint32_t batch, uint32_t *smem,
+                                                const FxScTables *T, bool clear_dense, uint32_t nblk) {
   const uint32_t lane = threadIdx.x & 63, wave = threadIdx.x >> 6;
   const uint32_t gl = lane % FX_GLANES, g = lane / FX_GLANES;
   const WithinR2 within(P.r2_density);
@@ -4236,11 +4316,10 @@
   uint32_t *cnt = base + 8 * FX_GROUP_CAP;
   unsigned long long *skey = reinterpret_cast<unsigned long long *>(base);
   float *sw = reinterpret_cast<float *>(base + 2 * FX_GROUP_CAP);
-  const FxScTables *T = tables_to_lds(B, smem + FX_NWAVE * FX_GROUPS * FX_GROUP_WORDS);
 
   uint32_t total = B.kp_offset[batch];
   if (total > P.max_total_kp) total = P.max_total_kp;
-  const uint32_t stride = gridDim.x * FX_NWAVE * FX_GROUPS;
+  const uint32_t stride = nblk * FX_NWAVE * FX_GROUPS;
   static_assert(FX_GROUP_CAP == 4 * FX_GLANES, "a lane fetches four slots of the row's bin list");
   uint2 f_rm = make_uint2(0u, 0u), f_pb = make_uint2(0u, 0u);
   uint32_t f_nS = 0, f_nb = 0;
@@ -4279,7 +4358,15 @@
     }
     float *out = B.desc + (size_t)row * FX_DESC_FLOATS;
     uint16_t *my_bins = B.desc_bins + (size_t)row * FX_GROUP_CAP;
-    if (live) {
+    const bool too_long = live && (nS > FX_GROUP_CAP || nS > P.list_cap);
+    uint32_t dense_fail = 0;
+    bool clear_it = live;
+    if (ONE && too_long) {
+      const bool dense = nS > P.dense_min || nS > P.list_cap;
+      dense_fail = dense && B.kp_nbrs[(size_t)scan * P.max_keypoints + k] == FX_NONE ? 1u : 0u;
+      clear_it = dense && (clear_dense || dense_fail);
+    }
+    if (clear_it) {
       if (nb_prev > FX_GROUP_CAP) {
         desc_zero_row(out, gl, FX_GLANES);
       } else {
@@ -4290,9 +4377,7 @@
         if (t0 + 3u < nb_prev) out[pb.y >> 16] = 0.0f;
       }
     }
-    const bool too_long = live && (nS > FX_GROUP_CAP || nS > P.list_cap);
-    uint32_t dense_fail = 0;
-    {
+    if (!ONE) {
       const bool lead = too_long && gl == 0;
       const bool to_dense = lead && (nS > P.dense_min || nS > P.list_cap);
       const bool to_list = lead && !to_dense && nS > FX_WAVE_CAP, to_wave = lead && !to_dense && !to_list;
@@ -4348,7 +4433,7 @@
       __builtin_amdgcn_fence(__ATOMIC_RELEASE, "workgroup");
       desc_fill_nan(out, gl, FX_GLANES);
     }
-    if (too_long && gl == 0) B.desc_nbins[row] = FX_ROW_DIRTY;
+    if (clear_it && too_long && gl == 0) B.desc_nbins[row] = FX_ROW_DIRTY;
     if (too_long) live = false;
     if (!live) nS = 0;
     __builtin_amdgcn_wave_barrier();
@@ -4440,6 +4525,11 @@
     __builtin_amdgcn_fence(__ATOMIC_ACQUIRE, "wavefront");
     if (live && nAll != 0 && gl == 0) B.desc_nbins[row] = cnt[2];
   }
+}
+extern "C" __global__ __launch_bounds__(FX_WG, FX_GROUP_OCC) void k_desc_group(FxDevParams P, FxBuffers B, uint32_t batch) {
+  extern __shared__ __attribute__((aligned(16))) uint32_t smem[];
+  const FxScTables *T = tables_to_lds(B, smem + FX_NWAVE * FX_GROUPS * FX_GROUP_WORDS);
+  desc_group_rows<false>(P, B, batch, smem, T, true, gridDim.x);
 }
 
 struct DescLds {
@@ -4474,7 +4564,7 @@
   return L;
 }
 
-template <bool FAST, int NT, bool GS = false>
+template <bool FAST, int NT, bool GS = false, bool OWN = false>
 __device__ __forceinline__ bool desc_body(const FxDevParams &P, const FxBuffers &B, uint32_t row, uint32_t scan, uint32_t k,
                           uint32_t cap, uint32_t *smem, bool from_list, uint32_t *gs = nullptr) {
   DescLds L = GS ? desc_carve_gs(smem, gs, cap) : desc_carve(smem, cap);
@@ -4498,6 +4588,15 @@
   }
 
   if (tid < 4) L.s_w[tid] = 0;
+  uint16_t *my_bins = B.desc_bins + (size_t)row * FX_GROUP_CAP;
+  if (OWN) {
+    const uint32_t nb_prev = B.desc_nbins[row];
+    if (nb_prev > FX_GROUP_CAP)
+      desc_zero_row(out, tid, NT);
+    else if (tid < nb_prev)
+      out[my_bins[tid]] = 0.0f;
+    __builtin_amdgcn_fence(__ATOMIC_RELEASE, "workgroup");
+  }
   uint32_t *tl = reinterpret_cast<uint32_t *>(L.img) + FX_DGRID3 * FX_DGRID3 * FX_DGRID3;
   for (uint32_t t = tid; t < sizeof(FxScTables) / 4; t += NT) tl[t] = __float_as_uint(reinterpret_cast<const float *>(B.tables)[t]);
   wg_sync<GS>();
@@ -4680,6 +4779,7 @@
   if (tid == 0) B.kp_nbrs[(size_t)scan * P.max_keypoints + k] = nAll;
   if (nAll == 0) {
     desc_fill_nan(out, tid, NT);
+    if (OWN && tid == 0) B.desc_nbins[row] = FX_ROW_DIRTY;
     wg_sync<GS>();
     return true;
   }
@@ -4733,14 +4833,19 @@
     float acc = 0.0f;
     for (uint32_t q = s0; q < s1; ++q) acc += sorted_w[q];
     out[bin] = acc;
+    if (OWN) {
+      const uint32_t i = atomicAdd(&L.s_w[3], 1u);
+      if (i < FX_GROUP_CAP) my_bins[i] = (uint16_t)bin;
+    }
   }
   wg_sync<GS>();
+  if (OWN && tid == 0) B.desc_nbins[row] = L.s_w[3] <= FX_GROUP_CAP ? L.s_w[3] : FX_ROW_DIRTY;
   FX_STAMP(4);
   FX_STAMP(5);
   return true;
 }
 
-template <bool FAST, int NT>
+template <bool FAST, int NT, bool ONE = false>
 __device__ __forceinline__ void desc_wg_loop(const FxDevParams &P, const FxBuffers &B, uint32_t batch, uint32_t cap,
                                              uint32_t *smem, uint32_t bid, uint32_t nblk) {
   const uint32_t n_items = B.counters[4];
@@ -4749,12 +4854,13 @@
     const uint2 rm = B.row_map[row];
     const uint32_t nS = B.s_cnt[row];
     if (nS > P.list_cap || nS > cap) continue;
-    desc_body<FAST, NT>(P, B, row, rm.x, rm.y, cap, smem, true);
+    desc_body<FAST, NT, false, ONE>(P, B, row, rm.x, rm.y, cap, smem, true);
     __syncthreads();
   }
 }
 #define FX_DESC_WG_FAST_T 256
 #define FX_DSLOW_T 256
+template <bool OWN = false>
 __device__ __forceinline__ void dense_slow_loop(const FxDevParams &P, const FxBuffers &B, uint32_t *smem, uint32_t bid, uint32_t nblk) {
   const uint32_t n_rows = min(B.counters[6], P.max_dense_rows);
   uint32_t *gs = B.gsd_pool + (size_t)bid * P.gsd_words;
@@ -4762,7 +4868,7 @@
     const uint32_t row = B.dense_rows[slot];
     if (row == FX_NONE) continue;
     const uint2 rm = B.row_map[row];
-    desc_body<true, FX_DSLOW_T, true>(P, B, row, rm.x, rm.y, P.max_points, smem, false, gs);
+    desc_body<true, FX_DSLOW_T, true, OWN>(P, B, row, rm.x, rm.y, P.max_points, smem, false, gs);
     wg_global_sync();
   }
 }
@@ -4783,6 +4889,30 @@
     desc_wave_body<true>(P, B, batch, smem, blockIdx.x - n_wg, n_mid - n_wg);
 }
 
+#ifndef FX_DESC_OCC
+#define FX_DESC_OCC 3
+#endif
+#define FX_DESC_TABLES (FX_NWAVE * FX_ONE_WAVE_WORDS)
+static_assert(FX_DSLOW_T == FX_WG && FX_DESC_WG_FAST_T == FX_WG, "k_desc's kinds of workgroups");
+extern "C" __global__ __launch_bounds__(FX_WG, FX_DESC_OCC) void k_desc(FxDevParams P, FxBuffers B, uint32_t batch, uint32_t cap,
+                                                                       uint32_t n_dslow) {
+  if (blockIdx.x == 0 && threadIdx.x == 0) {
+    B.tier_hint[4] = B.counters[6];
+    B.tier_hint[5] = B.counters[13];
+  }
+  extern __shared__ __attribute__((aligned(16))) uint32_t smem[];
+  const uint32_t n_main = gridDim.x - n_dslow;
+  if (blockIdx.x >= n_main) {
+    dense_slow_loop<true>(P, B, smem, blockIdx.x - n_main, n_dslow);
+    return;
+  }
+  desc_wg_loop<true, FX_DESC_WG_FAST_T, true>(P, B, batch, cap, smem, blockIdx.x, n_main);
+  __syncthreads();
+  const FxScTables *T = tables_to_lds(B, smem + FX_DESC_TABLES);
+  desc_wave_body<true, true>(P, B, batch, smem, blockIdx.x, n_main, T);
+  desc_group_rows<true>(P, B, batch, smem, T, n_dslow == 0u, n_main);
+}
+
 #define FX_DG 25
 #define FX_DGZ 7
 #define FX_DCELLS (FX_DG * FX_DG * FX_DGZ)
@@ -4805,8 +4935,6 @@
 #ifndef FX_DFIN_OCC
 #define FX_DFIN_OCC 1
 #endif
-__device__ __forceinline__ uint32_t dense_class(uint32_t nS) { return nS > 8192u ? 0u : (nS > 4096u ? 1u : (nS > 2048u ? 2u : 3u)); }
-__device__ __forceinline__ uint32_t dense_class_counter(uint32_t cls) { return cls == 0u ? 2u : (cls == 1u ? 3u : (cls == 2u ? 7u : 10u)); }
 __device__ __forceinline__ uint32_t dense_nth(const FxDevParams &P, const FxBuffers &B, uint32_t i) {
 #pragma unroll
   for (uint32_t cls = 0; cls < 4; ++cls) {
@@ -5602,6 +5730,7 @@
     if (k < K) B.row_xa[row0 + k] = B.xaxis[base + lanes_below(m)];
     base += (uint32_t)__popcll(m);
   }
+  if (P.desc_classify) desc_classify_rows(P, B, row0, row0 + K, 0u, 1u);
 }
 
 extern "C" __global__ __launch_bounds__(FX_WG) void k_pack_features(FxDevParams P, FxBuffers B, uint32_t batch,
@@ -5779,6 +5908,9 @@
   if (e != hipSuccess) return e;
   e = hipFuncSetAttribute((const void *)k_desc_mid, hipFuncAttributeMaxDynamicSharedMemorySize, (int)desc_big);
   if (e != hipSuccess) return e;
+  e = hipFuncSetAttribute((const void *)k_desc, hipFuncAttributeMaxDynamicSharedMemorySize,
+                          (int)std::max(desc_big, (size_t)(FX_DESC_TABLES + FX_TABLE_WORDS) * 4));
+  if (e != hipSuccess) return e;
   e = hipFuncSetAttribute((const void *)k_dense_finish, hipFuncAttributeMaxDynamicSharedMemorySize, (int)fxk_dense_finish_lds_bytes());
   return e;
 }
@@ -5905,6 +6037,15 @@
   static_assert((16 + FX_DESC_BINS + 16) * 4 <= (FX_NWAVE * FX_WAVE_WORDS + FX_TABLE_WORDS) * 4, "the dense tier's rows in k_desc_mid's LDS");
   n_dslow = std::min(n_dslow, P.gsd_slots);
   hipLaunchKernelGGL(k_desc_mid, dim3(n_wg + n_wave + n_dslow), dim3(FX_WG), lds_wave > lds_wg ? lds_wave : lds_wg, s, P, B, batch, cap, n_wg, n_dslow);
+}
+size_t fxk_desc_one_lds_bytes(uint32_t cap) {
+  const size_t lds_tiers = (size_t)(FX_DESC_TABLES + FX_TABLE_WORDS) * 4, lds_wg = fxk_desc_lds_bytes(cap);
+  return lds_tiers > lds_wg ? lds_tiers : lds_wg;
+}
+void fxk_desc(hipStream_t s, const FxDevParams &P, const FxBuffers &B, uint32_t batch, uint32_t cap, uint32_t grid, uint32_t n_dslow) {
+  static_assert((16 + FX_DESC_BINS + 16) * 4 <= (FX_DESC_TABLES + FX_TABLE_WORDS) * 4, "the dense tier's rows in k_desc's LDS");
+  n_dslow = std::min(n_dslow, P.gsd_slots);
+  hipLaunchKernelGGL(k_desc, dim3(grid + n_dslow), dim3(FX_WG), fxk_desc_one_lds_bytes(cap), s, P, B, batch, cap, n_dslow);
 }
 size_t fxk_dense_slow_words(uint32_t max_points) { return ((size_t)FX_DESC_WORDS_PER_POINT * max_points + 3) & ~(size_t)3; }
 void fxk_dense(hipStream_t s, const FxDevParams &P, const FxBuffers &B, uint32_t n_cu, uint32_t rows, uint32_t items, uint32_t skip) {
```

Result: no change. 2.132 million scans/s, median of 3 (-0.4%).
